# martinmodrak/math

Measured on AMD Instinct MI355X. Metric: gradient evals/sec (fp64), GP-marginal log-density N=4096, higher is better.
Workload: dtype f64; 1 GPU; gp_marginal_gradient; N=4096, kernel=exp_quad, parallelism=replicas1

## Files before the change

### include/smg_hip.h

```cpp
#ifndef SMG_HIP_H
#define SMG_HIP_H

#include <stddef.h>

#ifdef __cplusplus
extern "C" {
#endif

enum smg_status_code {
  SMG_OK = 0,
  SMG_ERR_HIP = 1,
  SMG_ERR_NOT_PD = 2,
  SMG_ERR_NOT_SYMMETRIC = 4,
  SMG_ERR_NONFINITE = 8,
  SMG_ERR_ARG = 16,
  SMG_ERR_OOM = 32,
  SMG_ERR_NOT_POSITIVE = 64,
  SMG_ERR_SYNC = 128
};

typedef struct smg_ctx smg_ctx;

int smg_device_count(int* n_host);
int smg_ctx_create(int device, size_t initial_arena_bytes, smg_ctx** out_host);
// ... 13 lines not shown
int smg_publish_to_host(smg_ctx* ctx, const double* src, long long n, double* dst);
int smg_gather_scalars(smg_ctx* ctx, const double* const* src, int n, double* dst, int* status_out);

int smg_memcpy_h2d(smg_ctx* ctx, void* dst, const void* src_host, size_t bytes);
int smg_memcpy_d2h(smg_ctx* ctx, void* dst_host, const void* src, size_t bytes);
int smg_memcpy_d2d(smg_ctx* ctx, void* dst, const void* src, size_t bytes);
int smg_memset(smg_ctx* ctx, void* dst, int value, size_t bytes);
int smg_memset_async(smg_ctx* ctx, void* dst, size_t bytes);
int smg_join_async(smg_ctx* ctx);
int smg_sync(smg_ctx* ctx);
int smg_sync_all(smg_ctx* ctx);
int smg_marker_record(smg_ctx* ctx, int slot);
int smg_marker_wait(smg_ctx* ctx, int slot);
int smg_status(smg_ctx* ctx, int* status_host);
int smg_status_armed(smg_ctx* ctx, int* armed);
int smg_status_enqueue(smg_ctx* ctx, int* host_dst);
int smg_status_inject(smg_ctx* ctx, int bits);
int smg_set_inv_block_mode(smg_ctx* ctx, int mode);
int smg_inv_block_fused(smg_ctx* ctx, int n);
int smg_set_gemm_stage_mode(smg_ctx* ctx, int mode);
int smg_set_gemm_cut_mode(smg_ctx* ctx, int mode);

enum smg_family {
  SMG_FAM_GEMM = 0, SMG_FAM_CHOL_FWD = 1, SMG_FAM_CHOL_REV = 2,
  SMG_FAM_GP = 3, SMG_FAM_MVN = 4, SMG_FAM_TRSV = 5, SMG_FAM_GLM = 6,
  SMG_FAM_ELEMWISE = 7,
  SMG_FAM_PANEL = 8,
  SMG_FAM_COMM = 9,
  SMG_FAM_COUNT = 10
};
int smg_profile_enable(smg_ctx* ctx, int on);
int smg_profile_read(smg_ctx* ctx, int family, double* total_ms_host, long long* count_host);
int smg_profile_flops(smg_ctx* ctx, int family, double* flops_host);

int smg_fill_unif(smg_ctx* ctx, double* out, long long n, unsigned long long seed,
                  double a, double b, double scale);
int smg_fill_bernoulli(smg_ctx* ctx, int* out, long long n, unsigned long long seed, double p);

int smg_gemm(smg_ctx* ctx, int transA, int transB, int uplo, int m, int n, int k,
             double alpha, const double* A, int lda, const double* B, int ldb,
             double beta, double* C, int ldc);
#define SMG_TRI_A_LOWER 1
#define SMG_TRI_A_UPPER 2
#define SMG_TRI_B_LOWER 4
#define SMG_TRI_B_UPPER 8
int smg_gemm_tri(smg_ctx* ctx, int transA, int transB, int uplo, int tri, int m, int n, int k, double alpha,
                 const double* A, int lda, const double* B, int ldb, double beta, double* C, int ldc);
int smg_gemm_bz(smg_ctx* ctx, int transA, int transB, int uplo, int tri, int m, int n, int k, double alpha,
                const double* A, int lda, const double* B, int ldb, double beta, double* C, int ldc, int bz);
int smg_gemm_cut(smg_ctx* ctx, int transA, int transB, int uplo, int tri, int m, int n, int k, double alpha,
                 const double* A, int lda, const double* B, int ldb, double beta, double* C, int ldc, int bz,
                 int cut_a, int cut_b);


int smg_gp_exp_quad_cov_fwd(smg_ctx* ctx, const double* x, int n, double sigma,
                            double l, double* K, int ldk);
int smg_gp_exp_quad_cov_rev(smg_ctx* ctx, const double* x, int n, double sigma,
                            double l, const double* Kadj, int ldka, double* out2);

int smg_gp_exp_quad_cov_nd_fwd(smg_ctx* ctx, const double* x, int D, int n, double sigma,
                               double l, double* K, int ldk);
int smg_gp_exp_quad_cov_nd_rev(smg_ctx* ctx, const double* x, int D, int n, double sigma,
                               double l, const double* Kadj, int ldka, double* out2);

enum smg_gp_family { SMG_GP_EXP_QUAD = 0, SMG_GP_EXPONENTIAL = 1, SMG_GP_MATERN32 = 2, SMG_GP_MATERN52 = 3 };
int smg_gp_cov_fwd(smg_ctx* ctx, int family, const double* x, int D, int n, double sigma, double l,
// ... 274 lines not shown
```

### math_amd/csrc/ctx.hip

```cpp
#include <cstdio>
#include <cstdlib>
#include <cstring>

#include "smg_internal.h"

namespace {

constexpr size_t kAlign = 256;

__global__ void k_reduce_partials(const double* __restrict__ p, int nparts,
                                  int width, double* out, int accumulate) {
  __shared__ double lds[16];
  const int c = blockIdx.x;
  double s = 0.0;
  for (int i = threadIdx.x; i < nparts; i += blockDim.x) s += p[(size_t)i * width + c];
  s = block_sum(s, lds);
  if (threadIdx.x == 0) out[c] = accumulate ? out[c] + s : s;
}

__global__ __launch_bounds__(256) void k_publish(const double* __restrict__ src, long long n, double* dst,
                                                 long long* done, long long seq) {
  for (long long i = threadIdx.x; i < n; i += blockDim.x)
    __hip_atomic_store(dst + i, src[i], __ATOMIC_RELAXED, __HIP_MEMORY_SCOPE_SYSTEM);
  asm volatile("s_waitcnt vmcnt(0)" ::: "memory");
// ... 490 lines not shown
  SMG_HIP_TRY(hipMemcpyAsync(dst, src, bytes, hipMemcpyDeviceToDevice, ctx->stream));
  return SMG_OK;
}

int smg_memset(smg_ctx* ctx, void* dst, int v, size_t bytes) {
  if (!bytes) return SMG_OK;
  if (v == 0) {
    const std::pair<void*, size_t> r(dst, bytes);
    return smg_zero_ranges_impl(ctx, ctx->stream, &r, 1);
  }
  SMG_HIP_TRY(hipMemsetAsync(dst, v, bytes, ctx->stream));
  return SMG_OK;
}

}

int smg_zero_ranges_impl(smg_ctx* ctx, hipStream_t stream, const std::pair<void*, size_t>* r, int count,
                         unsigned max_grid) {
  zero_ranges z{};
  size_t most = 0;
  auto launch = [&]() -> int {
    if (!z.count) return SMG_OK;
    const size_t g = (most / 2 + 255) / 256;
    hipLaunchKernelGGL(k_zero_ranges, dim3(g < max_grid ? (g < 1 ? 1 : (unsigned)g) : max_grid), dim3(256), 0, stream,
                       z);
    SMG_LAUNCH_CHECK();
    z.count = 0;
    most = 0;
    return SMG_OK;
  };
  for (int i = 0; i < count; ++i) {
    const size_t b = r[i].second;
    if (!b) continue;
    if ((reinterpret_cast<uintptr_t>(r[i].first) & 7) || (b & 7)) {
      SMG_HIP_TRY(hipMemsetAsync(r[i].first, 0, b, stream));
      continue;
    }
    z.p[z.count] = static_cast<double*>(r[i].first);
    z.n[z.count] = b / 8;
    most = b / 8 > most ? b / 8 : most;
    if (++z.count == ZR_MAX)
      if (int rc = launch()) return rc;
  }
  return launch();
}

extern "C" {

int smg_zero_stream_begin(smg_ctx* ctx) {
  if (ctx->zero_stream) return SMG_OK;
  if (hipStreamCreateWithFlags(&ctx->zero_stream, hipStreamNonBlocking) != hipSuccess ||
      hipEventCreateWithFlags(&ctx->zero_ev_main, hipEventDisableTiming) != hipSuccess ||
      hipEventCreateWithFlags(&ctx->zero_ev_done, hipEventDisableTiming) != hipSuccess) {
    hipGetLastError();
    ctx->zero_stream = nullptr;
    return SMG_ERR_HIP;
  }
  return SMG_OK;
}

int smg_marker_event(smg_ctx* ctx, int slot, hipEvent_t* ev) {
  if (slot < 0 || slot >= 64) return SMG_ERR_ARG;
  while ((int)ctx->marker_ev.size() <= slot) {
    hipEvent_t e;
    if (hipEventCreateWithFlags(&e, hipEventDisableTiming) != hipSuccess) {
      ctx->host_status |= SMG_ERR_HIP;
// ... 142 lines not shown
  if (in_host_scratch(ctx, host_dst, sizeof(int))) {
    hipLaunchKernelGGL(k_status_copy, dim3(1), dim3(64), 0, ctx->stream, ctx->status_d, host_dst);
    SMG_LAUNCH_CHECK();
  } else {
    SMG_HIP_TRY(hipMemcpyAsync(host_dst, ctx->status_d, sizeof(int), hipMemcpyDeviceToHost, ctx->stream));
  }
  ctx->status_armed = 0;
  return SMG_OK;
}

namespace {
__global__ void k_status_or(int* st, int bits) {
  if (threadIdx.x == 0) st[0] |= bits;
}
}

int smg_status_inject(smg_ctx* ctx, int bits) {
  if (!ctx) return SMG_ERR_ARG;
  hipLaunchKernelGGL(k_status_or, dim3(1), dim3(64), 0, ctx->stream, ctx->status_d, bits);
  SMG_LAUNCH_CHECK();
  ctx->status_armed = 1;
  return SMG_OK;
}

int smg_profile_enable(smg_ctx* ctx, int on) {
  hipStreamSynchronize(ctx->stream);
  prof_drain(ctx);
  ctx->prof_on = on;
  for (int i = 0; i < SMG_FAM_COUNT; ++i) {
    ctx->prof_ms[i] = 0;
    ctx->prof_count[i] = 0;
    ctx->prof_flops[i] = 0;
  }
  return SMG_OK;
}

int smg_profile_read(smg_ctx* ctx, int family, double* ms, long long* count) {
  if (family < 0 || family >= SMG_FAM_COUNT) return SMG_ERR_ARG;
  hipStreamSynchronize(ctx->stream);
  prof_drain(ctx);
  if (ms) *ms = ctx->prof_ms[family];
  if (count) *count = ctx->prof_count[family];
  return SMG_OK;
}

int smg_profile_flops(smg_ctx* ctx, int family, double* flops) {
  if (!ctx || family < 0 || family >= SMG_FAM_COUNT || !flops) return SMG_ERR_ARG;
  *flops = ctx->prof_flops[family];
  return SMG_OK;
}

}

namespace {
__device__ __forceinline__ unsigned long long splitmix(unsigned long long seed, long long i) {
  unsigned long long z = seed + (unsigned long long)(i + 1) * 0x9E3779B97F4A7C15ULL;
  z = (z ^ (z >> 30)) * 0xBF58476D1CE4E5B9ULL;
  z = (z ^ (z >> 27)) * 0x94D049BB133111EBULL;
  return z ^ (z >> 31);
}
__global__ void k_fill_unif(double* out, long long n, unsigned long long seed, double a, double b,
                            double scale) {
  for (long long i = (long long)blockIdx.x * blockDim.x + threadIdx.x; i < n;
       i += (long long)gridDim.x * blockDim.x) {
    const double u = (double)(splitmix(seed, i) >> 11) * (1.0 / 9007199254740992.0);
    const double v = __dadd_rn(a, __dmul_rn(b - a, u));
    out[i] = scale == 1.0 ? v : __dmul_rn(v, scale);
  }
// ... 27 lines not shown
```

### math_amd/csrc/smg_internal.h

```cpp
#pragma once
#include <hip/hip_runtime.h>

#include <cstddef>
#include <cstdint>
#include <utility>
#include <vector>

#include "../../include/smg_hip.h"

#ifndef SMG_GEMM_CUT_DEFAULT
#define SMG_GEMM_CUT_DEFAULT 1
#endif

typedef double d4 __attribute__((ext_vector_type(4)));
typedef double d2v __attribute__((ext_vector_type(2)));

struct smg_arena_block {
  char* base;
  size_t size;
};

struct smg_prof_slot {
  hipEvent_t start, stop;
  int family;
// ... 23 lines not shown
  hipStream_t copy_stream;
  hipEvent_t zero_ev_main, zero_ev_done;
  int zero_pending;
  std::vector<std::pair<void*, size_t>> zero_queue;
  hipEvent_t inv_ev, inv_ev_main, inv_ev_aux;
  int inv_pending;
  hipEvent_t inv_ev_w;
  int inv_w_recorded;
  int* flags_d;
  int flag_epoch;
  unsigned* inv_ctr_d;
  long long inv_launches;
  int inv_per_cu, inv_cus;
  int inv_mode;
  int gemm_stage;
  int gemm_cut;
  void* host_scratch;
  size_t host_scratch_size;
  void* pin_io;
  size_t pin_io_size;
  void* res_h;
  size_t res_h_size;
  long long* done_h;
  long long done_seq;
  unsigned int* red_counter_d;
  double* ws[12];
  size_t ws_doubles[12];
  int prof_on;
  std::vector<smg_prof_slot> prof_pending;
  std::vector<hipEvent_t> prof_pool;
  double prof_ms[SMG_FAM_COUNT];
  double prof_flops[SMG_FAM_COUNT];
  long long prof_count[SMG_FAM_COUNT];
  void* comm;
};

#define SMG_HIP_TRY(expr)                          \
  do {                                             \
    hipError_t _e = (expr);                        \
    if (_e != hipSuccess) {                        \
      if (ctx) ctx->host_status |= SMG_ERR_HIP;    \
      return SMG_ERR_HIP;                          \
    }                                              \
  } while (0)

#define SMG_LAUNCH_CHECK()                         \
  do {                                             \
    hipError_t _e = hipGetLastError();             \
    if (_e != hipSuccess) {                        \
      ctx->host_status |= SMG_ERR_HIP;             \
      return SMG_ERR_HIP;                          \
    }                                              \
  } while (0)

struct smg_prof_scope {
  smg_ctx* ctx;
  int fam;
  hipEvent_t a, b;
  bool on;
  smg_prof_scope(smg_ctx* c, int f);
  ~smg_prof_scope();
};

enum { SMG_WS_GEMM = 0, SMG_WS_RED = 1, SMG_WS_TMP = 2, SMG_WS_TMP2 = 3, SMG_WS_ALIAS = 4,
       SMG_WS_GEMM_SIDE = 5, SMG_WS_INV = 6, SMG_WS_CW = 7, SMG_WS_RHS = 8,
       SMG_WS_GLM = 9,
// ... 121 lines not shown
```

### math_amd/hip.py

```python
import ctypes
import os

import numpy as np

_HERE = os.path.dirname(os.path.abspath(__file__))
LIB_PATH = os.path.join(_HERE, "lib", "libsmg_hip.so")

SMG_OK = 0
STATUS = {1: "hip", 2: "not_pd", 4: "not_symmetric", 8: "nonfinite", 16: "arg", 32: "oom", 64: "not_positive"}
GP_FAMILIES = {"exp_quad": 0, "exponential": 1, "matern32": 2, "matern52": 3}
FAMILIES = {"gemm": 0, "chol_fwd": 1, "chol_rev": 2, "gp": 3, "mvn": 4, "trsv": 5, "glm": 6, "elementwise": 7, "panel": 8, "comm": 9}

_P = ctypes.c_void_p
_I = ctypes.c_int
_L = ctypes.c_longlong
_D = ctypes.c_double
_S = ctypes.c_size_t

_SIGS = {
    "smg_device_count": (_I, [ctypes.POINTER(_I)]),
    "smg_ctx_create": (_I, [_I, _S, ctypes.POINTER(_P)]),
    "smg_ctx_destroy": (_I, [_P]),
    "smg_ctx_device": (_I, [_P]),
    "smg_ctx_stream": (_P, [_P]),
    "smg_arena_alloc": (_P, [_P, _S]),
    "smg_arena_mark": (_S, [_P]),
    "smg_arena_rewind": (_I, [_P, _S]),
    "smg_arena_recover_all": (_I, [_P]),
    "smg_arena_used": (_S, [_P]),
    "smg_arena_reserved": (_S, [_P]),
    "smg_host_scratch": (_P, [_P, _S]),
    "smg_memcpy_h2d": (_I, [_P, _P, _P, _S]),
    "smg_memcpy_d2h": (_I, [_P, _P, _P, _S]),
    "smg_memcpy_d2d": (_I, [_P, _P, _P, _S]),
    "smg_memset": (_I, [_P, _P, _I, _S]),
    "smg_memset_async": (_I, [_P, _P, _S]),
    "smg_join_async": (_I, [_P]),
    "smg_sync": (_I, [_P]),
    "smg_sync_all": (_I, [_P]),
    "smg_status": (_I, [_P, ctypes.POINTER(_I)]),
    "smg_status_armed": (_I, [_P, ctypes.POINTER(_I)]),
    "smg_status_enqueue": (_I, [_P, _P]),
    "smg_status_inject": (_I, [_P, _I]),
    "smg_set_inv_block_mode": (_I, [_P, _I]),
    "smg_inv_block_fused": (_I, [_P, _I]),
    "smg_set_gemm_stage_mode": (_I, [_P, _I]),
    "smg_set_gemm_cut_mode": (_I, [_P, _I]),
    "smg_pinned_io": (_P, [_P, _S]),
    "smg_pinned_result": (_P, [_P, _S]),
    "smg_gather_scalars": (_I, [_P, _P, _I, _P, _P]),
    "smg_pack_tril": (_I, [_P, _I, _I, _P, _I, _P]),
    "smg_unpack_tril_add": (_I, [_P, _I, _I, _P, _P, _I]),
    "smg_publish_to_host": (_I, [_P, _P, _L, _P]),
    "smg_profile_enable": (_I, [_P, _I]),
    "smg_profile_read": (_I, [_P, _I, ctypes.POINTER(_D), ctypes.POINTER(_L)]),
    "smg_profile_flops": (_I, [_P, _I, ctypes.POINTER(_D)]),
    "smg_fill_unif": (_I, [_P, _P, _L, ctypes.c_ulonglong, _D, _D, _D]),
    "smg_fill_bernoulli": (_I, [_P, _P, _L, ctypes.c_ulonglong, _D]),
    "smg_gemm": (_I, [_P, _I, _I, _I, _I, _I, _I, _D, _P, _I, _P, _I, _D, _P, _I]),
    "smg_gemm_tri": (_I, [_P, _I, _I, _I, _I, _I, _I, _I, _D, _P, _I, _P, _I, _D, _P, _I]),
    "smg_gemm_bz": (_I, [_P, _I, _I, _I, _I, _I, _I, _I, _D, _P, _I, _P, _I, _D, _P, _I, _I]),
    "smg_gemm_cut": (_I, [_P, _I, _I, _I, _I, _I, _I, _I, _D, _P, _I, _P, _I, _D, _P, _I, _I, _I, _I]),
    "smg_gp_exp_quad_cov_fwd": (_I, [_P, _P, _I, _D, _D, _P, _I]),
    "smg_gp_exp_quad_cov_rev": (_I, [_P, _P, _I, _D, _D, _P, _I, _P]),
    "smg_bernoulli_logit_glm_checked": (_I, [_P, _P, _P, _L, _I, _L, _P, _P, _P]),
    "smg_bernoulli_logit_glm_io": (_I, [_P, _P, _P, _L, _I, _L, _D, _P, _P, _P, _P]),
    "smg_marker_record": (_I, [_P, _I]),
    "smg_marker_wait": (_I, [_P, _I]),
    "smg_gp_exp_quad_cov_nd_fwd": (_I, [_P, _P, _I, _I, _D, _D, _P, _I]),
    "smg_gp_exp_quad_cov_nd_rev": (_I, [_P, _P, _I, _I, _D, _D, _P, _I, _P]),
    "smg_add_diag_fwd": (_I, [_P, _P, _I, _I, _D, _P, _P, _I]),
    "smg_add_diag_rev": (_I, [_P, _P, _I, _I, _P, _I, _P, _I]),
    "smg_cholesky_block_size": (_I, [_I]),
    "smg_check_symmetric": (_I, [_P, _P, _I, _I]),
    "smg_cholesky_fwd": (_I, [_P, _P, _I, _I, _P, _I, _P]),
    "smg_cholesky_fwd_checked": (_I, [_P, _P, _I, _I, _P, _I, _P]),
    "smg_cholesky_fwd_checked_mark": (_I, [_P, _P, _I, _I, _P, _I, _P]),
    "smg_status_mark_wait": (_I, [_P, _P]),
    "smg_cholesky_rev": (_I, [_P, _P, _I, _P, _P, _I, _I, _P, _I]),
    "smg_mdivide_left_tri_fwd": (_I, [_P, _I, _P, _I, _P, _I, _I, _I, _P, _I]),
    "smg_mdivide_left_tri_rev": (_I, [_P, _I, _P, _I, _P, _I, _P, _I, _I, _I, _P, _I, _P, _I, _P]),
    "smg_mdivide_left_tri_aux_fwd": (_I, [_P, _I, _P, _I, _P, _P, _I, _I, _I, _P, _I]),
    "smg_mdivide_left_tri_aux_rev": (_I, [_P, _I, _P, _I, _P, _P, _I, _P, _I, _I, _I, _P, _I, _P, _I, _P]),
    "smg_chol_tangent_fwd": (_I, [_P, _P, _I, _P, _P, _I, _I, _P, _P, _P, _P, _P, _I]),
    "smg_chol_tangent_fwd_w": (_I, [_P, _P, _I, _P, _P, _I, _I, _P, _P, _P, _P, _I]),
    "smg_chol_tangent_rev": (_I, [_P, _P, _I, _P, _P, _P, _P, _I, _P, _I, _I, _P, _I, _P, _I, _P]),
    "smg_multiply_lower_fwd": (_I, [_P, _P, _I, _P, _I, _I, _P, _I]),
    "smg_multiply_lower_rev": (_I, [_P, _P, _I, _P, _I, _P, _I, _I, _P, _I, _P, _I, _P]),
    "smg_multiply_fwd": (_I, [_P, _P, _I, _P, _I, _I, _I, _I, _P, _I]),
# ... 214 lines not shown
```

### math_amd/include/stan/math/amd/matrix.hpp

```cpp
#ifndef STAN_MATH_AMD_MATRIX_HPP
#define STAN_MATH_AMD_MATRIX_HPP


#include <stan/math/amd/device.hpp>
#include <stan/math/amd/host_parallel.hpp>
#include <stan/math/rev/core/grad.hpp>
#include <stan/math/rev/core/var.hpp>
#include <stan/math/rev/core/vari.hpp>

#include <algorithm>
#include <cmath>
#include <functional>
#include <new>
#include <sstream>
#include <stdexcept>
#include <vector>

namespace stan {
namespace math {

enum class dev_structure : int {
  general = 0,
  lower = 1,
  symmetric = 2
// ... 6 lines not shown
  int n = 0, k = 1;
  long long ss = 0;
  double adj = 0.0;
  size_t sweep = 0;
  void expand_into(double* Aadj) const {
    amd::check(smg_cholesky_inverse_adjoint(amd::ctx(), C, n, n, s, k, ss, adj, Aadj, n), "cholesky_decompose");
  }
};

inline bool others_write_device_adjoint(size_t pos, const void* node, const vari* except) {
  const auto& w = ChainableStack::instance_->dev_writers_;
  auto it = std::upper_bound(w.begin(), w.end(), pos, [](size_t p, const dev_writer& d) { return p < d.pos; });
  for (; it != w.end(); ++it)
    if (it->v != except && it->v->may_write_device_adjoint(node)) return true;
  return false;
}

class structured_adjoint_sink {
 public:
  virtual bool take_inverse_adjoint(const inverse_adjoint& d, double* dadj) {
    (void)d;
    (void)dadj;
    return false;
  }
  virtual bool take_mvn_adjoint(const vari* owner, const double* ws, double adj, int k = 1) {
    (void)owner;
    (void)ws;
    (void)adj;
    (void)k;
    return false;
  }
  virtual void prepare_mvn_adjoint() {}
  virtual void expand_adjoint() {}
  virtual const double* inverse_factor() { return nullptr; }
  virtual bool gp_source(smg_gp_source* out) {
    (void)out;
    return false;
  }
  virtual bool chol_source(smg_gp_source* out) {
    (void)out;
    return false;
  }
};

class dev_matrix_vari;

class deferred_value_source {
 public:
  virtual void form_values(dev_matrix_vari* m) = 0;

 protected:
  ~deferred_value_source() = default;
};

namespace amd {
inline bool& deferred_values_flag() {
  static thread_local bool on = true;
  return on;
}
inline bool deferred_values_enabled() { return deferred_values_flag(); }
inline void set_deferred_values(bool on) { deferred_values_flag() = on; }
inline size_t& materialisation_count() {
  static thread_local size_t n = 0;
  return n;
}
}

class dev_matrix_vari {
  double* val_;
  deferred_value_source* pending_ = nullptr;

 public:
  const int rows_;
  const int cols_;
  double* adj_;
  dev_structure structure_;
  double* aux_;
  dev_matrix_vari* transpose_of_ = nullptr;
  structured_adjoint_sink* sink_ = nullptr;

  dev_matrix_vari(int rows, int cols, dev_structure s = dev_structure::general)
      : val_(amd::alloc_doubles(size_t(rows) * cols)),
        rows_(rows),
        cols_(cols),
        adj_(amd::alloc_doubles(size_t(rows) * cols)),
        structure_(s),
        aux_(nullptr) {
    register_device_adjoint(adj_, size_t(rows) * cols);
  }

  size_t size() const { return size_t(rows_) * cols_; }

  const double* val() {
    if (pending_) force_values();
    return val_;
  }
  double* raw_val() { return val_; }
  bool values_pending() const { return pending_ != nullptr; }
  void defer_values(deferred_value_source* producer) { pending_ = producer; }
  void force_values() {
    deferred_value_source* p = pending_;
    if (!p) return;
    pending_ = nullptr;
    ++amd::materialisation_count();
    p->form_values(this);
  }

  static inline void* operator new(size_t nbytes) {
    return ChainableStack::instance_->memalloc_.alloc(nbytes);
  }
  static inline void operator delete(void*) {}
};

class dev_var_matrix {
 public:
  dev_matrix_vari* vi_;

  dev_var_matrix() : vi_(nullptr) {}
  explicit dev_var_matrix(dev_matrix_vari* vi) : vi_(vi) {}

  int rows() const { return vi_->rows_; }
  int cols() const { return vi_->cols_; }
  size_t size() const { return vi_->size(); }
  const double* val_ptr() const { return vi_->val(); }
  double* adj_ptr() const { return vi_->adj_; }

  std::vector<double> val() const {
    std::vector<double> h(size());
    amd::to_host(h.data(), vi_->val(), size());
    return h;
  }
  std::vector<double> adj() const {
    if (vi_->sink_) vi_->sink_->expand_adjoint();
    join_device_adjoints();
    std::vector<double> h(size());
    amd::to_host(h.data(), vi_->adj_, size());
    return h;
  }

#ifdef STAN_MATH_AMD_HAS_EIGEN
  operator Eigen::Matrix<var, Eigen::Dynamic, Eigen::Dynamic>() const;
  operator Eigen::Matrix<var, Eigen::Dynamic, 1>() const;
#endif
};

template <typename T>
class dev_data {
 public:
  const T* ptr_ = nullptr;
  size_t n_ = 0;
  int rows_ = 0, cols_ = 0;
  dev_data() = default;
  dev_data(const T* p, size_t n, int rows, int cols) : ptr_(p), n_(n), rows_(rows), cols_(cols) {}
  size_t size() const { return n_; }
  int rows() const { return rows_; }
  int cols() const { return cols_; }
  const T* data() const { return ptr_; }
};

inline dev_data<double> to_dev_data(const double* h, size_t n, int rows = -1, int cols = 1) {
  double* d = amd::alloc_doubles(n);
  amd::to_device(d, h, n);
  return dev_data<double>(d, n, rows < 0 ? int(n) : rows, cols);
}
inline dev_data<double> to_dev_data(const std::vector<double>& v) {
  return to_dev_data(v.data(), v.size());
}
inline dev_data<int> to_dev_data(const std::vector<int>& v) {
  int* d = amd::alloc_ints(v.size());
  amd::to_device_int(d, v.data(), v.size());
  return dev_data<int>(d, v.size(), int(v.size()), 1);
}

namespace internal {
struct dev_operand {
  dev_matrix_vari* vi = nullptr;
  const double* data = nullptr;
  int rows = 0, cols = 0;
  const double* val() const { return vi ? vi->val() : data; }
  double* adj() const { return vi ? vi->adj_ : nullptr; }
  size_t size() const { return size_t(rows) * size_t(cols); }
};
inline dev_operand operand(const dev_var_matrix& m) { return dev_operand{m.vi_, nullptr, m.rows(), m.cols()}; }
inline dev_operand operand(const dev_data<double>& d) { return dev_operand{nullptr, d.data(), d.rows(), d.cols()}; }
}

inline dev_var_matrix to_dev_var_matrix(const double* host_colmajor, int rows, int cols) {
  auto* vi = new dev_matrix_vari(rows, cols);
  amd::to_device(vi->raw_val(), host_colmajor, size_t(rows) * cols);
  return dev_var_matrix(vi);
}

namespace internal {

enum block_layout : int { layout_dense = 0, layout_lower = 1, layout_sym = 2, layout_diag = 3 };

inline size_t tril_off(size_t n, size_t j) { return j * n - j * (j - 1) / 2; }
inline size_t tril_count(size_t n) { return n * (n + 1) / 2; }

inline void block_column_ptrs(const std::vector<host_block>& blocks, const host_block& b, size_t j, vari** out);

template <typename F>
inline void block_column_own(const host_block& b, size_t j, F&& f) {
  const size_t r = size_t(b.rows);
  switch (b.layout) {
    case layout_lower: {
      for (size_t i = 0; i < j && i < r; ++i) f(i, b.dummy);
      vari* c = b.first + tril_off(r, j) - j;
      for (size_t i = j; i < r; ++i) f(i, c + i);
      break;
    }
    case layout_sym: {
      vari* p = b.first + j;
      for (size_t i = 0; i < j && i < r; ++i) {
        f(i, p);
        p += r - i - 1;
// ... 101 lines not shown
  size_t pos_;
  size_t ran_ = 0;
  bool wrote_ = false;
  explicit dev_to_host_vari(size_t blk)
      : vari(0.0), blk_(blk), pos_(ChainableStack::instance_->var_stack_.size() - 1) {
    local_adjoint_vari::register_dev_writer(this);
  }
  bool reads_other_adjoints() const override { return true; }
  bool touches_adjoints_in(const vari*, const vari*) const override { return false; }
  bool may_write_device_adjoint(const void* node) const override {
    auto* st = ChainableStack::instance_;
    return node == st->host_blocks_[blk_].node && (ran_ != st->sweep_ || wrote_);
  }
  void chain() override {
    auto* st = ChainableStack::instance_;
    ran_ = st->sweep_;
    wrote_ = false;
    const host_block b = st->host_blocks_[blk_];
    if (!b.n) return;
    const bool touched = b.dirty || b.touched_sweep == st->sweep_;
    if (!touched) return;
    wrote_ = true;
    smg_ctx* c = amd::ctx();
    double* stage = static_cast<double*>(smg_host_scratch(c, b.n * sizeof(double)));
    if (!stage) throw std::bad_alloc();
    host_parallel_for(b.n, [&](size_t s, size_t e) {
      for (size_t i = s; i < e; ++i) stage[i] = b.first[i].adj_;
    });
    double* dst = amd::alloc_doubles(b.n);
    auto* node = static_cast<dev_matrix_vari*>(b.node);
    amd::check(smg_memcpy_h2d(c, dst, stage, b.n * sizeof(double)), "to_host");
    const int mode = block_pack_mode(b.layout);
    if (mode < 0)
      amd::check(smg_axpy(c, (long long)b.n, 1.0, dst, 1, node->adj_, 1), "to_host");
    else
      amd::check(smg_unpack_tril_add(c, mode, mode == 2 ? int(b.n) : b.rows, dst, node->adj_, b.rows), "to_host");
    amd::check(smg_sync(c), "to_host");
  }
};

inline void publish_block_adjoints(size_t from) {
  auto* st = ChainableStack::instance_;
  if (from >= st->host_blocks_.size() || !amd::has_ctx()) return;
  smg_ctx* c = amd::ctx();
  join_device_adjoints();
  const size_t nb = st->host_blocks_.size();
  std::vector<size_t> off(nb + 1, 0);
  for (size_t k = from; k < nb; ++k) {
    const host_block& b = st->host_blocks_[k];
    off[k + 1] = off[k] + (b.n ? b.n + (b.layout == layout_lower ? 1 : 0) : 0);
  }
  if (off[nb] == 0) return;
  double* stage = static_cast<double*>(smg_host_scratch(c, off[nb] * sizeof(double)));
  if (!stage) throw std::bad_alloc();
  for (size_t k = from; k < nb; ++k) {
    const host_block b = st->host_blocks_[k];
    if (!b.n) continue;
    auto* node = static_cast<dev_matrix_vari*>(b.node);
    if (node->sink_) node->sink_->expand_adjoint();
    const double* src = node->adj_;
    const int mode = block_pack_mode(b.layout);
    const size_t cnt = off[k + 1] - off[k];
    if (mode >= 0) {
      double* t = amd::alloc_doubles(cnt);
      amd::check(smg_pack_tril(c, mode, mode == 2 ? int(b.n) : b.rows, node->adj_, b.rows, t), "grad");
      if (b.layout == layout_lower) amd::check(smg_sum_strict_upper(c, b.rows, node->adj_, b.rows, t + b.n), "grad");
      src = t;
    }
    amd::check(smg_memcpy_d2h(c, stage + off[k], src, cnt * sizeof(double)), "grad");
  }
  amd::check(smg_sync(c), "grad");
  for (size_t k = from; k < nb; ++k) {
    host_block& b = st->host_blocks_[k];
    if (!b.n) continue;
    const double* h = stage + off[k];
    host_parallel_for(b.n, [&](size_t s, size_t e) {
      for (size_t i = s; i < e; ++i) b.first[i].adj_ = h[i];
    });
    if (b.layout == layout_lower && b.dummy) {
      b.dummy->adj_ += h[b.n] - b.dummy_dev;
      b.dummy_dev = h[b.n];
    }
  }
}

inline void stream_varis(vari* first, const double* src, size_t n, const std::function<void()>& overlap) {
  if (!n) {
    if (overlap) overlap();
    return;
  }
  smg_ctx* c = amd::ctx();
  int armed = 0;
  amd::check(smg_status_armed(c, &armed), "to_host");
  double* stage = static_cast<double*>(smg_host_scratch(c, (n + 1) * sizeof(double)));
  if (!stage) throw std::bad_alloc();
  const int nch = n >= (size_t(1) << 21) ? 8 : 1;
  const size_t chunk = (n + size_t(nch) - 1) / size_t(nch);
  if (armed) amd::check(smg_status_enqueue(c, reinterpret_cast<int*>(stage + n)), "to_host");
  for (int k = 0; k < nch; ++k) {
// ... 56 lines not shown
  b.base_elems = base_elems;
  b.n = size_t(std::min(B->rows_, B->cols_));
  b.first = static_cast<vari*>(st->memalloc_.alloc((b.n ? b.n : 1) * sizeof(vari)));
  b.dummy = nullptr;
  if (b.n) {
    double* t = amd::alloc_doubles(b.n);
    amd::check(smg_pack_tril(amd::ctx(), 2, int(b.n), B->val(), b.rows, t), "add_diag");
    stream_varis(b.first, t, b.n, nullptr);
  }
  return push_block(b);
}

class host_to_dev_vari : public host_local_vari {
 public:
  dev_matrix_vari* dst_;
  vari** elems_;
  host_to_dev_vari(dev_matrix_vari* dst, vari** elems) : host_local_vari(0.0), dst_(dst), elems_(elems) {}
  bool touches_adjoints_in(const vari* lo, const vari* hi) const override {
    const size_t n = dst_->size();
    return !host_parallel_all(n, [&](size_t s, size_t e) {
      for (size_t i = s; i < e; ++i)
        if (elems_[i] >= lo && elems_[i] < hi) return false;
      return true;
    });
  }
  void chain() override {
    const size_t n = dst_->size();
    if (!n) return;
    smg_ctx* c = amd::ctx();
    int armed = 0;
    amd::check(smg_status_armed(c, &armed), "to_dev");
    double* h = static_cast<double*>(smg_host_scratch(c, (n + 1) * sizeof(double)));
    if (!h) throw std::bad_alloc();
    amd::check(smg_memcpy_d2h(c, h, dst_->adj_, n * sizeof(double)), "to_dev");
    if (armed) amd::check(smg_status_enqueue(c, reinterpret_cast<int*>(h + n)), "to_dev");
    amd::check(smg_sync(c), "to_dev");
    if (armed) amd::throw_if_sync(*reinterpret_cast<int*>(h + n), "to_dev", "a persistent solve");
    for (size_t i = 0; i < n; ++i) elems_[i]->adj_ += h[i];
  }
};

inline dev_var_matrix to_dev_vars(const var* d, size_t n, int rows, int cols, const char* nan_fn = nullptr,
                                  const char* nan_name = nullptr);
}

inline dev_var_matrix to_dev(const std::vector<var>& v, int rows = -1, int cols = 1) {
  const size_t n = v.size();
  if (rows < 0) rows = int(n);
  if (size_t(rows) * size_t(cols) != n) throw std::invalid_argument("to_dev: rows * cols != size");
  return internal::to_dev_vars(v.data(), n, rows, cols);
}

inline std::vector<var> to_var_vector(const dev_var_matrix& m) {
  std::vector<var> out(m.size());
  internal::materialise(m.vi_, [&](const host_block& b) { internal::fill_block_pointers(b, out.data()); });
  return out;
}

namespace internal {
inline void throw_not_nan(const char* fn, const char* name, size_t i) {
  std::ostringstream m;
  m << fn << ": " << name << "[" << i + 1 << "] is nan, but must not be nan!";
  throw std::domain_error(m.str());
}

inline dev_var_matrix to_dev_vars(const var* d, size_t n, int rows, int cols, const char* nan_fn,
                                  const char* nan_name) {
// ... 41 lines not shown
```

### math_amd/include/stan/math/eigen/interop.hpp

```cpp
#ifndef STAN_MATH_EIGEN_INTEROP_HPP
#define STAN_MATH_EIGEN_INTEROP_HPP


#include <Eigen/Dense>

#if defined(STAN_MATH_AMD_MATRIX_HPP) && !defined(STAN_MATH_AMD_HAS_EIGEN)
#error "include <stan/math.hpp> (or define STAN_MATH_AMD_HAS_EIGEN) before stan/math/amd/matrix.hpp"
#endif
#ifndef STAN_MATH_AMD_HAS_EIGEN
#define STAN_MATH_AMD_HAS_EIGEN 1
#endif

#include <stan/math/amd/matrix.hpp>
#include <stan/math/rev/core.hpp>
#include <stan/math/rev/fun/cholesky_decompose.hpp>
#include <stan/math/rev/fun/gp_exp_quad_cov.hpp>
#include <stan/math/rev/fun/gp_matern_cov.hpp>
#include <stan/math/rev/fun/gp_ard_cov.hpp>
#include <stan/math/rev/fun/gp_cross_cov.hpp>
#include <stan/math/rev/fun/gp_periodic_cov.hpp>
#include <stan/math/rev/fun/multi_normal_cholesky_lpdf.hpp>
#include <stan/math/rev/fun/bernoulli_logit_glm_lpmf.hpp>
#include <stan/math/rev/fun/categorical_logit_glm_lpmf.hpp>
#include <stan/math/rev/fun/neg_binomial_2_log_glm_lpmf.hpp>
// ... 78 lines not shown
  e.n = size_t(m.size());
  e.rows = int(m.rows());
  e.cols = int(m.cols());
  e.block = recognise_block_index(e.vd, e.n, e.rows, e.cols);
  if (e.block >= 0) e.node = static_cast<dev_matrix_vari*>(ChainableStack::instance_->host_blocks_[size_t(e.block)].node);
  if (nan_fn) {
    if (e.node) {
      smg_ctx* c = amd::ctx();
      double* flag = amd::alloc_doubles(1);
      amd::check(smg_memset(c, flag, 0, sizeof(double)), nan_fn);
      amd::check(smg_check_domain(c, e.node->val(), (long long)e.n, 0, flag), nan_fn);
      double f = 0;
      amd::to_host(&f, flag, 1);
      if (f == 0.0) return e;
    }
    for (size_t i = 0; i < e.n; ++i)
      if (std::isnan(e.vd[i].vi_->val_)) throw_not_nan(nan_fn, nan_name, i);
  }
  return e;
}
template <int R, int C, int O, int MR, int MC>
inline eig_in prepare(const Eigen::Matrix<double, R, C, O, MR, MC>& m, const char* nan_fn = nullptr,
                      const char* nan_name = nullptr) {
  eig_in e;
  e.dd = m.data();
  e.n = size_t(m.size());
  e.rows = int(m.rows());
  e.cols = int(m.cols());
  if (nan_fn)
    for (size_t i = 0; i < e.n; ++i)
      if (std::isnan(e.dd[i])) throw_not_nan(nan_fn, nan_name, i);
  return e;
}
inline dev_operand commit(const eig_in& e) {
  if (e.node) return operand(dev_var_matrix(e.node));
  if (e.vd) return operand(to_dev_vars(e.vd, e.n, e.rows, e.cols));
  return operand(to_dev_data(e.dd, e.n, e.rows, e.cols));
}
}

template <int R = Eigen::Dynamic, int C = Eigen::Dynamic>
inline Eigen::Matrix<var, R, C> to_host_matrix(const dev_var_matrix& m) {
  Eigen::Matrix<var, R, C> out(m.rows(), m.cols());
  var* d = out.data();
  internal::materialise(m.vi_, [&](const host_block& b) { internal::fill_block_pointers(b, d); });
  return out;
}

template <int R, int C, int O, int MR, int MC>
inline dev_var_matrix to_dev(const Eigen::Matrix<var, R, C, O, MR, MC>& m) {
  return internal::to_dev_vars(m.data(), size_t(m.size()), int(m.rows()), int(m.cols()));
}

inline dev_var_matrix::operator Eigen::Matrix<var, Eigen::Dynamic, Eigen::Dynamic>() const {
  return to_host_matrix<Eigen::Dynamic, Eigen::Dynamic>(*this);
}
inline dev_var_matrix::operator Eigen::Matrix<var, Eigen::Dynamic, 1>() const {
  return to_host_matrix<Eigen::Dynamic, 1>(*this);
}

template <int R, int C, int O, int MR, int MC>
inline dev_data<double> to_dev_data(const Eigen::Matrix<double, R, C, O, MR, MC>& m) {
  return to_dev_data(m.data(), size_t(m.size()), int(m.rows()), int(m.cols()));
}

inline matrix_d value_of(const dev_var_matrix& m) {
  std::vector<double> v = m.val();
  return Eigen::Map<matrix_d>(v.data(), m.rows(), m.cols());
// ... 86 lines not shown
template <int R, int C>
inline var sum(const Eigen::Matrix<var, R, C>& m) {
  return sum(to_dev(m));
}

namespace internal {
template <typename T_m>
inline matrix_v add_diag_output(const Eigen::Matrix<T_m, Eigen::Dynamic, Eigen::Dynamic>& mat, const eig_in& em,
                                const dev_var_matrix& B) {
  if constexpr (!is_var<T_m>::value) {
    return to_host_matrix(B);
  } else {
    matrix_v out(mat.rows(), mat.cols());
    const long base = em.block;
    vari** elems = nullptr;
    if (base < 0 && em.n) {
      elems = ChainableStack::instance_->memalloc_.alloc_array<vari*>(em.n);
      host_parallel_for(em.n, [&](size_t s, size_t e) {
        for (size_t i = s; i < e; ++i) elems[i] = em.vd[i].vi_;
      });
    }
    const size_t k = materialise_diag(B.vi_, base, elems);
    fill_block_pointers(ChainableStack::instance_->host_blocks_[k], out.data());
    return out;
  }
}
}

template <typename T_m, typename T_a,
          typename = std::enable_if_t<internal::is_ad_scalar<T_m>::value && internal::is_ad_scalar<T_a>::value &&
                                      internal::any_var<T_m, T_a>::value>>
inline matrix_v add_diag(const Eigen::Matrix<T_m, Eigen::Dynamic, Eigen::Dynamic>& mat, const T_a& to_add) {
  const internal::eig_in em = internal::prepare(mat);
  const internal::dev_operand a = internal::commit(em);
  if constexpr (internal::is_var<T_a>::value)
    return internal::add_diag_output(mat, em, internal::add_diag_dev(a, to_add.val(), to_add.vi_, {}));
  else
    return internal::add_diag_output(mat, em, internal::add_diag_dev(a, double(to_add), nullptr, {}));
}
template <typename T_m, typename T_a, int R, int C,
          typename = std::enable_if_t<internal::is_ad_scalar<T_m>::value && internal::is_ad_scalar<T_a>::value &&
                                      internal::any_var<T_m, T_a>::value>>
inline matrix_v add_diag(const Eigen::Matrix<T_m, Eigen::Dynamic, Eigen::Dynamic>& mat,
                         const Eigen::Matrix<T_a, R, C>& to_add) {
  const size_t k = size_t(std::min(mat.rows(), mat.cols()));
  if (size_t(to_add.size()) != k) {
    std::ostringstream m;
    m << "add_diag: number of elements of to_add has dimension = " << to_add.size() << ", expecting dimension = " << k
      << "; a function was called with arguments of different scalar, array, vector, or matrix types, and they "
         "were not consistently sized;  all arguments must be scalars or multidimensional values of the same shape.";
    throw std::invalid_argument(m.str());
  }
  const internal::eig_in em = internal::prepare(mat);
  const internal::eig_in ed = internal::prepare(to_add);
  const internal::dev_operand a = internal::commit(em);
  internal::dev_operand d = internal::commit(ed);
  d.rows = int(d.size());
  d.cols = 1;
  return internal::add_diag_output(mat, em, internal::add_diag_dev(a, 0.0, nullptr, d));
}

template <int R, int C>
inline var log_sum_exp(const Eigen::Matrix<var, R, C>& x) {
  return log_sum_exp(to_dev(x));
}
template <int R, int C>
inline Eigen::Matrix<var, R, C> lgamma(const Eigen::Matrix<var, R, C>& x) {
  return to_host_matrix<R, C>(lgamma(to_dev(x)));
}
template <int R, int C>
inline Eigen::Matrix<var, R, C> digamma(const Eigen::Matrix<var, R, C>& x) {
  return to_host_matrix<R, C>(digamma(to_dev(x)));
}

template <int TriView, typename T1, int R1, int C1, typename T2, int R2, int C2,
          typename = std::enable_if_t<internal::is_ad_scalar<T1>::value && internal::is_ad_scalar<T2>::value &&
                                      internal::any_var<T1, T2>::value>>
inline Eigen::Matrix<var, R1, C2> mdivide_left_tri(const Eigen::Matrix<T1, R1, C1>& A,
                                                   const Eigen::Matrix<T2, R2, C2>& b) {
  internal::check_square("mdivide_left_tri", "A", int(A.rows()), int(A.cols()));
  internal::check_multiplicable("mdivide_left_tri", int(A.rows()), int(A.cols()), int(b.rows()), int(b.cols()), "A",
                                "b");
  const internal::dev_operand a = internal::commit(internal::prepare(A));
  const internal::dev_operand bb = internal::commit(internal::prepare(b));
  return to_host_matrix<R1, C2>(internal::mdivide_left_tri_dev<TriView>(a, bb));
}
template <int TriView, int R, int C>
inline Eigen::Matrix<var, R, C> mdivide_left_tri(const Eigen::Matrix<var, R, C>& A) {
// ... 217 lines not shown
  throw std::invalid_argument(m.str());
}

template <typename S>
struct mvt_dev {
  std::vector<const double*> val;
  std::vector<double*> adj;
};
inline mvt_dev<double> mvt_to_dev(const std::vector<const double*>& p, int n) {
  std::vector<double> h;
  h.reserve(p.size() * size_t(n));
  for (const double* e : p) h.insert(h.end(), e, e + n);
  dev_data<double> d = to_dev_data(h.data(), h.size(), n, int(p.size()));
  mvt_dev<double> out;
  for (size_t i = 0; i < p.size(); ++i) {
    out.val.push_back(d.data() + i * size_t(n));
    out.adj.push_back(nullptr);
  }
  return out;
}
inline mvt_dev<var> mvt_to_dev(const std::vector<const var*>& p, int n) {
  dev_matrix_vari* node = nullptr;
  if (p.size() == 1) {
    node = to_dev_vars(p[0], size_t(n), n, 1).vi_;
  } else {
    std::vector<var> h;
    h.reserve(p.size() * size_t(n));
    for (const var* e : p) h.insert(h.end(), e, e + n);
    node = to_dev_vars(h.data(), h.size(), n, int(p.size())).vi_;
  }
  mvt_dev<var> out;
  for (size_t i = 0; i < p.size(); ++i) {
    out.val.push_back(node->val() + i * size_t(n));
    out.adj.push_back(node->adj_ + i * size_t(n));
  }
  return out;
}

}

template <bool propto = false, typename T_y, typename T_loc, typename T_covar,
          typename = std::enable_if_t<internal::is_mvt_arg<T_y>::value && internal::is_mvt_arg<T_loc>::value &&
                                      (internal::is_ad_scalar<typename internal::scalar_of<T_covar>::type>::value)>>
inline std::conditional_t<internal::any_var<T_y, T_loc, T_covar>::value, var, double> multi_normal_cholesky_lpdf(
    const T_y& y, const T_loc& mu, const T_covar& L) {
  using S_y = typename internal::scalar_of<T_y>::type;
  using S_mu = typename internal::scalar_of<T_loc>::type;
  using S_L = typename internal::scalar_of<T_covar>::type;
  using ret_t = std::conditional_t<internal::any_var<T_y, T_loc, T_covar>::value, var, double>;
  constexpr bool L_var = internal::is_var<S_L>::value;
  constexpr bool any_v = internal::any_var<T_y, T_loc, T_covar>::value;
  const char* fn = "multi_normal_cholesky_lpdf";
  const size_t len_y = internal::is_array_mvt<T_y>::value ? size_t(y.size()) : 1;
  const size_t len_mu = internal::is_array_mvt<T_loc>::value ? size_t(mu.size()) : 1;
  const size_t max_len = std::max(len_y, len_mu);
  internal::check_consistent_size_mvt(fn, "y", y, max_len);
  internal::check_consistent_size_mvt(fn, "mu", mu, max_len);
  if (len_y == 0 || len_mu == 0) return ret_t(0.0);
  std::vector<const S_y*> py;
  std::vector<const S_mu*> pm;
  std::vector<int> ny, nm;
  internal::seq_of(y, py, ny);
  internal::seq_of(mu, pm, nm);
  const size_t size_vec = max_len;
  const int size_y = ny[0], size_mu = nm[0];
  if (size_vec > 1) {
    for (size_t i = 1; i < ny.size(); ++i)
// ... 2 lines not shown
    for (size_t i = 1; i < nm.size(); ++i)
      internal::size_match(fn, "Size of one of the vectors of the location variable", nm[i],
                           "Size of another vector of the location variable", nm[i - 1]);
  }
  internal::size_match(fn, "Size of random variable", size_y, "size of location parameter", size_mu);
  internal::size_match(fn, "Size of random variable", size_y, "rows of covariance parameter", (long long)L.rows());
  internal::size_match(fn, "Size of random variable", size_y, "columns of covariance parameter",
                       (long long)L.cols());
  for (size_t i = 0; i < size_vec; ++i) {
    const S_mu* m = pm[len_mu > 1 ? i : 0];
    for (int j = 0; j < size_mu; ++j) {
      const double v = internal::host_value(m[j]);
      if (!std::isfinite(v)) {
        std::ostringstream o;
        o << fn << ": Location parameter[" << j + 1 << "] is " << v << ", but must be finite!";
        throw std::domain_error(o.str());
      }
    }
    const S_y* yy = py[len_y > 1 ? i : 0];
    for (int j = 0; j < size_y; ++j)
      if (std::isnan(internal::host_value(yy[j]))) {
        std::ostringstream o;
        o << fn << ": Random variable[" << j + 1 << "] is nan, but must not be nan!";
        throw std::domain_error(o.str());
      }
  }
  if (size_y == 0) return ret_t(0.0);
  if (propto && !any_v) return ret_t(0.0);
  internal::dev_operand Ld;
  const double* aux = nullptr;
  bool lower_only = false;
  double host_logdet = 0.0;
  if constexpr (std::is_same<T_covar, dev_var_matrix>::value) {
    Ld = internal::operand(L);
    aux = L.vi_->aux_;
    lower_only = L.vi_->structure_ == dev_structure::lower;
  } else {
    const internal::eig_in eL = internal::prepare(L);
    Ld = internal::commit(eL);
    if (Ld.vi) {
      aux = Ld.vi->aux_;
      lower_only = Ld.vi->structure_ == dev_structure::lower;
    }
    if (!L_var && propto)
      for (int i = 0; i < size_y; ++i) host_logdet += std::log(1.0 / internal::host_value(L(i, i)));
  }
  const internal::mvt_dev<S_y> dy = internal::mvt_to_dev(py, size_y);
  const internal::mvt_dev<S_mu> dm = internal::mvt_to_dev(pm, size_y);
  auto* obs = ChainableStack::instance_->memalloc_.alloc_array<internal::mvn_obs>(size_vec);
  for (size_t i = 0; i < size_vec; ++i) {
    const size_t iy = len_y > 1 ? i : 0, im = len_mu > 1 ? i : 0;
    obs[i] = internal::mvn_obs{dy.val[iy], dy.adj[iy], dm.val[im], dm.adj[im]};
  }
  double lp = 0.0;
  vari* node = internal::mvn_cholesky_multi(Ld, aux, lower_only, obs, int(size_vec), !propto, !propto || L_var,
                                            host_logdet, &lp);
  if constexpr (any_v)
    return node ? var(node) : var(lp);
  else
    return lp;
}

namespace internal {
template <typename T_x>
inline dev_data<double> gp_points_to_device(const std::vector<T_x>& x, int& D) {
  const size_t n = x.size();
  D = n ? int(x[0].size()) : 1;
  for (size_t i = 0; i < n; ++i)
    for (int d = 0; d < int(x[i].size()); ++d)
      if (std::isnan(x[i](d))) {
        std::ostringstream m;
        m << "gp_exp_quad_cov: x[" << d + 1 << "] is nan, but must not be nan!";
// ... 314 lines not shown
```

### math_amd/include/stan/math/mix/fvar_functors.hpp

```cpp
#ifndef STAN_MATH_MIX_FVAR_FUNCTORS_HPP
#define STAN_MATH_MIX_FVAR_FUNCTORS_HPP


#include <stan/math/amd/matrix.hpp>
#include <stan/math/fwd/core/fvar.hpp>
#include <stan/math/rev/core.hpp>
#include <stan/math/rev/fun/cholesky_decompose.hpp>
#include <cstdlib>
#include <stan/math/rev/fun/gp_exp_quad_cov.hpp>
#include <stan/math/rev/fun/mdivide_left_tri.hpp>
#include <stan/math/rev/fun/multi_normal_cholesky_lpdf.hpp>
#include <stan/math/rev/fun/multiply.hpp>
#include <stan/math/rev/fun/tangent_ops.hpp>
#include <stan/math/rev/fun/log_sum_exp.hpp>
#include <stan/math/rev/fun/bernoulli_logit_glm_lpmf.hpp>

#include <vector>

namespace stan {
namespace math {

struct dev_fvar_matrix {
  dev_var_matrix val_;
  dev_var_matrix d_;
  int rows() const { return val_.rows(); }
  int cols() const { return val_.cols(); }
};

inline dev_fvar_matrix gp_exp_quad_cov(const dev_data<double>& x, const fvar<var>& sigma,
                                       const fvar<var>& length_scale) {
  dev_fvar_matrix K;
  K.val_ = gp_exp_quad_cov(x, sigma.val_, length_scale.val_);
  K.d_ = gp_exp_quad_cov_tangent(x, sigma.val_, length_scale.val_, sigma.d_, length_scale.d_);
  return K;
}
inline dev_fvar_matrix gp_exp_quad_cov(const std::vector<double>& x, const fvar<var>& sigma,
                                       const fvar<var>& length_scale) {
  return gp_exp_quad_cov(internal::gp_x_to_device(x), sigma, length_scale);
}

inline dev_fvar_matrix add_diag(const dev_fvar_matrix& A, const fvar<var>& d) {
  return dev_fvar_matrix{add_diag(A.val_, d.val_), add_diag(A.d_, d.d_)};
}
inline dev_fvar_matrix add_diag(const dev_fvar_matrix& A, double d) {
  return dev_fvar_matrix{add_diag(A.val_, d), A.d_};
}

namespace internal {
class multiply_lower_dev_vari : public device_vari {
 public:
  dev_matrix_vari* A_;
  dev_matrix_vari* B_;
  dev_matrix_vari* C_;
  multiply_lower_dev_vari(dev_matrix_vari* A, dev_matrix_vari* B)
      : device_vari(0.0), A_(A), B_(B), C_(new dev_matrix_vari(A->rows_, B->cols_, dev_structure::lower)) {
    const int n = A->rows_;
    amd::check(smg_multiply_lower_fwd(amd::ctx(), A_->val(), n, B_->val(), n, n, C_->raw_val(), n), "multiply");
  }
  void chain() override {
    const int n = A_->rows_;
    double* ws = amd::alloc_doubles(size_t(n) * n);
    amd::check(smg_multiply_lower_rev(amd::ctx(), A_->val(), n, B_->val(), n, C_->adj_, n, n, A_->adj_, n,
                                      B_->adj_, n, ws),
               "multiply");
  }
};
}

namespace internal {
class add_dev_vari : public device_vari {
 public:
  dev_matrix_vari* A_;
  dev_matrix_vari* B_;
  dev_matrix_vari* C_;
  add_dev_vari(dev_matrix_vari* A, dev_matrix_vari* B)
      : device_vari(0.0), A_(A), B_(B), C_(new dev_matrix_vari(A->rows_, A->cols_)) {
    smg_ctx* c = amd::ctx();
    amd::check(smg_copy_matrix(c, A->rows_, A->cols_, A->val(), A->rows_, C_->raw_val(), C_->rows_, 0, 0), "add");
    amd::check(smg_axpy(c, (long long)C_->size(), 1.0, B->val(), 1, C_->raw_val(), 1), "add");
  }
  void chain() override {
    smg_ctx* c = amd::ctx();
    amd::check(smg_axpy(c, (long long)C_->size(), 1.0, C_->adj_, 1, A_->adj_, 1), "add");
    amd::check(smg_axpy(c, (long long)C_->size(), 1.0, C_->adj_, 1, B_->adj_, 1), "add");
  }
};

class tril_dev_vari : public device_vari {
 public:
  dev_matrix_vari* A_;
  dev_matrix_vari* C_;
  explicit tril_dev_vari(dev_matrix_vari* A)
      : device_vari(0.0), A_(A), C_(new dev_matrix_vari(A->rows_, A->cols_, dev_structure::lower)) {
    smg_ctx* c = amd::ctx();
    amd::zero(C_->raw_val(), C_->size());
    amd::check(smg_add_tril(c, A->rows_, A->cols_, 1.0, A->val(), A->rows_, C_->raw_val(), C_->rows_), "tril");
  }
  void chain() override {
    amd::check(smg_add_tril(amd::ctx(), A_->rows_, A_->cols_, 1.0, C_->adj_, C_->rows_, A_->adj_, A_->rows_),
               "tril");
  }
};

class lse_tangent_dev_vari : public device_vari {
 public:
  dev_matrix_vari* x_;
  dev_matrix_vari* xd_;
  double lse_;
  lse_tangent_dev_vari(double t, double lse, dev_matrix_vari* x, dev_matrix_vari* xd)
      : device_vari(t), x_(x), xd_(xd), lse_(lse) {}
  void chain() override {
    amd::check(smg_lse_tangent_rev(amd::ctx(), x_->val(), xd_->val(), (long long)x_->size(), lse_, val_, adj_,
                                   x_->adj_, xd_->adj_),
               "log_sum_exp");
  }
};

class glm_tangent_dev_vari : public device_vari {
 public:
  dev_matrix_vari* eta_;
  dev_matrix_vari* etad_;
  vari* alpha_;
  vari* alphad_;
  double a_, ad_;
  const int* y_;
  double* out2_;
  glm_tangent_dev_vari(double t, dev_matrix_vari* eta, dev_matrix_vari* etad, vari* alpha, vari* alphad, double a,
                       double ad, const int* y)
      : device_vari(t), eta_(eta), etad_(etad), alpha_(alpha), alphad_(alphad), a_(a), ad_(ad), y_(y),
        out2_(amd::alloc_doubles(2)) {}
  void chain() override {
    amd::check(smg_glm_tangent_rev(amd::ctx(), eta_->val(), a_, etad_->val(), ad_, y_, (long long)eta_->size(), adj_,
                                   eta_->adj_, etad_->adj_, out2_),
               "bernoulli_logit_glm_lpmf");
    if (alpha_) add_pending_adjoint(alpha_, out2_);
    if (alphad_) add_pending_adjoint(alphad_, out2_ + 1);
  }
};
}

inline dev_var_matrix add(const dev_var_matrix& A, const dev_var_matrix& B) {
  if (A.rows() != B.rows() || A.cols() != B.cols()) throw std::invalid_argument("add: size mismatch");
  return dev_var_matrix((new internal::add_dev_vari(A.vi_, B.vi_))->C_);
}
inline dev_var_matrix tril(const dev_var_matrix& A) {
  return dev_var_matrix((new internal::tril_dev_vari(A.vi_))->C_);
}

#ifdef STAN_MATH_AMD_HAS_EIGEN
template <int R, int C>
inline dev_fvar_matrix to_dev(const Eigen::Matrix<fvar<var>, R, C>& m, int rows = -1, int cols = -1) {
  const size_t n = size_t(m.size());
  std::vector<var> v(n), d(n);
  for (size_t i = 0; i < n; ++i) {
    v[i] = m(Eigen::Index(i)).val_;
    d[i] = m(Eigen::Index(i)).d_;
  }
  if (rows < 0) {
    rows = int(m.rows());
    cols = int(m.cols());
  }
  return dev_fvar_matrix{to_dev(v, rows, cols), to_dev(d, rows, cols)};
}
#endif
inline dev_fvar_matrix to_dev(const std::vector<fvar<var>>& x, int rows = -1, int cols = 1) {
  std::vector<var> v(x.size()), d(x.size());
// ... 77 lines not shown
    lp.d_ = var(0.0);
    return lp;
  }
  dev_var_matrix eta = multiply(x, beta.val_);
  dev_var_matrix etad = multiply(x, beta.d_);
  smg_ctx* c = amd::ctx();
  double* out = amd::alloc_doubles(1);
  amd::check(smg_glm_tangent_fwd(c, eta.val_ptr(), alpha.val_.val(), etad.val_ptr(), alpha.d_.val(), y.data(), R, out),
             "bernoulli_logit_glm_lpmf");
  double t = 0.0;
  amd::to_host(&t, out, 1);
  lp.d_ = var(new internal::glm_tangent_dev_vari(t, eta.vi_, etad.vi_, alpha.val_.vi_, alpha.d_.vi_,
                                                 alpha.val_.val(), alpha.d_.val(), y.data()));
  return lp;
}
template <bool propto = false>
inline fvar<var> bernoulli_logit_glm_lpmf(const dev_data<int>& y, const dev_data<double>& x, const fvar<var>& alpha,
                                          const std::vector<fvar<var>>& beta) {
  return bernoulli_logit_glm_lpmf<propto>(y, x, alpha, to_dev(beta));
}

namespace internal {
class chol_tangent_dev_vari : public device_vari {
 public:
  dev_matrix_vari* L_;
  dev_matrix_vari* Ad_;
  dev_matrix_vari* Ld_;
  double* W_;
  double* Wt_;
  double* Y_;
  double* P_;
  chol_tangent_dev_vari(dev_matrix_vari* L, dev_matrix_vari* Ad)
      : device_vari(0.0), L_(L), Ad_(Ad), Ld_(new dev_matrix_vari(L->rows_, L->cols_, dev_structure::lower)) {
    const int n = L->rows_;
    const size_t nn = size_t(n) * n;
    Wt_ = amd::alloc_doubles(nn);
    Y_ = amd::alloc_doubles(nn);
    P_ = amd::alloc_doubles(nn);
    const double* Wf = L_->sink_ ? L_->sink_->inverse_factor() : nullptr;
    if (Wf) {
      W_ = const_cast<double*>(Wf);
      amd::check(smg_chol_tangent_fwd_w(amd::ctx(), L_->val(), n, W_, Ad_->val(), n, n, Wt_, Y_, P_, Ld_->raw_val(), n),
                 "cholesky_decompose");
      return;
    }
    W_ = amd::alloc_doubles(nn);
    amd::check(smg_chol_tangent_fwd(amd::ctx(), L_->val(), n, L_->aux_, Ad_->val(), n, n, W_, Wt_, Y_, P_, Ld_->raw_val(), n),
               "cholesky_decompose");
  }
  void chain() override {
    const int n = L_->rows_;
    double* ws = amd::alloc_doubles(2 * size_t(n) * n);
    amd::check(smg_chol_tangent_rev(amd::ctx(), L_->val(), n, W_, Wt_, Y_, P_, n, Ld_->adj_, n, n, L_->adj_, n,
                                    Ad_->adj_, n, ws),
               "cholesky_decompose");
  }
};
inline bool chol_tangent_composed() {
  static const bool c = [] {
    const char* e = std::getenv("SMG_CHOL_TANGENT_COMPOSED");
    return e && std::atoi(e) != 0;
  }();
  return c;
}
}

inline dev_fvar_matrix cholesky_decompose(const dev_fvar_matrix& A) {
  dev_fvar_matrix L;
  if (!internal::chol_tangent_composed()) {
    L.val_ = internal::cholesky_decompose_with_inverse(A.val_);
    L.d_ = dev_var_matrix((new internal::chol_tangent_dev_vari(L.val_.vi_, A.d_.vi_))->Ld_);
    return L;
  }
  L.val_ = cholesky_decompose(A.val_);
  dev_var_matrix X = mdivide_left_tri<1>(L.val_, A.d_);
  dev_var_matrix Y = mdivide_left_tri<1>(L.val_, transpose(X));
  dev_var_matrix P = phi_lower(Y);
  L.d_ = dev_var_matrix((new internal::multiply_lower_dev_vari(L.val_.vi_, P.vi_))->C_);
  return L;
}

namespace internal {
inline var mvn_cholesky_tangent(const dev_fvar_matrix& L, const dev_data<double>& r) {
  dev_var_matrix w = mdivide_left_tri<1>(L.val_, r);
  dev_var_matrix z = mdivide_left_tri<1>(L.val_, multiply(L.d_, w));
  return dot_product(w, z) - diag_ratio_sum(L.d_, L.val_);
}
template <bool propto>
inline fvar<var> mvn_cholesky_fvar(const std::vector<double>& y, const std::vector<double>& mu,
                                   const dev_fvar_matrix& L) {
  fvar<var> lp;
  lp.val_ = multi_normal_cholesky_lpdf<propto>(y, mu, L.val_);
  if (y.empty()) return lp;
  std::vector<double> r(y.size());
  for (size_t i = 0; i < y.size(); ++i) r[i] = y[i] - mu[i];
  lp.d_ = mvn_cholesky_tangent(L, to_dev_data(r));
  return lp;
}
}

template <bool propto = false>
inline fvar<var> multi_normal_cholesky_lpdf(const dev_data<double>& y, const dev_fvar_matrix& L) {
// ... 36 lines not shown
```

### math_amd/include/stan/math/rev/core/autodiffstackstorage.hpp

```cpp
#ifndef STAN_MATH_REV_CORE_AUTODIFFSTACKSTORAGE_HPP
#define STAN_MATH_REV_CORE_AUTODIFFSTACKSTORAGE_HPP


#include <stan/math/memory/stack_alloc.hpp>

#include <cstddef>
#include <vector>

namespace stan {
namespace math {

class vari;
class chainable_alloc;

struct dev_buffer {
  double* ptr;
  size_t n;
};
struct pending_adjoint {
  vari* target;
  const double* src;
};
struct host_block {
  vari* first;
  size_t n;
  void* node;
  vari* dummy;
  int rows, cols;
  bool dirty;
  int layout = 0;
  long base = -1;
  vari* const* base_elems = nullptr;
  double dummy_dev = 0.0;
  size_t touched_sweep = 0;
};
struct dev_writer {
  size_t pos;
  vari* v;
};

template <typename ChainableT, typename ChainableAllocT>
struct AutodiffStackSingleton {
  using AutodiffStackSingleton_t = AutodiffStackSingleton<ChainableT, ChainableAllocT>;

  struct AutodiffStackStorage {
    AutodiffStackStorage& operator=(const AutodiffStackStorage&) = delete;

    std::vector<ChainableT*> var_stack_;
    std::vector<ChainableT*> var_nochain_stack_;
    std::vector<ChainableAllocT*> var_alloc_stack_;
    stack_alloc memalloc_;

    std::vector<size_t> nested_var_stack_sizes_;
    std::vector<size_t> nested_var_nochain_stack_sizes_;
    std::vector<size_t> nested_var_alloc_stack_starts_;

    std::vector<dev_buffer> dev_adj_stack_;
    std::vector<size_t> nested_dev_adj_sizes_;
    std::vector<size_t> nested_dev_marks_;
    std::vector<pending_adjoint> pending_;
    std::vector<host_block> host_blocks_;
    std::vector<size_t> nested_host_block_sizes_;
    std::vector<dev_writer> dev_writers_;
    std::vector<size_t> block_order_;
    size_t block_order_sweep_ = 0;
    size_t sweep_ = 0;
    void (*publish_)(size_t from) = nullptr;
    int no_publish_ = 0;
  };

  AutodiffStackSingleton() : own_instance_(init()) {}
  ~AutodiffStackSingleton() {
    if (own_instance_) {
      delete instance_;
      instance_ = nullptr;
    }
  }
  AutodiffStackSingleton(const AutodiffStackSingleton_t&) = delete;
  AutodiffStackSingleton& operator=(const AutodiffStackSingleton_t&) = delete;

#ifdef STAN_MATH_AMD_TLS_INITIAL_EXEC
  static inline thread_local AutodiffStackStorage* instance_ __attribute__((tls_model("initial-exec"))) = nullptr;
#else
  static inline thread_local AutodiffStackStorage* instance_ = nullptr;
#endif

 private:
  static bool init() {
    if (!instance_) {
      instance_ = new AutodiffStackStorage();
      return true;
    }
    return false;
  }
  bool own_instance_;
};

using ChainableStack = AutodiffStackSingleton<vari, chainable_alloc>;

// ... 6 lines not shown
```

### math_amd/include/stan/math/rev/core/grad.hpp

```cpp
#ifndef STAN_MATH_REV_CORE_GRAD_HPP
#define STAN_MATH_REV_CORE_GRAD_HPP


#include <stan/math/amd/device.hpp>
#include <stan/math/rev/core/vari.hpp>

#include <algorithm>
#include <cstdint>
#include <typeinfo>
#include <stdexcept>
#include <vector>

namespace stan {
namespace math {

inline void register_device_adjoint(double* p, size_t n) {
  if (n >= (size_t(1) << 17))
    amd::check(smg_memset_async(amd::ctx(), p, n * sizeof(double)), "zero");
  else
    amd::zero(p, n);
  ChainableStack::instance_->dev_adj_stack_.push_back({p, n});
}

inline void join_device_adjoints() {
  if (amd::has_ctx()) amd::check(smg_join_async(amd::ctx()), "grad");
}

inline void add_pending_adjoint(vari* target, const double* src) {
  ChainableStack::instance_->pending_.push_back({target, src});
}

inline void flush_pending(bool status = false) {
  auto& pend = ChainableStack::instance_->pending_;
  int armed = 0;
  if (status && amd::has_ctx()) amd::check(smg_status_armed(amd::ctx(), &armed), "grad");
  if (pend.empty() && !armed) return;
  smg_ctx* c = amd::ctx();
  const size_t n = pend.size();
  double* stage = static_cast<double*>(smg_pinned_result(c, (n + 1) * sizeof(double)));
  if (!stage) throw std::bad_alloc();
  std::vector<const double*> src(n);
  for (size_t i = 0; i < n; ++i) src[i] = pend[i].src;
  int* st = reinterpret_cast<int*>(stage + n);
  amd::check(smg_gather_scalars(c, src.data(), int(n), stage, armed ? st : nullptr), "flush_pending");
  auto& blocks = ChainableStack::instance_->host_blocks_;
  for (size_t i = 0; i < n; ++i) {
    vari* t = pend[i].target;
    t->adj_ += stage[i];
    for (auto& b : blocks)
      if (t >= b.first && t < b.first + b.n) b.dirty = true;
  }
  pend.clear();
  if (armed) amd::throw_if_sync(*st, "grad", "the reverse sweep");
}

inline void log_host_touches(vari* v) {
  auto* st = ChainableStack::instance_;
  auto& blocks = st->host_blocks_;
// ... 105 lines not shown

static inline void recover_memory() {
  if (!empty_nested())
    throw std::logic_error("empty_nested() must be true before calling recover_memory()");
  auto* st = ChainableStack::instance_;
  st->var_stack_.clear();
  st->dev_writers_.clear();
  st->var_nochain_stack_.clear();
  for (auto* a : st->var_alloc_stack_) delete a;
  st->var_alloc_stack_.clear();
  st->dev_adj_stack_.clear();
  st->pending_.clear();
  st->host_blocks_.clear();
  if (amd::has_ctx()) smg_arena_recover_all(amd::ctx());
  st->memalloc_.recover_all();
}

static inline void zero_host_blocks(size_t from) {
  auto& blocks = ChainableStack::instance_->host_blocks_;
  for (size_t k = from; k < blocks.size(); ++k) {
    host_block& b = blocks[k];
    for (size_t i = 0; i < b.n; ++i) b.first[i].adj_ = 0.0;
    if (b.dummy) b.dummy->adj_ = 0.0;
    b.dummy_dev = 0.0;
    b.dirty = false;
  }
}

static inline void set_zero_all_adjoints() {
  auto* st = ChainableStack::instance_;
  ++st->sweep_;
  for (auto* v : st->var_stack_) v->set_zero_adjoint();
  for (auto* v : st->var_nochain_stack_) v->set_zero_adjoint();
  for (auto& b : st->dev_adj_stack_) amd::zero(b.ptr, b.n);
  zero_host_blocks(0);
  st->pending_.clear();
}

static inline void set_zero_all_adjoints_nested() {
  if (empty_nested())
    throw std::logic_error(
        "empty_nested() must be false before calling set_zero_all_adjoints_nested()");
  auto* st = ChainableStack::instance_;
  ++st->sweep_;
  const size_t s1 = st->nested_var_stack_sizes_.back();
  for (size_t i = (s1 == 0U) ? 0U : (s1 - 1); i < st->var_stack_.size(); ++i)
    st->var_stack_[i]->set_zero_adjoint();
  const size_t s2 = st->nested_var_nochain_stack_sizes_.back();
  for (size_t i = (s2 == 0U) ? 0U : (s2 - 1); i < st->var_nochain_stack_.size(); ++i)
    st->var_nochain_stack_[i]->set_zero_adjoint();
  for (size_t i = st->nested_dev_adj_sizes_.back(); i < st->dev_adj_stack_.size(); ++i)
    amd::zero(st->dev_adj_stack_[i].ptr, st->dev_adj_stack_[i].n);
  zero_host_blocks(st->nested_host_block_sizes_.back());
  st->pending_.clear();
}

static inline void free_memory() { ChainableStack::instance_->memalloc_.free_all(); }

}
}
#endif
```

### math_amd/include/stan/math/rev/fun/bernoulli_logit_glm_lpmf.hpp

```cpp
#ifndef STAN_MATH_REV_FUN_BERNOULLI_LOGIT_GLM_LPMF_HPP
#define STAN_MATH_REV_FUN_BERNOULLI_LOGIT_GLM_LPMF_HPP


#include <stan/math/amd/comm.hpp>
#include <stan/math/amd/matrix.hpp>
#include <stan/math/rev/core.hpp>
#include <stan/math/rev/fun/normal_lpdf.hpp>

#include <cmath>
#include <sstream>
#include <stdexcept>
#include <string>
#include <type_traits>
#include <vector>

namespace stan {
namespace math {

struct glm_shard {
  const int* y = nullptr;
  const double* yd = nullptr;
  const double* x = nullptr;
  long long rows = 0;
  int M = 0;
// ... 3 lines not shown
  bool distributed = false;
};

inline void row_partition(long long R, int world, int rank, long long* begin, long long* end) {
  *begin = R * rank / world;
  *end = R * (rank + 1) / world;
}

namespace internal {

class glm_dev_vari : public local_adjoint_vari {
 public:
  vari* alpha_vi_;
  vari** beta_vi_;
  dev_matrix_vari* beta_dev_;
  double* g_;
  const double* g_dev_;
  int M_;
  glm_dev_vari(double lp, vari* a, vari** b, dev_matrix_vari* bd, double* g, const double* gd, int M)
      : local_adjoint_vari(lp), alpha_vi_(a), beta_vi_(b), beta_dev_(bd), g_(g), g_dev_(gd), M_(M) {}
  bool touches_adjoints_in(const vari* lo, const vari* hi) const override {
    auto in = [&](const vari* v) { return v && v >= lo && v < hi; };
    if (in(alpha_vi_)) return true;
    if (beta_vi_)
      for (int j = 0; j < M_; ++j)
        if (in(beta_vi_[j])) return true;
    return false;
  }
  void chain() override {
    if (alpha_vi_) alpha_vi_->adj_ += adj_ * g_[0];
    if (beta_vi_)
      for (int j = 0; j < M_; ++j) beta_vi_[j]->adj_ += adj_ * g_[1 + j];
    if (beta_dev_)
      amd::check(smg_axpy(amd::ctx(), M_, adj_, g_dev_, 1, beta_dev_->adj_, 1),
                 "bernoulli_logit_glm_lpmf");
  }
};

inline void glm_throw_y_bounds(const char* fn, const int* y, long long n, int lo, int hi, long long row0) {
  smg_ctx* c = amd::ctx();
  const long long chunk = 1 << 20;
  for (long long i0 = 0; i0 < n; i0 += chunk) {
    const long long k = n - i0 < chunk ? n - i0 : chunk;
    int* stage = static_cast<int*>(smg_host_scratch(c, size_t(k) * sizeof(int)));
    if (!stage) throw std::bad_alloc();
    amd::check(smg_memcpy_d2h(c, stage, y + i0, size_t(k) * sizeof(int)), fn);
    amd::check(smg_sync(c), fn);
    for (long long i = 0; i < k; ++i)
      if (stage[i] < lo || stage[i] > hi) {
        std::ostringstream m;
        m << fn << ": Vector of dependent variables[" << row0 + i0 + i + 1 << "] is " << stage[i]
          << ", but must be in the interval [" << lo << ", " << hi << "]";
        throw std::domain_error(m.str());
      }
  }
  std::ostringstream m;
  m << fn << ": Vector of dependent variables is out of bounds (on another rank's rows), but must be in "
          "the interval [" << lo << ", " << hi << "]";
  throw std::domain_error(m.str());
}

struct glm_params {
  double alpha = 0;
  vari* alpha_vi = nullptr;
  std::vector<double> beta;
  vari** beta_vi = nullptr;
  dev_matrix_vari* beta_dev = nullptr;
// ... 175 lines not shown
```

### math_amd/include/stan/math/rev/fun/cholesky_decompose.hpp

```cpp
#ifndef STAN_MATH_REV_FUN_CHOLESKY_DECOMPOSE_HPP
#define STAN_MATH_REV_FUN_CHOLESKY_DECOMPOSE_HPP


#include <stan/math/amd/matrix.hpp>
#include <stan/math/rev/core.hpp>

#include <cmath>
#include <cstdlib>
#include <sstream>
#include <stdexcept>
#include <utility>
#include <vector>

namespace stan {
namespace math {

namespace internal {

class add_diag_dev_vari : public device_vari, public structured_adjoint_sink, public deferred_value_source {
 public:
  dev_operand A_;
  dev_matrix_vari* B_;
  vari* d_vi_;
  double* dadj_;
  dev_operand dv_;
  size_t pos_;
  inverse_adjoint dep_, exp_;
  const double d_;
  smg_gp_source src_;
  bool has_src_ = false;

  add_diag_dev_vari(const dev_operand& A, double d, vari* d_vi, const dev_operand& dv)
      : device_vari(0.0), A_(A), B_(new dev_matrix_vari(A.rows, A.cols)), d_vi_(d_vi),
        dadj_(d_vi ? amd::alloc_doubles(1) : nullptr), dv_(dv),
        pos_(ChainableStack::instance_->var_stack_.size() - 1), d_(d), src_{} {
    if (A.rows == A.cols && !dv.rows) B_->sink_ = this;
    if (amd::deferred_values_enabled() && B_->sink_ == this && A.rows > 0 && A_.vi && A_.vi->sink_ &&
        std::isfinite(d) && A_.vi->sink_->gp_source(&src_) && src_.n == A.rows) {
      src_.d = d;
      has_src_ = true;
      B_->defer_values(this);
      return;
    }
    form_values(B_);
  }
  void form_values(dev_matrix_vari*) override {
    smg_ctx* c = amd::ctx();
    const int m = A_.rows, n = A_.cols, k = m < n ? m : n;
    const double* dvec = dv_.rows ? dv_.val() : nullptr;
    if (m == n) {
      amd::check(smg_add_diag_fwd(c, A_.val(), m, m, d_, dvec, B_->raw_val(), m), "add_diag");
    } else if (m && n) {
      amd::check(smg_memcpy_d2d(c, B_->raw_val(), A_.val(), size_t(m) * n * sizeof(double)), "add_diag");
      amd::check(smg_add_diag_fwd(c, B_->raw_val(), m, k, d_, dvec, B_->raw_val(), m), "add_diag");
    }
  }
  bool chol_source(smg_gp_source* out) override {
    if (!has_src_ || !B_->values_pending()) return false;
    *out = src_;
    return true;
  }
  bool may_write_device_adjoint(const void* node) const override {
    return (A_.vi && node == A_.vi) || (dv_.vi && node == dv_.vi);
  }
  bool take_inverse_adjoint(const inverse_adjoint& d, double*) override {
    if (B_->sink_ != this) return false;
    if (dep_.C && dep_.sweep == ChainableStack::instance_->sweep_) return false;
    dep_ = d;
    return true;
  }
  void expand_adjoint() override {
    const size_t sw = ChainableStack::instance_->sweep_;
    if (exp_.C && exp_.sweep == sw) exp_.expand_into(B_->adj_);
    exp_ = inverse_adjoint{};
    if (dep_.C && dep_.sweep == sw) dep_.expand_into(B_->adj_);
    dep_ = inverse_adjoint{};
  }

  void chain() override {
    smg_ctx* c = amd::ctx();
    const int m = A_.rows, n = A_.cols, k = m < n ? m : n;
    if (!m || !n) return;
    auto* st = ChainableStack::instance_;
    if (dep_.C && dep_.sweep == st->sweep_) {
      const inverse_adjoint d = dep_;
      dep_ = inverse_adjoint{};
      if (!others_write_device_adjoint(pos_, B_, d.owner)) {
        inverse_adjoint pass = d;
        pass.owner = this;
        const bool passed = A_.vi && A_.vi->sink_ && A_.vi->sink_->take_inverse_adjoint(pass, dadj_);
        if (!passed) {
          if (A_.adj()) pass.expand_into(A_.adj());
          if (dadj_)
            amd::check(smg_gp_inverse_adjoint(c, d.C, n, n, d.s, d.k, d.ss, d.adj, nullptr, n, nullptr, 1, 1.0, 1.0,
                                              dadj_, nullptr),
                       "add_diag");
        }
        if (d_vi_) add_pending_adjoint(d_vi_, dadj_);
        exp_ = d;
        return;
      }
      d.expand_into(B_->adj_);
    }
    double* dadj = dv_.rows ? dv_.adj() : dadj_;
    if (dadj_) amd::check(smg_memset(c, dadj_, 0, sizeof(double)), "add_diag");
    const int vec = dv_.rows ? 1 : 0;
    if (m == n) {
      amd::check(smg_add_diag_rev(c, B_->adj_, m, m, A_.adj(), m, dadj, vec), "add_diag");
    } else {
      if (A_.adj())
        amd::check(smg_axpy(c, (long long)m * n, 1.0, B_->adj_, 1, A_.adj(), 1), "add_diag");
      amd::check(smg_add_diag_rev(c, B_->adj_, m, k, nullptr, 0, dadj, vec), "add_diag");
    }
    if (d_vi_) add_pending_adjoint(d_vi_, dadj_);
  }
};

class cholesky_dev_vari : public device_vari, public structured_adjoint_sink {
 public:
  dev_matrix_vari* A_;
  dev_matrix_vari* L_;
  int n_;
  size_t pos_;
  const vari* dep_owner_ = nullptr;
  const double* dep_ws_ = nullptr;
  double dep_adj_ = 0.0;
  int dep_k_ = 1;
  size_t dep_sweep_ = 0;
  double* ws_ = nullptr;
  bool early_ = false;
  const double* winv_ = nullptr;
  bool v_ready_ = false;
  bool c_ready_ = false;
  const double* exp_ws_ = nullptr;
  double exp_adj_ = 0.0;
  int exp_k_ = 1;
  size_t exp_sweep_ = 0;
  void expand(const double* ws, double adj, int k) const {
    for (int o = 0; o < k; ++o)
      amd::check(smg_mvn_cholesky_rev(amd::ctx(), L_->raw_val(), n_, L_->aux_, n_, ws + 2 * size_t(n_) * o, adj, 1, nullptr,
                                      nullptr, L_->adj_, n_),
                 "cholesky_decompose");
  }

  static std::vector<std::pair<std::pair<size_t, int>, bool>>& history() {
    static thread_local std::vector<std::pair<std::pair<size_t, int>, bool>> h;
    return h;
  }
  static int history_of(size_t pos, int n) {
    for (const auto& e : history())
      if (e.first.first == pos && e.first.second == n) return e.second ? 1 : 0;
    return -1;
  }
  static bool predicted(size_t pos, int n) { return history_of(pos, n) == 1; }
  void record(bool closed) const {
    auto& h = history();
    for (auto& e : h)
      if (e.first.first == pos_ && e.first.second == n_) {
        e.second = closed;
        return;
      }
    if (h.size() >= 64) h.erase(h.begin());
    h.push_back({{pos_, n_}, closed});
  }

  static bool closed_form_enabled() {
    static const bool on = [] {
      const char* e = std::getenv("SMG_CHOL_MVN_CLOSED_FORM");
      return !(e && e[0] == '0');
    }();
    return on;
  }

  cholesky_dev_vari(dev_matrix_vari* A, dev_matrix_vari* L)
// ... 49 lines not shown
    smg_ctx* c = amd::ctx();
    auto* st = ChainableStack::instance_;
    const size_t nn = size_t(n_) * n_;
    const bool deposit = dep_owner_ && dep_sweep_ == st->sweep_;
    if (deposit) {
      const vari* owner = dep_owner_;
      dep_owner_ = nullptr;
      const bool dense = others_write_device_adjoint(pos_, L_, owner);
      record(!dense);
      if (!dense) {
        exp_ws_ = dep_ws_;
        exp_adj_ = dep_adj_;
        exp_k_ = dep_k_;
        exp_sweep_ = st->sweep_;
        if (v_ready_) {
          amd::check(smg_cholesky_mvn_rev_v(c, n_, dep_ws_ + n_, dep_k_, 2LL * n_, dep_adj_, nullptr, n_, ws_,
                                            c_ready_ ? 1 : 0),
                     "cholesky_decompose");
        } else {
          if (!ws_) ws_ = amd::alloc_doubles(smg_cholesky_mvn_rev_ws_doubles(n_));
          amd::check(smg_cholesky_mvn_rev(c, L_->raw_val(), n_, L_->aux_, n_, dep_ws_ + n_, dep_k_, 2LL * n_, dep_adj_,
                                          nullptr, n_, ws_),
                     "cholesky_decompose");
        }
        inverse_adjoint d;
        d.owner = this;
        d.C = ws_ + size_t(n_) * n_;
        d.s = dep_ws_ + n_;
        d.n = n_;
        d.k = dep_k_;
        d.ss = 2LL * n_;
        d.adj = dep_adj_;
        d.sweep = st->sweep_;
        if (!(A_->sink_ && A_->sink_->take_inverse_adjoint(d, nullptr))) d.expand_into(A_->adj_);
        return;
      }
      expand(dep_ws_, dep_adj_, dep_k_);
    }
    if (!deposit) record(false);
    double* work = amd::alloc_doubles(nn);
    amd::check(smg_copy_tril(c, n_, n_, L_->adj_, n_, work, n_), "cholesky_decompose");
    amd::check(smg_cholesky_rev(c, L_->raw_val(), n_, L_->aux_, work, n_, n_, A_->adj_, n_),
               "cholesky_decompose");
  }
};

inline void check_square(const char* fn, const char* name, int rows, int cols) {
  if (rows != cols) {
    std::ostringstream m;
    m << fn << ": Expecting a square matrix; rows of " << name << " (" << rows << ") and columns of "
      << name << " (" << cols << ") must match in size";
    throw std::invalid_argument(m.str());
  }
}

inline void throw_not_symmetric_dev(const char* fn, const char* name, const double* A, int n) {
  std::vector<double> h(size_t(n) * n);
  amd::to_host(h.data(), A, h.size());
  amd::throw_not_symmetric_host(fn, name, h.data(), n);
}


inline dev_var_matrix add_diag_dev(const dev_operand& A, double d, vari* d_vi, const dev_operand& dv) {
  if (dv.rows || dv.cols) {
    const size_t k = size_t(A.rows < A.cols ? A.rows : A.cols);
    if (dv.size() != k) {
      std::ostringstream m;
      m << "add_diag: number of elements of to_add has dimension = " << dv.size() << ", expecting dimension = " << k
        << "; a function was called with arguments of different scalar, array, vector, or matrix types, and they "
           "were not consistently sized;  all arguments must be scalars or multidimensional values of the same shape.";
      throw std::invalid_argument(m.str());
    }
  }
  auto* node = new add_diag_dev_vari(A, d, d_vi, dv);
  return dev_var_matrix(node->B_);
}

}

inline dev_var_matrix add_diag(const dev_var_matrix& A, const var& d) {
  return internal::add_diag_dev(internal::operand(A), d.val(), d.vi_, {});
}
inline dev_var_matrix add_diag(const dev_var_matrix& A, double d) {
  return internal::add_diag_dev(internal::operand(A), d, nullptr, {});
}
inline dev_var_matrix add_diag(const dev_data<double>& A, const var& d) {
  return internal::add_diag_dev(internal::operand(A), d.val(), d.vi_, {});
}
inline dev_var_matrix add_diag(const dev_var_matrix& A, const dev_var_matrix& d) {
  return internal::add_diag_dev(internal::operand(A), 0.0, nullptr, internal::operand(d));
}
inline dev_var_matrix add_diag(const dev_var_matrix& A, const dev_data<double>& d) {
  return internal::add_diag_dev(internal::operand(A), 0.0, nullptr, internal::operand(d));
}
inline dev_var_matrix add_diag(const dev_data<double>& A, const dev_var_matrix& d) {
  return internal::add_diag_dev(internal::operand(A), 0.0, nullptr, internal::operand(d));
}

namespace internal {
inline dev_var_matrix cholesky_decompose_impl(const dev_var_matrix& A, var* host_out,
                                              const std::function<bool()>* verify = nullptr, bool want_w = false) {
  const char* fn = "cholesky_decompose";
  internal::check_square(fn, "A", A.rows(), A.cols());
  const int n = A.rows();
  smg_ctx* c = amd::ctx();
  if (verify && !(host_out && n > 0 && smg_cholesky_stream_panels(n) <= 64)) {
    if (!(*verify)()) return dev_var_matrix();
    verify = nullptr;
  }
  if (n == 0) return dev_var_matrix(new dev_matrix_vari(0, 0, dev_structure::lower));
  auto* L = new dev_matrix_vari(n, n, dev_structure::lower);
  L->aux_ = amd::alloc_doubles(size_t(smg_cholesky_aux_doubles(n)));
  const size_t pos = ChainableStack::instance_->var_stack_.size();
  double* inv_ws = nullptr;
  want_w = want_w && !host_out && n % 512 == 0 && n >= 1024;
  if (want_w || (internal::cholesky_dev_vari::closed_form_enabled() && internal::cholesky_dev_vari::predicted(pos, n)))
    inv_ws = amd::alloc_doubles(smg_cholesky_mvn_rev_ws_doubles(n));
  int inv_started = 0;
  const int panels = smg_cholesky_stream_panels(n);
  smg_gp_source src{};
  const bool gen = A.vi_->values_pending() && A.vi_->sink_ && A.vi_->sink_->chol_source(&src);
  const double* Aval = gen ? nullptr : A.val_ptr();
  host_block b{};
  if (host_out && panels <= 64) {
    b.node = L;
    b.rows = b.cols = n;
    b.dirty = false;
    b.layout = layout_lower;
    b.n = tril_count(size_t(n));
    b.first = static_cast<vari*>(ChainableStack::instance_->memalloc_.alloc(b.n * sizeof(vari)));
    b.dummy = new vari(0.0, vari::unstacked_tag{});
    double* packed = amd::alloc_doubles(b.n);
    double* stage = static_cast<double*>(smg_host_scratch(c, b.n * sizeof(double)));
    if (!stage) throw std::bad_alloc();
    amd::phase_mark(20);
    amd::check(gen ? smg_cholesky_fwd_gp_mark_stream(c, &src, L->raw_val(), n, L->aux_, inv_ws, &inv_started, packed,
                                                     stage, 0)
                   : smg_cholesky_fwd_checked_mark_stream(c, Aval, n, n, L->raw_val(), n, L->aux_, inv_ws, &inv_started,
                                                          packed, stage, 0),
               fn);
    amd::phase_mark(0);
    if (verify && !(*verify)()) {
      amd::check(smg_sync_all(c), fn);
      int st = 0;
      amd::check(smg_status_mark_wait(c, &st), fn);
      return dev_var_matrix();
// ... 64 lines not shown
```

### math_amd/include/stan/math/rev/fun/gp_ard_cov.hpp

```cpp
#ifndef STAN_MATH_REV_FUN_GP_ARD_COV_HPP
#define STAN_MATH_REV_FUN_GP_ARD_COV_HPP


#include <stan/math/rev/fun/gp_matern_cov.hpp>

#include <cmath>
#include <sstream>
#include <stdexcept>
#include <string>
#include <vector>

namespace stan {
namespace math {

namespace internal {

class gp_ard_cov_dev_vari : public device_vari, public structured_adjoint_sink, public deferred_value_source {
 public:
  const int family_;
  const char* fn_;
  const double* x_;
  double* z_;
  double* zt_;
  const int n_;
// ... 43 lines not shown
  bool gp_source(smg_gp_source* out) override {
    if (!std::isfinite(sigma_d_)) return false;
    out->family = family_;
    out->D = D_;
    out->n = n_;
    out->x = z_;
    out->sigma = sigma_d_;
    out->l = 1.0;
    out->d = 0.0;
    return true;
  }

  bool may_write_device_adjoint(const void*) const override { return false; }

  bool wants_out() const { return sigma_vi_ || l_vis_; }
  void deposit_out() {
    if (sigma_vi_) add_pending_adjoint(sigma_vi_, out_);
    if (l_vis_)
      for (int d = 0; d < D_; ++d) add_pending_adjoint(l_vis_[d], out_ + 1 + d);
  }

  bool take_inverse_adjoint(const inverse_adjoint& d, double* dadj) override {
    if (d.n != n_) return false;
    if (dep_.C && dep_.sweep == ChainableStack::instance_->sweep_) return false;
    amd::check(smg_gp_ard_cov_inverse_adjoint(amd::ctx(), family_, d.C, n_, n_, d.s, d.k, d.ss, d.adj, zt_, D_, sigma_d_,
                                              l_d_, dadj, wants_out() ? out_ : nullptr),
               fn_);
    dep_ = d;
    return true;
  }

  void expand_adjoint() override {
    const size_t sw = ChainableStack::instance_->sweep_;
    if (exp_.C && exp_.sweep == sw) exp_.expand_into(K_->adj_);
    exp_ = inverse_adjoint{};
    if (dep_.C && dep_.sweep == sw) dep_.expand_into(K_->adj_);
    dep_ = inverse_adjoint{};
  }

  void chain() override {
    auto* st = ChainableStack::instance_;
    if (dep_.C && dep_.sweep == st->sweep_) {
      const inverse_adjoint d = dep_;
      dep_ = inverse_adjoint{};
      if (!others_write_device_adjoint(pos_, K_, d.owner)) {
        deposit_out();
        exp_ = d;
        return;
      }
      d.expand_into(K_->adj_);
    }
    if (!wants_out()) return;
    smg_ctx* c = amd::ctx();
    amd::check(smg_memset(c, out_, 0, size_t(1 + D_) * sizeof(double)), fn_);
    amd::check(smg_gp_ard_cov_rev(c, family_, zt_, D_, n_, sigma_d_, l_d_, K_->adj_, n_, out_), fn_);
    deposit_out();
  }
};

inline void gp_ard_check_hyper(const char* fn, double sigma, const std::vector<double>& l, size_t D) {
  gp_check_positive_finite(fn, "magnitude", sigma);
  for (size_t d = 0; d < l.size(); ++d) {
    const std::string name = "length scale[" + std::to_string(d + 1) + "]";
    gp_check_positive_finite(fn, name.c_str(), l[d]);
  }
  if (l.size() != D) {
    std::ostringstream m;
    m << fn << ": x dimension (" << D << ") and number of length scales (" << l.size() << ") must match in size";
    throw std::invalid_argument(m.str());
  }
  if (l.size() > size_t(SMG_GP_ARD_MAX_D)) {
    std::ostringstream m;
    m << fn << ": number of length scales (" << l.size() << ") exceeds the supported " << SMG_GP_ARD_MAX_D;
    throw std::invalid_argument(m.str());
  }
}

inline dev_var_matrix gp_ard_cov_dev(int family, const char* fn, const dev_data<double>& x, int D, double sigma,
                                     vari* sigma_vi, const std::vector<double>& l, const std::vector<vari*>& l_vis) {
  const int n = D > 0 ? int(x.size() / size_t(D)) : 0;
  auto* node = new gp_ard_cov_dev_vari(family, fn, x.data(), n, D, sigma, sigma_vi, l.data(),
                                       l_vis.empty() ? nullptr : l_vis.data());
  return dev_var_matrix(node->K_);
}

}
}
}
// ... 2 lines not shown
```

### math_amd/include/stan/math/rev/fun/gp_cross_cov.hpp

```cpp
#ifndef STAN_MATH_REV_FUN_GP_CROSS_COV_HPP
#define STAN_MATH_REV_FUN_GP_CROSS_COV_HPP


#include <stan/math/rev/fun/gp_ard_cov.hpp>

#include <cmath>
#include <sstream>
#include <stdexcept>
#include <vector>

namespace stan {
namespace math {

namespace internal {

class gp_cross_cov_dev_vari : public device_vari {
 public:
  const int family_;
  const char* fn_;
  const double* x1_;
  const double* x2_;
  const int n1_, n2_, D_;
  const double sigma_d_, l_d_;
  vari* sigma_vi_;
  vari* l_vi_;
  dev_matrix_vari* K_;
  double* out2_;

  gp_cross_cov_dev_vari(int family, const char* fn, const double* x1, int n1, const double* x2, int n2, int D,
                        double sigma, vari* sigma_vi, double l, vari* l_vi)
      : device_vari(0.0),
        family_(family),
        fn_(fn),
        x1_(x1),
        x2_(x2),
        n1_(n1),
        n2_(n2),
        D_(D),
        sigma_d_(sigma),
        l_d_(l),
        sigma_vi_(sigma_vi),
        l_vi_(l_vi),
        K_(new dev_matrix_vari(n1, n2, dev_structure::general)),
        out2_(amd::alloc_doubles(2)) {
    amd::check(smg_gp_cross_cov_fwd(amd::ctx(), family_, x1_, n1_, x2_, n2_, D_, sigma_d_, l_d_, K_->raw_val(), n1_),
               fn_);
  }

  bool may_write_device_adjoint(const void*) const override { return false; }

  void chain() override {
    if (!sigma_vi_ && !l_vi_) return;
    smg_ctx* c = amd::ctx();
    amd::check(smg_memset(c, out2_, 0, 2 * sizeof(double)), fn_);
    amd::check(smg_gp_cross_cov_rev(c, family_, x1_, n1_, x2_, n2_, D_, sigma_d_, l_d_, K_->adj_, n1_, out2_), fn_);
    if (sigma_vi_) add_pending_adjoint(sigma_vi_, out2_);
    if (l_vi_) add_pending_adjoint(l_vi_, out2_ + 1);
  }
};

class gp_ard_cross_cov_dev_vari : public device_vari {
 public:
  const int family_;
  const char* fn_;
  const int n1_, n2_, D_;
  double* z1_;
  double* z1t_;
  double* z2_;
  double* z2t_;
  const double sigma_d_;
  double* l_d_;
  vari* sigma_vi_;
  vari** l_vis_;
  dev_matrix_vari* K_;
  double* out_;

  gp_ard_cross_cov_dev_vari(int family, const char* fn, const double* x1, int n1, const double* x2, int n2, int D,
                            double sigma, vari* sigma_vi, const double* l, vari* const* l_vis)
      : device_vari(0.0),
        family_(family),
        fn_(fn),
        n1_(n1),
        n2_(n2),
        D_(D),
        z1_(amd::alloc_doubles(size_t(n1) * D)),
        z1t_(amd::alloc_doubles(size_t(n1) * D)),
        z2_(amd::alloc_doubles(size_t(n2) * D)),
        z2t_(amd::alloc_doubles(size_t(n2) * D)),
        sigma_d_(sigma),
        l_d_(ChainableStack::instance_->memalloc_.alloc_array<double>(D)),
        sigma_vi_(sigma_vi),
        l_vis_(l_vis ? ChainableStack::instance_->memalloc_.alloc_array<vari*>(D) : nullptr),
        K_(new dev_matrix_vari(n1, n2, dev_structure::general)),
        out_(amd::alloc_doubles(size_t(1 + D))) {
    for (int d = 0; d < D; ++d) {
      l_d_[d] = l[d];
      if (l_vis_) l_vis_[d] = l_vis[d];
    }
    smg_ctx* c = amd::ctx();
    amd::check(smg_gp_ard_scale(c, x1, D_, n1_, l_d_, z1_, z1t_), fn_);
    amd::check(smg_gp_ard_scale(c, x2, D_, n2_, l_d_, z2_, z2t_), fn_);
    amd::check(smg_gp_cross_cov_fwd(c, family_, z1_, n1_, z2_, n2_, D_, sigma_d_, 1.0, K_->raw_val(), n1_), fn_);
  }

  bool may_write_device_adjoint(const void*) const override { return false; }

  void chain() override {
    if (!sigma_vi_ && !l_vis_) return;
    smg_ctx* c = amd::ctx();
    amd::check(smg_memset(c, out_, 0, size_t(1 + D_) * sizeof(double)), fn_);
    amd::check(smg_gp_ard_cross_cov_rev(c, family_, z1t_, n1_, z2t_, n2_, D_, sigma_d_, l_d_, K_->adj_, n1_, out_), fn_);
    if (sigma_vi_) add_pending_adjoint(sigma_vi_, out_);
    if (l_vis_)
      for (int d = 0; d < D_; ++d) add_pending_adjoint(l_vis_[d], out_ + 1 + d);
  }
};

inline void gp_cross_throw_nan(const char* fn, const char* name) {
  std::ostringstream m;
  m << fn << ": " << name << " is nan, but must not be nan!";
  throw std::domain_error(m.str());
}
inline void gp_cross_check_not_nan(const char* fn, const char* name, const std::vector<double>& x) {
  for (size_t i = 0; i < x.size(); ++i)
    if (std::isnan(x[i])) gp_cross_throw_nan(fn, name);
}

inline void gp_cross_check_hyper(int family, const char* fn, double sigma, const vari* sigma_vi, double l,
                                 const vari* l_vi) {
  if (family != SMG_GP_EXP_QUAD) {
    gp_check_hyper(fn, sigma, l);
    return;
  }
  const bool vv = sigma_vi && l_vi, dv = !sigma_vi;
  gp_check_positive(fn, vv ? "sigma" : dv ? "marginal variance" : "magnitude", sigma);
  gp_check_positive(fn, vv ? "length_scale" : dv ? "length-scale" : "length scale", l);
}

inline dev_var_matrix gp_cross_cov_dev(int family, const char* fn, const dev_data<double>& x1,
                                       const dev_data<double>& x2, int D, double sigma, vari* sigma_vi, double l,
                                       vari* l_vi) {
  const int n1 = int(x1.size() / size_t(D)), n2 = int(x2.size() / size_t(D));
  if (n1 == 0 || n2 == 0) return dev_var_matrix(new dev_matrix_vari(n1, n2, dev_structure::general));
  auto* node = new gp_cross_cov_dev_vari(family, fn, x1.data(), n1, x2.data(), n2, D, sigma, sigma_vi, l, l_vi);
// ... 55 lines not shown
```

### math_amd/include/stan/math/rev/fun/gp_exp_quad_cov.hpp

```cpp
#ifndef STAN_MATH_REV_FUN_GP_EXP_QUAD_COV_HPP
#define STAN_MATH_REV_FUN_GP_EXP_QUAD_COV_HPP


#include <stan/math/amd/matrix.hpp>
#include <stan/math/rev/core.hpp>

#include <cmath>
#include <sstream>
#include <stdexcept>
#include <vector>

namespace stan {
namespace math {

namespace internal {
inline void gp_check_positive(const char* fn, const char* name, double v) {
  if (!(v > 0)) {
    std::ostringstream m;
    m << fn << ": " << name << " is " << v << ", but must be > 0!";
    throw std::domain_error(m.str());
  }
}

class gp_exp_quad_cov_dev_vari : public device_vari, public structured_adjoint_sink, public deferred_value_source {
// ... 44 lines not shown
    if (!std::isfinite(sigma_d_) || !std::isfinite(l_d_)) return false;
    out->family = family_;
    out->D = D_;
    out->n = n_;
    out->x = x_;
    out->sigma = sigma_d_;
    out->l = l_d_;
    out->d = 0.0;
    return true;
  }

  bool may_write_device_adjoint(const void*) const override { return false; }

  bool take_inverse_adjoint(const inverse_adjoint& d, double* dadj) override {
    if (d.n != n_) return false;
    if (dep_.C && dep_.sweep == ChainableStack::instance_->sweep_) return false;
    double* const out2 = (sigma_vi_ || l_vi_) ? out2_ : nullptr;
    if (K_->values_pending())
      amd::check(smg_gp_cov_inverse_adjoint_x(amd::ctx(), family_, d.C, n_, n_, d.s, d.k, d.ss, d.adj, x_, D_, sigma_d_,
                                              l_d_, dadj, out2),
                 fn_);
    else
      amd::check(family_ == SMG_GP_EXP_QUAD
                     ? smg_gp_inverse_adjoint(amd::ctx(), d.C, n_, n_, d.s, d.k, d.ss, d.adj, K_->raw_val(), n_, x_, D_,
                                              sigma_d_, l_d_, dadj, out2)
                     : smg_gp_cov_inverse_adjoint(amd::ctx(), family_, d.C, n_, n_, d.s, d.k, d.ss, d.adj,
                                                  K_->raw_val(), n_, x_, D_, sigma_d_, l_d_, dadj, out2),
                 fn_);
    dep_ = d;
    return true;
  }
  void expand_adjoint() override {
    const size_t sw = ChainableStack::instance_->sweep_;
    if (exp_.C && exp_.sweep == sw) exp_.expand_into(K_->adj_);
    exp_ = inverse_adjoint{};
    if (dep_.C && dep_.sweep == sw) dep_.expand_into(K_->adj_);
    dep_ = inverse_adjoint{};
  }

  void chain() override {
    auto* st = ChainableStack::instance_;
    if (dep_.C && dep_.sweep == st->sweep_) {
      const inverse_adjoint d = dep_;
      dep_ = inverse_adjoint{};
      if (!others_write_device_adjoint(pos_, K_, d.owner)) {
        if (sigma_vi_) add_pending_adjoint(sigma_vi_, out2_);
        if (l_vi_) add_pending_adjoint(l_vi_, out2_ + 1);
        exp_ = d;
        return;
      }
      d.expand_into(K_->adj_);
    }
    if (!sigma_vi_ && !l_vi_) return;
    smg_ctx* c = amd::ctx();
    amd::check(smg_memset(c, out2_, 0, 2 * sizeof(double)), fn_);
    amd::check(family_ == SMG_GP_EXP_QUAD
                   ? smg_gp_exp_quad_cov_nd_rev(c, x_, D_, n_, sigma_d_, l_d_, K_->adj_, n_, out2_)
                   : smg_gp_cov_rev(c, family_, x_, D_, n_, sigma_d_, l_d_, K_->adj_, n_, out2_),
               fn_);
    if (sigma_vi_) add_pending_adjoint(sigma_vi_, out2_);
    if (l_vi_) add_pending_adjoint(l_vi_, out2_ + 1);
  }
};

inline dev_var_matrix gp_exp_quad_cov_dev(const dev_data<double>& x, int D, double sigma, vari* sigma_vi, double l,
                                          vari* l_vi, const char* sigma_name = nullptr,
                                          const char* l_name = nullptr) {
  const char* fn = "gp_exp_quad_cov";
  gp_check_positive(fn, sigma_name ? sigma_name : sigma_vi ? "sigma" : "marginal variance", sigma);
  gp_check_positive(fn, l_name ? l_name : l_vi ? "length_scale" : "length-scale", l);
  const int n = D > 0 ? int(x.size() / size_t(D)) : 0;
  auto* node = new gp_exp_quad_cov_dev_vari(x.data(), n, D, sigma, sigma_vi, l, l_vi);
  return dev_var_matrix(node->K_);
}
inline dev_var_matrix gp_exp_quad_cov_dev(const dev_data<double>& x, double sigma, vari* sigma_vi, double l,
                                          vari* l_vi) {
  return gp_exp_quad_cov_dev(x, 1, sigma, sigma_vi, l, l_vi);
}

inline dev_data<double> gp_x_to_device(const std::vector<double>& x) {
  for (size_t i = 0; i < x.size(); ++i)
    if (std::isnan(x[i])) {
      std::ostringstream m;
      m << "gp_exp_quad_cov: x is nan, but must not be nan!";
      throw std::domain_error(m.str());
    }
  return to_dev_data(x);
}
}

inline dev_var_matrix gp_exp_quad_cov(const std::vector<double>& x, const var& sigma,
// ... 27 lines not shown
```

### math_amd/include/stan/math/rev/fun/gp_periodic_cov.hpp

```cpp
#ifndef STAN_MATH_REV_FUN_GP_PERIODIC_COV_HPP
#define STAN_MATH_REV_FUN_GP_PERIODIC_COV_HPP


#include <stan/math/rev/fun/gp_cross_cov.hpp>

#include <cmath>
#include <sstream>
#include <stdexcept>
#include <type_traits>
#include <vector>

namespace stan {
namespace math {

namespace internal {

class gp_periodic_cov_dev_vari : public device_vari {
 public:
  const char* fn_;
  const double* x1_;
  const double* x2_;
  const int n1_, n2_, D_;
  const double sigma_d_, l_d_, p_d_;
  vari* sigma_vi_;
  vari* l_vi_;
  vari* p_vi_;
  dev_matrix_vari* K_;
  double* out3_;

  gp_periodic_cov_dev_vari(const char* fn, const double* x1, int n1, const double* x2, int n2, int D, double sigma,
                           vari* sigma_vi, double l, vari* l_vi, double p, vari* p_vi, dev_structure s)
      : device_vari(0.0),
        fn_(fn),
        x1_(x1),
        x2_(x2),
        n1_(n1),
        n2_(n2),
        D_(D),
        sigma_d_(sigma),
        l_d_(l),
        p_d_(p),
        sigma_vi_(sigma_vi),
        l_vi_(l_vi),
        p_vi_(p_vi),
        K_(new dev_matrix_vari(n1, n2, s)),
        out3_(amd::alloc_doubles(3)) {
    amd::check(smg_gp_periodic_cov_fwd(amd::ctx(), x1_, n1_, x2_, n2_, D_, sigma_d_, l_d_, p_d_, K_->raw_val(), n1_),
               fn_);
  }

  bool may_write_device_adjoint(const void*) const override { return false; }

  void chain() override {
    if (!sigma_vi_ && !l_vi_ && !p_vi_) return;
    smg_ctx* c = amd::ctx();
    amd::check(smg_memset(c, out3_, 0, 3 * sizeof(double)), fn_);
    amd::check(smg_gp_periodic_cov_rev(c, x1_, n1_, x2_, n2_, D_, sigma_d_, l_d_, p_d_, K_->adj_, n1_, out3_), fn_);
    if (sigma_vi_) add_pending_adjoint(sigma_vi_, out3_);
    if (l_vi_) add_pending_adjoint(l_vi_, out3_ + 1);
    if (p_vi_) add_pending_adjoint(p_vi_, out3_ + 2);
  }
};

class gp_dot_prod_cov_dev_vari : public device_vari {
 public:
  const char* fn_;
  const int n1_, n2_;
  const double sigma_d_;
  vari* sigma_vi_;
  dev_matrix_vari* K_;
  double* out1_;

  gp_dot_prod_cov_dev_vari(const char* fn, const double* x1, int n1, const double* x2, int n2, int D, double sigma,
                           vari* sigma_vi, dev_structure s)
      : device_vari(0.0),
        fn_(fn),
        n1_(n1),
        n2_(n2),
        sigma_d_(sigma),
        sigma_vi_(sigma_vi),
        K_(new dev_matrix_vari(n1, n2, s)),
        out1_(amd::alloc_doubles(1)) {
    amd::check(smg_gp_dot_prod_cov_fwd(amd::ctx(), x1, n1_, x2, n2_, D, sigma_d_, K_->raw_val(), n1_), fn_);
  }

  bool may_write_device_adjoint(const void*) const override { return false; }

  void chain() override {
    if (!sigma_vi_) return;
    smg_ctx* c = amd::ctx();
    amd::check(smg_memset(c, out1_, 0, sizeof(double)), fn_);
    amd::check(smg_gp_dot_prod_cov_rev(c, n1_, n2_, sigma_d_, K_->adj_, n1_, out1_), fn_);
    add_pending_adjoint(sigma_vi_, out1_);
  }
};

template <typename T>
struct gp_hyper_is_var : std::is_same<std::decay_t<T>, var> {};
template <typename T>
struct gp_hyper_ok : std::integral_constant<bool, gp_hyper_is_var<T>::value || std::is_arithmetic<std::decay_t<T>>::value> {
};
inline double gp_hyper_val(const var& v) { return v.val(); }
inline double gp_hyper_val(double v) { return v; }
inline vari* gp_hyper_vi(const var& v) { return v.vi_; }
inline vari* gp_hyper_vi(double) { return nullptr; }
template <typename T_s, typename T_l, typename T_p>
using gp_periodic_kinds = std::enable_if_t<gp_hyper_ok<T_s>::value && gp_hyper_ok<T_l>::value && gp_hyper_ok<T_p>::value &&
                                           (gp_hyper_is_var<T_s>::value || gp_hyper_is_var<T_l>::value ||
                                            gp_hyper_is_var<T_p>::value)>;

struct gp_periodic_hyper {
  double sigma;
  vari* sigma_vi;
  double l;
  vari* l_vi;
  double p;
  vari* p_vi;
  void check(const char* fn) const {
    gp_check_positive(fn, "signal standard deviation", sigma);
    gp_check_positive(fn, "length-scale", l);
    gp_check_positive(fn, "period", p);
  }
};
template <typename T_s, typename T_l, typename T_p>
inline gp_periodic_hyper gp_periodic_hyper_of(const T_s& sigma, const T_l& l, const T_p& p) {
// ... 104 lines not shown
```

### math_amd/include/stan/math/rev/fun/lgamma.hpp

```cpp
#ifndef STAN_MATH_REV_FUN_LGAMMA_HPP
#define STAN_MATH_REV_FUN_LGAMMA_HPP


#include <stan/math/amd/matrix.hpp>
#include <stan/math/prim/special.hpp>
#include <stan/math/rev/core.hpp>

#include <vector>

namespace stan {
namespace math {

namespace internal {
class lgamma_vari : public op_v_vari {
 public:
  lgamma_vari(double val, vari* avi) : op_v_vari(val, avi) {}
  void chain() override { avi_->adj_ += adj_ * digamma(avi_->val_); }
};
class digamma_vari : public op_v_vari {
 public:
  digamma_vari(double val, vari* avi) : op_v_vari(val, avi) {}
  void chain() override { avi_->adj_ += adj_ * trigamma(avi_->val_); }
};

template <int OP>
class unary_special_dev_vari : public device_vari {
 public:
  dev_matrix_vari* x_;
  dev_matrix_vari* y_;
  explicit unary_special_dev_vari(dev_matrix_vari* x)
      : device_vari(0.0), x_(x), y_(new dev_matrix_vari(x->rows_, x->cols_)) {
    const long long n = (long long)x_->size();
    amd::check(OP == 0 ? smg_lgamma_fwd(amd::ctx(), x_->val(), n, y_->raw_val())
                       : smg_digamma_fwd(amd::ctx(), x_->val(), n, y_->raw_val()),
               OP == 0 ? "lgamma" : "digamma");
  }
  void chain() override {
    const long long n = (long long)x_->size();
    amd::check(OP == 0 ? smg_lgamma_rev(amd::ctx(), x_->val(), n, y_->adj_, x_->adj_)
                       : smg_digamma_rev(amd::ctx(), x_->val(), n, y_->adj_, x_->adj_),
               OP == 0 ? "lgamma" : "digamma");
  }
};
}

inline var lgamma(const var& a) {
  return var(new internal::lgamma_vari(lgamma(a.val()), a.vi_));
}
inline var digamma(const var& a) {
  return var(new internal::digamma_vari(digamma(a.val()), a.vi_));
}

inline dev_var_matrix lgamma(const dev_var_matrix& x) {
  auto* node = new internal::unary_special_dev_vari<0>(x.vi_);
  return dev_var_matrix(node->y_);
}
inline dev_var_matrix digamma(const dev_var_matrix& x) {
  auto* node = new internal::unary_special_dev_vari<1>(x.vi_);
  return dev_var_matrix(node->y_);
}
inline std::vector<var> lgamma(const std::vector<var>& x) { return to_var_vector(lgamma(to_dev(x))); }
inline std::vector<var> digamma(const std::vector<var>& x) {
  return to_var_vector(digamma(to_dev(x)));
}

}
}
#endif
```

### math_amd/include/stan/math/rev/fun/log_determinant.hpp

```cpp
#ifndef STAN_MATH_REV_FUN_LOG_DETERMINANT_HPP
#define STAN_MATH_REV_FUN_LOG_DETERMINANT_HPP


#include <stan/math/amd/matrix.hpp>
#include <stan/math/rev/core.hpp>
#include <stan/math/rev/fun/cholesky_decompose.hpp>

namespace stan {
namespace math {
namespace internal {

class log_determinant_dev_vari : public device_vari {
 public:
  dev_matrix_vari* A_;
  double* LU_;
  int* piv_;
  log_determinant_dev_vari(double v, dev_matrix_vari* A, double* LU, int* piv)
      : device_vari(v), A_(A), LU_(LU), piv_(piv) {}
  void chain() override {
    const int n = A_->rows_;
    double* ws = amd::alloc_doubles(3 * size_t(n) * n);
    int* iws = amd::alloc_ints(size_t(n));
    amd::check(smg_log_determinant_rev(amd::ctx(), LU_, piv_, n, adj_, A_->adj_, n, ws, iws), "log_determinant");
  }
};

inline double log_determinant_value(const double* A, int n, double* LU, int* piv) {
  smg_ctx* c = amd::ctx();
  double* ws = amd::alloc_doubles(size_t(64) * 64);
  double* out = amd::alloc_doubles(1);
  amd::check(smg_log_determinant_fwd(c, A, n, n, LU, piv, ws, out), "log_determinant");
  double v = 0.0;
  amd::to_host(&v, out, 1);
  return v;
}

}

inline var log_determinant(const dev_var_matrix& m) {
  internal::check_square("log_determinant", "m", m.rows(), m.cols());
  const int n = m.rows();
  if (n == 0) return var(0.0);
  double* LU = amd::alloc_doubles(size_t(n) * n);
  int* piv = amd::alloc_ints(size_t(n));
  const double v = internal::log_determinant_value(m.val_ptr(), n, LU, piv);
  return var(new internal::log_determinant_dev_vari(v, m.vi_, LU, piv));
}

inline double log_determinant(const dev_data<double>& m) {
  internal::check_square("log_determinant", "m", m.rows(), m.cols());
  const int n = m.rows();
  if (n == 0) return 0.0;
  double* LU = amd::alloc_doubles(size_t(n) * n);
  int* piv = amd::alloc_ints(size_t(n));
  return internal::log_determinant_value(m.data(), n, LU, piv);
}
// ... 5 lines not shown
```

### math_amd/include/stan/math/rev/fun/log_sum_exp.hpp

```cpp
#ifndef STAN_MATH_REV_FUN_LOG_SUM_EXP_HPP
#define STAN_MATH_REV_FUN_LOG_SUM_EXP_HPP


#include <stan/math/amd/matrix.hpp>
#include <stan/math/rev/core.hpp>

#include <vector>

namespace stan {
namespace math {

namespace internal {
class log_sum_exp_dev_vari : public device_vari {
 public:
  dev_matrix_vari* x_;
  log_sum_exp_dev_vari(double v, dev_matrix_vari* x) : device_vari(v), x_(x) {}
  void chain() override {
    amd::check(smg_log_sum_exp_rev(amd::ctx(), x_->val(), (long long)x_->size(), val_, adj_,
                                   x_->adj_),
               "log_sum_exp");
  }
};
}

inline var log_sum_exp(const dev_var_matrix& x) {
  smg_ctx* c = amd::ctx();
  double* out = amd::alloc_doubles(1);
  amd::check(smg_log_sum_exp_fwd(c, x.val_ptr(), (long long)x.size(), out), "log_sum_exp");
  double v = 0;
  amd::to_host(&v, out, 1);
  return var(new internal::log_sum_exp_dev_vari(v, x.vi_));
}

inline var log_sum_exp(const std::vector<var>& x) { return log_sum_exp(to_dev(x)); }

}
}
#endif
```

### math_amd/include/stan/math/rev/fun/mdivide_left_tri.hpp

```cpp
#ifndef STAN_MATH_REV_FUN_MDIVIDE_LEFT_TRI_HPP
#define STAN_MATH_REV_FUN_MDIVIDE_LEFT_TRI_HPP


#include <stan/math/amd/matrix.hpp>
#include <stan/math/rev/core.hpp>
#include <stan/math/rev/fun/cholesky_decompose.hpp>
#include <stan/math/rev/fun/multiply.hpp>

namespace stan {
namespace math {

namespace internal {

class mdivide_left_tri_dev_vari : public device_vari {
 public:
  const int lower_;
  dev_operand A_, B_;
  dev_matrix_vari* C_;
  const double* W_ = nullptr;
  mdivide_left_tri_dev_vari(int lower, const dev_operand& A, const dev_operand& B)
      : device_vari(0.0), lower_(lower), A_(A), B_(B), C_(new dev_matrix_vari(B.rows, B.cols)) {
    if (lower_ && B_.cols == 1 && B_.rows % 64 == 0 && A_.vi && A_.vi->sink_) W_ = A_.vi->sink_->inverse_factor();
    if (W_) {
      amd::check(smg_trmv_inv(amd::ctx(), 0, W_, A_.rows, B_.rows, B_.val(), C_->raw_val()), "mdivide_left_tri");
      return;
    }
    amd::check(smg_mdivide_left_tri_aux_fwd(amd::ctx(), lower_, A_.val(), A_.rows, aux(), B_.val(), B_.rows,
                                            B_.rows, B_.cols, C_->raw_val(), C_->rows_),
               "mdivide_left_tri");
  }
  const double* aux() const { return lower_ && A_.vi ? A_.vi->aux_ : nullptr; }
  void chain() override {
    const int m = B_.rows, n = B_.cols;
    double* ws = amd::alloc_doubles(size_t(m) * n);
    if (W_) {
      smg_ctx* c = amd::ctx();
      amd::check(smg_trmv_inv(c, 1, W_, A_.rows, m, C_->adj_, ws), "mdivide_left_tri");
      if (A_.adj()) amd::check(smg_rank1_lower(c, m, -1.0, ws, C_->raw_val(), A_.adj(), A_.rows), "mdivide_left_tri");
      if (B_.adj()) amd::check(smg_axpy(c, (long long)m, 1.0, ws, 1, B_.adj(), 1), "mdivide_left_tri");
      return;
    }
    amd::check(smg_mdivide_left_tri_aux_rev(amd::ctx(), lower_, A_.val(), A_.rows, aux(), C_->raw_val(), m,
                                            C_->adj_, m, m, n, A_.adj(), A_.rows, B_.adj(), m, ws),
               "mdivide_left_tri");
  }
};

template <int TriView>
inline dev_var_matrix mdivide_left_tri_dev(const dev_operand& A, const dev_operand& B) {
  static_assert(TriView == 1 || TriView == 2, "TriView must be Eigen::Lower or Eigen::Upper");
  check_square("mdivide_left_tri", "A", A.rows, A.cols);
  check_multiplicable("mdivide_left_tri", A.rows, A.cols, B.rows, B.cols, "A", "b");
  auto* node = new mdivide_left_tri_dev_vari(TriView == 1 ? 1 : 0, A, B);
  return dev_var_matrix(node->C_);
}

inline dev_data<double> dev_identity(int n) {
  double* I = amd::alloc_doubles(size_t(n) * n);
  smg_ctx* c = amd::ctx();
  amd::check(smg_memset(c, I, 0, size_t(n) * n * sizeof(double)), "mdivide_left_tri");
  amd::check(smg_add_diag_fwd(c, I, n, n, 1.0, nullptr, I, n), "mdivide_left_tri");
  return dev_data<double>(I, size_t(n) * n, n, n);
}

}

template <int TriView>
inline dev_var_matrix mdivide_left_tri(const dev_var_matrix& A, const dev_var_matrix& B) {
  return internal::mdivide_left_tri_dev<TriView>(internal::operand(A), internal::operand(B));
}
template <int TriView>
inline dev_var_matrix mdivide_left_tri(const dev_data<double>& A, const dev_var_matrix& B) {
  return internal::mdivide_left_tri_dev<TriView>(internal::operand(A), internal::operand(B));
}
template <int TriView>
inline dev_var_matrix mdivide_left_tri(const dev_var_matrix& A, const dev_data<double>& B) {
// ... 13 lines not shown
```

### math_amd/include/stan/math/rev/fun/multi_normal_cholesky_lpdf.hpp

```cpp
#ifndef STAN_MATH_REV_FUN_MULTI_NORMAL_CHOLESKY_LPDF_HPP
#define STAN_MATH_REV_FUN_MULTI_NORMAL_CHOLESKY_LPDF_HPP


#include <stan/math/amd/matrix.hpp>
#include <stan/math/rev/core.hpp>
#include <stan/math/rev/fun/multiply.hpp>

#include <cmath>
#include <sstream>
#include <stdexcept>
#include <vector>

namespace stan {
namespace math {

namespace internal {

class mvn_cholesky_dev_vari : public device_vari {
 public:
  dev_matrix_vari* L_;
  const double* ws_;
  int n_;
  dev_matrix_vari* y_;
  dev_matrix_vari* mu_;

  bool deposited_ = false;

  mvn_cholesky_dev_vari(double lp, dev_matrix_vari* L, const double* ws,
                        dev_matrix_vari* y = nullptr, dev_matrix_vari* mu = nullptr)
      : device_vari(lp), L_(L), ws_(ws), n_(L->rows_), y_(y), mu_(mu) {}

  bool may_write_device_adjoint(const void* node) const override {
    return (node == L_ && !deposited_) || (y_ && node == y_) || (mu_ && node == mu_);
  }

  void chain() override {
    const int lower_only = L_->structure_ == dev_structure::lower ? 1 : 0;
    deposited_ = lower_only && L_->sink_ && L_->sink_->take_mvn_adjoint(this, ws_, adj_);
    amd::check(smg_mvn_cholesky_rev(amd::ctx(), L_->val(), n_, L_->aux_, n_, ws_, adj_, lower_only,
                                    y_ ? y_->adj_ : nullptr, mu_ ? mu_->adj_ : nullptr,
                                    deposited_ ? nullptr : L_->adj_, n_),
               "multi_normal_cholesky_lpdf");
  }
};

inline void mvn_check_sizes(int ny, int nmu, const dev_var_matrix& L) {
  const char* fn = "multi_normal_cholesky_lpdf";
  auto mismatch = [&](const char* a, int x, const char* b, int y) {
    std::ostringstream m;
    m << fn << ": " << a << " (" << x << ") and " << b << " (" << y << ") must match in size";
    throw std::invalid_argument(m.str());
  };
  if (ny != nmu) mismatch("Size of random variable", ny, "size of location parameter", nmu);
  if (ny != L.rows()) mismatch("Size of random variable", ny, "rows of covariance parameter", L.rows());
  if (ny != L.cols()) mismatch("Size of random variable", ny, "columns of covariance parameter", L.cols());
}

inline void mvn_check_data(const std::vector<double>& y, const std::vector<double>* mu) {
  const char* fn = "multi_normal_cholesky_lpdf";
  if (mu)
    for (size_t i = 0; i < mu->size(); ++i)
      if (!std::isfinite((*mu)[i])) {
        std::ostringstream m;
        m << fn << ": Location parameter[" << i + 1 << "] is " << (*mu)[i] << ", but must be finite!";
        throw std::domain_error(m.str());
      }
  for (size_t i = 0; i < y.size(); ++i)
    if (std::isnan(y[i])) {
      std::ostringstream m;
      m << fn << ": Random variable[" << i + 1 << "] is nan, but must not be nan!";
      throw std::domain_error(m.str());
    }
}

// ... 56 lines not shown
    return false;
  }
  void chain() override {
    smg_ctx* c = amd::ctx();
    deposited_ = lower_only_ && L_.vi && L_.vi->sink_ && L_.vi->sink_->take_mvn_adjoint(this, ws_, adj_, k_);
    for (int i = 0; i < k_; ++i)
      amd::check(smg_mvn_cholesky_rev(c, L_.val(), n_, aux_, n_, ws_ + 2 * size_t(n_) * i, adj_, lower_only_,
                                      obs_[i].yadj, obs_[i].muadj, deposited_ ? nullptr : L_.adj(), n_),
                 "multi_normal_cholesky_lpdf");
  }
};

inline vari* mvn_cholesky_multi(const dev_operand& L, const double* aux, bool lower_only, mvn_obs* obs, int k,
                                bool include_const, bool include_logdet, double host_logdet, double* lp_out) {
  const char* fn = "multi_normal_cholesky_lpdf";
  const int n = L.rows;
  smg_ctx* c = amd::ctx();
  double* ws = amd::alloc_doubles(2 * size_t(n) * size_t(k) + size_t(k));
  double* lp_d = ws + 2 * size_t(n) * size_t(k);
  const double* W = lower_only && L.vi && L.vi->sink_ ? L.vi->sink_->inverse_factor() : nullptr;
  for (int i = 0; i < k; ++i)
    amd::check(W ? smg_mvn_cholesky_fwd_inv(c, obs[i].y, obs[i].mu, L.val(), n, W, n, n, ws + 2 * size_t(n) * i,
                                            lp_d + i)
                 : smg_mvn_cholesky_fwd(c, obs[i].y, obs[i].mu, L.val(), n, aux, n, ws + 2 * size_t(n) * i, lp_d + i),
               fn);
  if (lower_only && L.vi && L.vi->sink_) L.vi->sink_->prepare_mvn_adjoint();
  std::vector<double> lps(static_cast<size_t>(k));
  amd::to_host(lps.data(), lp_d, lps.size());
  double lp = 0.0;
  for (double v : lps) lp += v;
  if (!include_const) lp -= -std::log(std::sqrt(2.0 * 3.14159265358979323846)) * n * k;
  if (!include_logdet) lp -= host_logdet * k;
  *lp_out = lp;
  bool any_adj = L.adj() != nullptr;
  for (int i = 0; i < k; ++i) any_adj = any_adj || obs[i].yadj || obs[i].muadj;
  if (!any_adj) return nullptr;
  return new mvn_multi_dev_vari(lp, L, aux, lower_only ? 1 : 0, ws, obs, k);
}

}

template <bool propto = false>
inline var multi_normal_cholesky_lpdf(const std::vector<double>& y, const std::vector<double>& mu,
                                      const dev_var_matrix& L) {
  internal::mvn_check_sizes(int(y.size()), int(mu.size()), L);
  internal::mvn_check_data(y, &mu);
  if (y.empty()) return var(0.0);
  dev_data<double> yd = to_dev_data(y), md = to_dev_data(mu);
  return internal::mvn_cholesky_dev<propto>(yd.data(), md.data(), int(y.size()), L);
}

template <bool propto = false>
inline var multi_normal_cholesky_lpdf(const dev_data<double>& y, const dev_var_matrix& L) {
  internal::mvn_check_sizes(int(y.size()), int(y.size()), L);
  return internal::mvn_cholesky_dev<propto>(y.data(), nullptr, int(y.size()), L);
}
template <bool propto = false>
inline var multi_normal_cholesky_lpdf(const dev_data<double>& y, const dev_data<double>& mu,
                                      const dev_var_matrix& L) {
  internal::mvn_check_sizes(int(y.size()), int(mu.size()), L);
  return internal::mvn_cholesky_dev<propto>(y.data(), mu.data(), int(y.size()), L);
}

template <bool propto = false>
inline var multi_normal_cholesky_lpdf(const dev_var_matrix& y, const dev_var_matrix& mu,
                                      const dev_var_matrix& L) {
  internal::mvn_check_sizes(int(y.size()), int(mu.size()), L);
// ... 15 lines not shown
```

### math_amd/include/stan/math/rev/fun/multiply.hpp

```cpp
#ifndef STAN_MATH_REV_FUN_MULTIPLY_HPP
#define STAN_MATH_REV_FUN_MULTIPLY_HPP


#include <stan/math/amd/matrix.hpp>
#include <stan/math/rev/core.hpp>

#include <sstream>
#include <stdexcept>

namespace stan {
namespace math {

namespace internal {

inline void check_positive_size(const char* fn, const char* name, const char* expr, int size) {
  if (size <= 0) {
    std::ostringstream m;
    m << fn << ": " << name << " must have a positive size, but is " << size << "; dimension size expression = "
      << expr;
    throw std::invalid_argument(m.str());
  }
}

inline void check_multiplicable(const char* fn, int a_rows, int a_cols, int b_rows, int b_cols,
// ... 10 lines not shown
}

class multiply_dev_vari : public device_vari {
 public:
  dev_operand A_, B_;
  dev_matrix_vari* C_;
  bool gram_;
  bool lowvec_;
  multiply_dev_vari(const dev_operand& A, const dev_operand& B)
      : device_vari(0.0), A_(A), B_(B), C_(new dev_matrix_vari(A.rows, B.cols)),
        gram_(A.vi && B.vi && B.vi->transpose_of_ == A.vi),
        lowvec_(A.vi && A.vi->structure_ == dev_structure::lower && A.rows == A.cols && B.cols == 1 &&
                A.rows % 64 == 0) {
    smg_ctx* c = amd::ctx();
    if (lowvec_) {
      amd::check(smg_trmv_inv(c, 0, A_.val(), A_.rows, A_.rows, B_.val(), C_->raw_val()), "multiply");
      return;
    }
    if (gram_) {
      amd::check(smg_gemm(c, 0, 1, 1, A_.rows, A_.rows, A_.cols, 1.0, A_.val(), A_.rows, A_.val(), A_.rows, 0.0,
                          C_->raw_val(), C_->rows_),
                 "multiply");
      amd::check(smg_sym_from_lower(c, C_->rows_, C_->raw_val(), C_->rows_), "multiply");
      return;
    }
    amd::check(smg_multiply_fwd(c, A_.val(), A_.rows, B_.val(), B_.rows, A_.rows, A_.cols, B_.cols, C_->raw_val(),
                                C_->rows_),
               "multiply");
  }
  void chain() override {
    smg_ctx* c = amd::ctx();
    if (lowvec_) {
      const int m = A_.rows;
      if (A_.adj()) amd::check(smg_rank1_lower(c, m, 1.0, C_->adj_, B_.val(), A_.adj(), m), "multiply");
      if (B_.adj()) {
        double* t = amd::alloc_doubles(size_t(m));
        amd::check(smg_trmv_inv(c, 1, A_.val(), A_.rows, m, C_->adj_, t), "multiply");
        amd::check(smg_axpy(c, (long long)m, 1.0, t, 1, B_.adj(), 1), "multiply");
      }
      return;
    }
    if (gram_) {
      const int m = C_->rows_;
      double* S = amd::alloc_doubles(size_t(m) * m);
      amd::check(smg_memcpy_d2d(c, S, C_->adj_, size_t(m) * m * sizeof(double)), "multiply");
      amd::check(smg_transpose(c, m, m, C_->adj_, m, S, m, 1.0), "multiply");
      amd::check(smg_gemm(c, 0, 0, 0, m, A_.cols, m, 1.0, S, m, A_.val(), A_.rows, 1.0, A_.adj(), A_.rows),
                 "multiply");
      return;
    }
    amd::check(smg_multiply_rev(c, A_.val(), A_.rows, B_.val(), B_.rows, C_->adj_, C_->rows_, A_.rows, A_.cols,
                                B_.cols, A_.adj(), A_.rows, B_.adj(), B_.rows),
               "multiply");
  }
};

class scale_dev_vari : public device_vari {
 public:
  dev_operand A_;
  double c_;
  vari* c_vi_;
  double* cadj_;
  dev_matrix_vari* B_;
  scale_dev_vari(const dev_operand& A, double c, vari* c_vi)
      : device_vari(0.0), A_(A), c_(c), c_vi_(c_vi), cadj_(c_vi ? amd::alloc_doubles(1) : nullptr),
        B_(new dev_matrix_vari(A.rows, A.cols)) {
    smg_ctx* x = amd::ctx();
    const long long n = (long long)A.rows * A.cols;
    amd::check(smg_memset(x, B_->raw_val(), 0, size_t(n) * sizeof(double)), "multiply");
    amd::check(smg_axpy(x, n, c_, A_.val(), 1, B_->raw_val(), 1), "multiply");
  }
  void chain() override {
    smg_ctx* x = amd::ctx();
    const long long n = (long long)A_.rows * A_.cols;
    if (A_.adj()) amd::check(smg_axpy(x, n, c_, B_->adj_, 1, A_.adj(), 1), "multiply");
    if (c_vi_) {
      amd::check(smg_memset(x, cadj_, 0, sizeof(double)), "multiply");
      amd::check(smg_dot(x, B_->adj_, A_.val(), n, cadj_), "multiply");
      add_pending_adjoint(c_vi_, cadj_);
    }
  }
};

class transpose_dev_vari : public device_vari {
 public:
  dev_matrix_vari* A_;
  dev_matrix_vari* B_;
  explicit transpose_dev_vari(dev_matrix_vari* A)
      : device_vari(0.0), A_(A), B_(new dev_matrix_vari(A->cols_, A->rows_)) {
    B_->transpose_of_ = A;
    amd::check(smg_transpose(amd::ctx(), A_->rows_, A_->cols_, A_->val(), A_->rows_, B_->raw_val(),
                             B_->rows_, 0.0),
               "transpose");
  }
  void chain() override {
    amd::check(smg_transpose(amd::ctx(), B_->rows_, B_->cols_, B_->adj_, B_->rows_, A_->adj_,
                             A_->rows_, 1.0),
               "transpose");
  }
};

class sum_dev_vari : public device_vari {
 public:
  dev_matrix_vari* A_;
  sum_dev_vari(double v, dev_matrix_vari* A) : device_vari(v), A_(A) {}
  void chain() override {
    const int uplo = A_->structure_ == dev_structure::lower ? 1 : 0;
    amd::check(smg_shift(amd::ctx(), A_->rows_, A_->cols_, adj_, A_->adj_, A_->rows_, uplo), "sum");
  }
};

class sum_v_vari : public host_local_vari {
 public:
  vari** v_;
  size_t n_;
  sum_v_vari(double s, vari** v, size_t n) : host_local_vari(s), v_(v), n_(n) {}
  void chain() override {
    for (size_t i = 0; i < n_; ++i) v_[i]->adj_ += adj_;
  }
  bool touches_adjoints_in(const vari* lo, const vari* hi) const override {
    for (size_t i = 0; i < n_; ++i)
      if (v_[i] >= lo && v_[i] < hi) return true;
    return false;
  }
};

inline dev_var_matrix multiply_dev(const dev_operand& A, const dev_operand& B) {
  check_multiplicable("multiply", A.rows, A.cols, B.rows, B.cols);
  auto* node = new multiply_dev_vari(A, B);
  return dev_var_matrix(node->C_);
}

}

inline dev_var_matrix multiply(const dev_var_matrix& A, const dev_var_matrix& B) {
  return internal::multiply_dev(internal::operand(A), internal::operand(B));
}
inline dev_var_matrix multiply(const dev_var_matrix& A, const dev_data<double>& B) {
  return internal::multiply_dev(internal::operand(A), internal::operand(B));
}
inline dev_var_matrix multiply(const dev_data<double>& A, const dev_var_matrix& B) {
// ... 53 lines not shown
```

### math_amd/include/stan/math/rev/fun/normal_id_glm_lpdf.hpp

```cpp
#ifndef STAN_MATH_REV_FUN_NORMAL_ID_GLM_LPDF_HPP
#define STAN_MATH_REV_FUN_NORMAL_ID_GLM_LPDF_HPP


#include <stan/math/rev/fun/bernoulli_logit_glm_lpmf.hpp>

#include <algorithm>
#include <cmath>
#include <sstream>
#include <stdexcept>
#include <string>
#include <vector>

namespace stan {
namespace math {
namespace internal {

class glm_sigma_dev_vari : public local_adjoint_vari {
 public:
  vari* alpha_vi_;
  vari** beta_vi_;
  dev_matrix_vari* beta_dev_;
  vari* sigma_vi_;
  double* g_;
  const double* g_dev_;
  int M_;
  glm_sigma_dev_vari(double lp, vari* a, vari** b, dev_matrix_vari* bd, vari* s, double* g,
                     const double* gd, int M)
      : local_adjoint_vari(lp), alpha_vi_(a), beta_vi_(b), beta_dev_(bd), sigma_vi_(s), g_(g), g_dev_(gd), M_(M) {}
  bool touches_adjoints_in(const vari* lo, const vari* hi) const override {
    auto in = [&](const vari* v) { return v && v >= lo && v < hi; };
    if (in(alpha_vi_) || in(sigma_vi_)) return true;
    if (beta_vi_)
      for (int j = 0; j < M_; ++j)
        if (in(beta_vi_[j])) return true;
    return false;
  }
  void chain() override {
    if (alpha_vi_) alpha_vi_->adj_ += adj_ * g_[0];
    if (beta_vi_)
      for (int j = 0; j < M_; ++j) beta_vi_[j]->adj_ += adj_ * g_[1 + j];
    if (beta_dev_)
      amd::check(smg_axpy(amd::ctx(), M_, adj_, g_dev_, 1, beta_dev_->adj_, 1), "normal_id_glm_lpdf");
    if (sigma_vi_) sigma_vi_->adj_ += adj_ * g_[M_ + 1];
  }
};

inline void glm_throw_nonfinite_y(const char* fn, const double* y, long long n, long long row0 = 0) {
  std::vector<double> h(size_t(n > 0 ? n : 0));
  for (long long i0 = 0; i0 < n; i0 += 1 << 20) {
    const long long c = std::min<long long>(1 << 20, n - i0);
    amd::to_host(h.data() + i0, y + i0, size_t(c));
  }
  for (long long i = 0; i < n; ++i)
    if (!std::isfinite(h[size_t(i)])) {
      std::ostringstream m;
      m << fn << ": Vector of dependent variables[" << row0 + i + 1 << "] is " << h[size_t(i)]
        << ", but must be finite!";
      throw std::domain_error(m.str());
    }
}

inline void normal_glm_check_scale(double sigma) {
  static const char* fn = "normal_id_glm_lpdf";
  if (!(sigma > 0)) {
    std::ostringstream m;
    m << fn << ": Scale vector is " << sigma << ", but must be > 0!";
    throw std::domain_error(m.str());
  }
  if (!std::isfinite(sigma)) {
    std::ostringstream m;
    m << fn << ": Scale vector is " << sigma << ", but must be finite!";
    throw std::domain_error(m.str());
  }
}

// ... 142 lines not shown
```

### math_amd/include/stan/math/rev/fun/spd_functors.hpp

```cpp
#ifndef STAN_MATH_REV_FUN_SPD_FUNCTORS_HPP
#define STAN_MATH_REV_FUN_SPD_FUNCTORS_HPP


#include <stan/math/amd/matrix.hpp>
#include <stan/math/rev/core.hpp>
#include <stan/math/rev/fun/cholesky_decompose.hpp>
#include <stan/math/rev/fun/multiply.hpp>

#include <cmath>
#include <sstream>
#include <stdexcept>
#include <string>

namespace stan {
namespace math {
namespace internal {

inline void check_multiplicable_named(const char* fn, const char* n1, int c1, const char* n2, int r2) {
  if (c1 != r2) {
    std::ostringstream m;
    m << fn << ": Columns of " << n1 << " (" << c1 << ") and Rows of " << n2 << " (" << r2
      << ") must match in size";
    throw std::invalid_argument(m.str());
  }
// ... 6 lines not shown
  amd::check(smg_status(c, &st), fn);
  if (st & SMG_ERR_NOT_SYMMETRIC) throw_not_symmetric_dev(fn, name, A, n);
  if (st) amd::throw_status(st, fn, name);
}

class mdivide_left_spd_dev_vari : public device_vari {
 public:
  dev_operand A_, B_;
  double* L_;
  double* aux_;
  dev_matrix_vari* C_;
  mdivide_left_spd_dev_vari(const dev_operand& A, const dev_operand& B)
      : device_vari(0.0), A_(A), B_(B), C_(new dev_matrix_vari(B.rows, B.cols)) {
    static const char* fn = "mdivide_left_spd";
    const int m = A.rows;
    smg_ctx* c = amd::ctx();
    L_ = amd::alloc_doubles(size_t(m) * m);
    aux_ = amd::alloc_doubles(size_t(smg_cholesky_aux_doubles(m)));
    amd::check(smg_mdivide_left_spd_fwd(c, A_.val(), m, B_.val(), m, m, B_.cols, L_, aux_, C_->raw_val(), m),
               fn);
    int st = 0;
    amd::check(smg_status(c, &st), fn);
    if (st & SMG_ERR_NOT_PD) {
      std::ostringstream msg;
      msg << fn << ": A is not positive definite.";
      throw std::domain_error(msg.str());
    }
    if (st) amd::throw_status(st, fn, "A");
  }
  void chain() override {
    const int m = B_.rows, n = B_.cols;
    if (!A_.adj() && !B_.adj()) return;
    double* ws = amd::alloc_doubles(size_t(m) * n);
    amd::check(smg_mdivide_left_spd_rev(amd::ctx(), L_, aux_, m, n, C_->raw_val(), m, C_->adj_, m, A_.adj(), m,
                                        B_.adj(), m, ws),
               "mdivide_left_spd");
  }
};

inline dev_var_matrix mdivide_left_spd_dev(const dev_operand& A, const dev_operand& B) {
  check_square("mdivide_left_spd", "A", A.rows, A.cols);
  check_multiplicable_named("mdivide_left_spd", "A", A.cols, "b", B.rows);
  auto* node = new mdivide_left_spd_dev_vari(A, B);
  return dev_var_matrix(node->C_);
}

class log_determinant_spd_dev_vari : public device_vari {
 public:
  dev_matrix_vari* A_;
  double* L_;
  double* aux_;
  log_determinant_spd_dev_vari(double v, dev_matrix_vari* A, double* L, double* aux)
      : device_vari(v), A_(A), L_(L), aux_(aux) {}
  void chain() override {
    const int n = A_->rows_;
    double* ws = amd::alloc_doubles(size_t(n) * n);
    amd::check(smg_log_determinant_spd_rev(amd::ctx(), L_, aux_, n, adj_, A_->adj_, n, ws),
               "log_determinant_spd");
  }
};

class mlt_self_transpose_dev_vari : public device_vari {
 public:
  dev_matrix_vari* L_;
  dev_matrix_vari* C_;
  explicit mlt_self_transpose_dev_vari(dev_matrix_vari* L)
      : device_vari(0.0), L_(L), C_(new dev_matrix_vari(L->rows_, L->rows_)) {
    const int K = L->rows_, J = L->cols_;
    double* ws = amd::alloc_doubles(size_t(K) * (J > 0 ? J : 1));
    amd::check(smg_multiply_lower_tri_self_transpose_fwd(amd::ctx(), L_->val(), K, K, J, C_->raw_val(), K, ws),
               "multiply_lower_tri_self_transpose");
  }
  void chain() override {
    const int K = L_->rows_, J = L_->cols_;
    double* ws = amd::alloc_doubles(size_t(2) * K * J + size_t(K) * K);
    amd::check(smg_multiply_lower_tri_self_transpose_rev(amd::ctx(), L_->val(), K, K, J, C_->adj_, K,
                                                         L_->adj_, K, ws),
               "multiply_lower_tri_self_transpose");
  }
};

class quad_form_sym_dev_vari : public device_vari {
 public:
  dev_operand A_, B_;
  dev_matrix_vari* C_;
  const int sym_adj_;
  quad_form_sym_dev_vari(const dev_operand& A, const dev_operand& B)
      : device_vari(0.0), A_(A), B_(B), C_(new dev_matrix_vari(B.cols, B.cols)),
        sym_adj_(A.vi && B.vi ? 1 : 0) {
    const int M = B.rows, N = B.cols;
    double* ws = amd::alloc_doubles(size_t(M) * N + size_t(N) * N);
    amd::check(smg_quad_form_sym_fwd(amd::ctx(), A_.val(), M, B_.val(), M, M, N, C_->raw_val(), N, ws),
               "quad_form_sym");
  }
  void chain() override {
    const int M = B_.rows, N = B_.cols;
    if (!A_.adj() && !B_.adj()) return;
    double* ws = amd::alloc_doubles(size_t(M) * N + size_t(N) * N);
    amd::check(smg_quad_form_sym_rev(amd::ctx(), A_.val(), M, B_.val(), M, M, N, C_->adj_, N, sym_adj_,
                                     A_.adj(), M, B_.adj(), M, ws),
               "quad_form_sym");
  }
};

inline dev_var_matrix quad_form_sym_dev(const dev_operand& A, const dev_operand& B) {
  static const char* fn = "quad_form_sym";
  check_square(fn, "A", A.rows, A.cols);
  if (A.vi && B.vi) {
    check_multiplicable_named(fn, "A", A.cols, "B", B.rows);
    check_symmetric_dev(fn, "A", A.val(), A.rows);
  } else {
    check_symmetric_dev(fn, "A", A.val(), A.rows);
    check_multiplicable_named(fn, "A", A.cols, "B", B.rows);
  }
  auto* node = new quad_form_sym_dev_vari(A, B);
  return dev_var_matrix(node->C_);
}

}

inline dev_var_matrix mdivide_left_spd(const dev_var_matrix& A, const dev_var_matrix& b) {
  return internal::mdivide_left_spd_dev(internal::operand(A), internal::operand(b));
}
inline dev_var_matrix mdivide_left_spd(const dev_data<double>& A, const dev_var_matrix& b) {
  return internal::mdivide_left_spd_dev(internal::operand(A), internal::operand(b));
}
inline dev_var_matrix mdivide_left_spd(const dev_var_matrix& A, const dev_data<double>& b) {
  return internal::mdivide_left_spd_dev(internal::operand(A), internal::operand(b));
}

inline var log_determinant_spd(const dev_var_matrix& m) {
  static const char* fn = "log_determinant_spd";
// ... 44 lines not shown
```

### math_amd/include/stan/math/rev/fun/tangent_ops.hpp

```cpp
#ifndef STAN_MATH_REV_FUN_TANGENT_OPS_HPP
#define STAN_MATH_REV_FUN_TANGENT_OPS_HPP


#include <stan/math/amd/matrix.hpp>
#include <stan/math/rev/core.hpp>

namespace stan {
namespace math {

namespace internal {

class gp_tangent_dev_vari : public device_vari {
 public:
  const double* x_;
  int n_;
  double s_, l_, ds_, dl_;
  vari* vis_[4];
  dev_matrix_vari* K_;
  double* out4_;
  gp_tangent_dev_vari(const double* x, int n, const var& s, const var& l, const var& ds,
                      const var& dl)
      : device_vari(0.0), x_(x), n_(n), s_(s.val()), l_(l.val()), ds_(ds.val()), dl_(dl.val()),
        vis_{s.vi_, l.vi_, ds.vi_, dl.vi_}, K_(new dev_matrix_vari(n, n)),
        out4_(amd::alloc_doubles(4)) {
    amd::check(smg_gp_exp_quad_cov_tangent_fwd(amd::ctx(), x_, n_, s_, l_, ds_, dl_, K_->raw_val(), n_),
               "gp_exp_quad_cov");
  }
  void chain() override {
    smg_ctx* c = amd::ctx();
    amd::check(smg_memset(c, out4_, 0, 4 * sizeof(double)), "gp_exp_quad_cov");
    amd::check(smg_gp_exp_quad_cov_tangent_rev(c, x_, n_, s_, l_, ds_, dl_, K_->adj_, n_, out4_),
               "gp_exp_quad_cov");
    for (int i = 0; i < 4; ++i)
      if (vis_[i]) add_pending_adjoint(vis_[i], out4_ + i);
  }
};

class phi_dev_vari : public device_vari {
 public:
  dev_matrix_vari* X_;
  dev_matrix_vari* Y_;
  explicit phi_dev_vari(dev_matrix_vari* X)
      : device_vari(0.0), X_(X), Y_(new dev_matrix_vari(X->rows_, X->cols_, dev_structure::lower)) {
    amd::check(smg_phi(amd::ctx(), X_->rows_, X_->val(), X_->rows_, Y_->raw_val(), Y_->rows_, 0), "phi");
  }
  void chain() override {
    amd::check(smg_phi(amd::ctx(), X_->rows_, Y_->adj_, Y_->rows_, X_->adj_, X_->rows_, 1), "phi");
  }
};

class dot_dev_vari : public device_vari {
 public:
  dev_matrix_vari* x_;
  dev_matrix_vari* y_;
  dot_dev_vari(double v, dev_matrix_vari* x, dev_matrix_vari* y) : device_vari(v), x_(x), y_(y) {}
  void chain() override {
    smg_ctx* c = amd::ctx();
    const long long n = (long long)x_->size();
    amd::check(smg_axpy(c, n, adj_, y_->val(), 1, x_->adj_, 1), "dot_product");
    amd::check(smg_axpy(c, n, adj_, x_->val(), 1, y_->adj_, 1), "dot_product");
  }
};

class diag_ratio_dev_vari : public device_vari {
 public:
  dev_matrix_vari* A_;
  dev_matrix_vari* B_;
  diag_ratio_dev_vari(double v, dev_matrix_vari* A, dev_matrix_vari* B) : device_vari(v), A_(A), B_(B) {}
  void chain() override {
    amd::check(smg_diag_ratio_rev(amd::ctx(), A_->rows_, A_->val(), A_->rows_, B_->val(), B_->rows_,
                                  adj_, A_->adj_, A_->rows_, B_->adj_, B_->rows_),
               "diag_ratio_sum");
  }
};

}

inline dev_var_matrix gp_exp_quad_cov_tangent(const dev_data<double>& x, const var& sigma,
                                              const var& l, const var& dsigma, const var& dl) {
  auto* node = new internal::gp_tangent_dev_vari(x.data(), int(x.size()), sigma, l, dsigma, dl);
  return dev_var_matrix(node->K_);
}

inline dev_var_matrix phi_lower(const dev_var_matrix& X) {
  auto* node = new internal::phi_dev_vari(X.vi_);
  return dev_var_matrix(node->Y_);
}

inline var dot_product(const dev_var_matrix& x, const dev_var_matrix& y) {
  if (x.size() != y.size()) throw std::invalid_argument("dot_product: size mismatch");
  smg_ctx* c = amd::ctx();
  double* out = amd::alloc_doubles(1);
  amd::check(smg_memset(c, out, 0, sizeof(double)), "dot_product");
  amd::check(smg_dot(c, x.val_ptr(), y.val_ptr(), (long long)x.size(), out), "dot_product");
  double v = 0;
  amd::to_host(&v, out, 1);
  return var(new internal::dot_dev_vari(v, x.vi_, y.vi_));
}

inline var diag_ratio_sum(const dev_var_matrix& A, const dev_var_matrix& B) {
  smg_ctx* c = amd::ctx();
  double* out = amd::alloc_doubles(1);
  amd::check(smg_memset(c, out, 0, sizeof(double)), "diag_ratio_sum");
  amd::check(smg_diag_ratio_fwd(c, A.rows(), A.val_ptr(), A.rows(), B.val_ptr(), B.rows(), out),
// ... 10 lines not shown
```

### math_amd/include/stan/math/rev/functor/gradient.hpp

```cpp
#ifndef STAN_MATH_REV_FUNCTOR_GRADIENT_HPP
#define STAN_MATH_REV_FUNCTOR_GRADIENT_HPP


#include <stan/math/amd/matrix.hpp>
#include <stan/math/rev/core.hpp>

#include <type_traits>
#include <vector>

namespace stan {
namespace math {

namespace internal {
template <typename Vec>
struct var_vector_of;
template <>
struct var_vector_of<std::vector<double>> {
  using type = std::vector<var>;
};
}

template <typename F, typename Vec>
void gradient(const F& f, const Vec& x, double& fx, Vec& grad_fx) {
  using VarVec = typename internal::var_vector_of<Vec>::type;
  start_nested();
  no_publish_scope quiet;
  try {
    VarVec x_var(x.size());
    for (size_t i = 0; i < size_t(x.size()); ++i) x_var[i] = var(new vari(x[i], false));
    var fx_var = f(x_var);
    fx = fx_var.val();
    grad(fx_var.vi_);
    grad_fx.resize(x.size());
    for (size_t i = 0; i < size_t(x.size()); ++i) grad_fx[i] = x_var[i].adj();
  } catch (const std::exception& e) {
    recover_memory_nested();
    throw;
  }
  recover_memory_nested();
}

template <typename F>
void gradient(const F& f, const dev_data<double>& x, double& fx, double* grad_dev) {
  start_nested();
  no_publish_scope quiet;
  try {
    smg_ctx* c = amd::ctx();
    auto* leaf = new dev_matrix_vari(x.rows(), x.cols());
    const size_t n = leaf->size();
    amd::check(smg_memcpy_d2d(c, leaf->raw_val(), x.data(), n * sizeof(double)), "gradient");
    var fx_var = f(dev_var_matrix(leaf));
    fx = fx_var.val();
    grad(fx_var.vi_);
    amd::check(smg_memcpy_d2d(c, grad_dev, leaf->adj_, n * sizeof(double)), "gradient");
  } catch (const std::exception& e) {
    recover_memory_nested();
    throw;
  }
  recover_memory_nested();
}

}
}
#endif
```

### math_amd/include/stan/math/rev/meta/operands_and_partials.hpp

```cpp
#ifndef STAN_MATH_REV_META_OPERANDS_AND_PARTIALS_HPP
#define STAN_MATH_REV_META_OPERANDS_AND_PARTIALS_HPP


#include <stan/math/amd/matrix.hpp>
#include <stan/math/rev/core.hpp>

#include <type_traits>
#include <vector>

namespace stan {
namespace math {

namespace internal {

template <typename T>
class broadcast_array {
  T& prim_;

 public:
  explicit broadcast_array(T& prim) : prim_(prim) {}
  T& operator[](int) { return prim_; }
  template <typename Y>
  void operator=(const Y& m) {
    prim_ = m[0];
// ... 192 lines not shown
      : partials_(amd::alloc_doubles(op.size())), operand_(op) {
    amd::zero(partials_, op.size());
  }
  void set_partials(const double* host) { amd::to_device(partials_, host, operand_.size()); }
  int size() const { return 0; }
  void dump_operands(vari**) const {}
  void dump_partials(double*) const {}
  dev_edge device() const { return dev_edge{operand_.vi_, partials_}; }

 private:
  const dev_var_matrix& operand_;
};

class ops_partials_vari : public local_adjoint_vari {
 public:
  size_t size_;
  vari** varis_;
  double* partials_;
  dev_edge dev_[5];
  int ndev_;
  ops_partials_vari(double v, size_t size, vari** varis, double* partials, const dev_edge* dev, int ndev)
      : local_adjoint_vari(v), size_(size), varis_(varis), partials_(partials), ndev_(ndev) {
    for (int i = 0; i < ndev; ++i) dev_[i] = dev[i];
  }
  bool touches_adjoints_in(const vari* lo, const vari* hi) const override {
    for (size_t i = 0; i < size_; ++i)
      if (varis_[i] >= lo && varis_[i] < hi) return true;
    return false;
  }
  void chain() override {
    for (size_t i = 0; i < size_; ++i) varis_[i]->adj_ += adj_ * partials_[i];
    for (int i = 0; i < ndev_; ++i)
      amd::check(smg_axpy(amd::ctx(), (long long)dev_[i].op->size(), adj_, dev_[i].partials, 1,
                          dev_[i].op->adj_, 1),
                 "operands_and_partials");
  }
};

template <typename... Ops>
struct ops_return {
  using type = typename std::conditional<(op_is_var<Ops>::value || ...), var, double>::type;
};

}

template <typename Op1 = double, typename Op2 = double, typename Op3 = double, typename Op4 = double,
          typename Op5 = double,
          typename T_return_type = typename internal::ops_return<Op1, Op2, Op3, Op4, Op5>::type>
class operands_and_partials;

template <typename Op1, typename Op2, typename Op3, typename Op4, typename Op5>
class operands_and_partials<Op1, Op2, Op3, Op4, Op5, double> {
 public:
  internal::ops_partials_edge<double, Op1> edge1_;
  internal::ops_partials_edge<double, Op2> edge2_;
  internal::ops_partials_edge<double, Op3> edge3_;
  internal::ops_partials_edge<double, Op4> edge4_;
  internal::ops_partials_edge<double, Op5> edge5_;
  explicit operands_and_partials(const Op1&) {}
  operands_and_partials(const Op1&, const Op2&) {}
  operands_and_partials(const Op1&, const Op2&, const Op3&) {}
  operands_and_partials(const Op1&, const Op2&, const Op3&, const Op4&) {}
  operands_and_partials(const Op1&, const Op2&, const Op3&, const Op4&, const Op5&) {}
  double build(double value) const { return value; }
};

template <typename Op1, typename Op2, typename Op3, typename Op4, typename Op5>
// ... 50 lines not shown
```

Measured before the change: 473.2 gradient evals/s.

## Defer zeroing of large device adjoints until first access

Large device adjoint buffers are no longer memset when a matrix vari is created. Each buffer is registered with a cleared flag and zeroed lazily the first time its adjoint is accessed or declared wanted by a consumer. Structured operands such as add_diag inputs and the lower Cholesky factor with a sink skip the eager request, so the large N×N adjoints they never accumulate into may never be zeroed. A zeroed-bytes counter is added for inspection. The risk is correctness if some code path writes an adjoint without going through the accessor.

```diff
diff --git a/include/smg_hip.h b/include/smg_hip.h
--- a/include/smg_hip.h
+++ b/include/smg_hip.h
@@ -69,6 +69,7 @@
 int smg_profile_enable(smg_ctx* ctx, int on);
 int smg_profile_read(smg_ctx* ctx, int family, double* total_ms_host, long long* count_host);
 int smg_profile_flops(smg_ctx* ctx, int family, double* flops_host);
+unsigned long long smg_zeroed_bytes(const smg_ctx* ctx);
 
 int smg_fill_unif(smg_ctx* ctx, double* out, long long n, unsigned long long seed,
                   double a, double b, double scale);
diff --git a/math_amd/csrc/ctx.hip b/math_amd/csrc/ctx.hip
--- a/math_amd/csrc/ctx.hip
+++ b/math_amd/csrc/ctx.hip
@@ -546,6 +546,7 @@
   for (int i = 0; i < count; ++i) {
     const size_t b = r[i].second;
     if (!b) continue;
+    ctx->zeroed_bytes += b;
     if ((reinterpret_cast<uintptr_t>(r[i].first) & 7) || (b & 7)) {
       SMG_HIP_TRY(hipMemsetAsync(r[i].first, 0, b, stream));
       continue;
@@ -754,8 +755,11 @@
     ctx->prof_count[i] = 0;
     ctx->prof_flops[i] = 0;
   }
-  return SMG_OK;
-}
+  ctx->zeroed_bytes = 0;
+  return SMG_OK;
+}
+
+unsigned long long smg_zeroed_bytes(const smg_ctx* ctx) { return ctx ? ctx->zeroed_bytes : 0; }
 
 int smg_profile_read(smg_ctx* ctx, int family, double* ms, long long* count) {
   if (family < 0 || family >= SMG_FAM_COUNT) return SMG_ERR_ARG;
diff --git a/math_amd/csrc/smg_internal.h b/math_amd/csrc/smg_internal.h
--- a/math_amd/csrc/smg_internal.h
+++ b/math_amd/csrc/smg_internal.h
@@ -79,6 +79,7 @@
   double prof_ms[SMG_FAM_COUNT];
   double prof_flops[SMG_FAM_COUNT];
   long long prof_count[SMG_FAM_COUNT];
+  unsigned long long zeroed_bytes;
   void* comm;
 };
 
diff --git a/math_amd/hip.py b/math_amd/hip.py
--- a/math_amd/hip.py
+++ b/math_amd/hip.py
@@ -55,6 +55,7 @@
     "smg_profile_enable": (_I, [_P, _I]),
     "smg_profile_read": (_I, [_P, _I, ctypes.POINTER(_D), ctypes.POINTER(_L)]),
     "smg_profile_flops": (_I, [_P, _I, ctypes.POINTER(_D)]),
+    "smg_zeroed_bytes": (ctypes.c_ulonglong, [_P]),
     "smg_fill_unif": (_I, [_P, _P, _L, ctypes.c_ulonglong, _D, _D, _D]),
     "smg_fill_bernoulli": (_I, [_P, _P, _L, ctypes.c_ulonglong, _D]),
     "smg_gemm": (_I, [_P, _I, _I, _I, _I, _I, _I, _D, _P, _I, _P, _I, _D, _P, _I]),
diff --git a/math_amd/include/stan/math/amd/matrix.hpp b/math_amd/include/stan/math/amd/matrix.hpp
--- a/math_amd/include/stan/math/amd/matrix.hpp
+++ b/math_amd/include/stan/math/amd/matrix.hpp
@@ -62,6 +62,7 @@
   }
   virtual void prepare_mvn_adjoint() {}
   virtual void expand_adjoint() {}
+  virtual void expect_dense_adjoint() {}
   virtual const double* inverse_factor() { return nullptr; }
   virtual bool gp_source(smg_gp_source* out) {
     (void)out;
@@ -99,11 +100,12 @@
 class dev_matrix_vari {
   double* val_;
   deferred_value_source* pending_ = nullptr;
+  double* adj_;
+  size_t adj_slot_;
 
  public:
   const int rows_;
   const int cols_;
-  double* adj_;
   dev_structure structure_;
   double* aux_;
   dev_matrix_vari* transpose_of_ = nullptr;
@@ -111,15 +113,20 @@
 
   dev_matrix_vari(int rows, int cols, dev_structure s = dev_structure::general)
       : val_(amd::alloc_doubles(size_t(rows) * cols)),
+        adj_(amd::alloc_doubles(size_t(rows) * cols)),
+        adj_slot_(register_device_adjoint(adj_, size_t(rows) * cols)),
         rows_(rows),
         cols_(cols),
-        adj_(amd::alloc_doubles(size_t(rows) * cols)),
         structure_(s),
-        aux_(nullptr) {
-    register_device_adjoint(adj_, size_t(rows) * cols);
-  }
+        aux_(nullptr) {}
 
   size_t size() const { return size_t(rows_) * cols_; }
+
+  double* adj() {
+    clear_device_adjoint(adj_slot_, true);
+    return adj_;
+  }
+  void want_adjoint() { clear_device_adjoint(adj_slot_, false); }
 
   const double* val() {
     if (pending_) force_values();
@@ -153,7 +160,7 @@
   int cols() const { return vi_->cols_; }
   size_t size() const { return vi_->size(); }
   const double* val_ptr() const { return vi_->val(); }
-  double* adj_ptr() const { return vi_->adj_; }
+  double* adj_ptr() const { return vi_->adj(); }
 
   std::vector<double> val() const {
     std::vector<double> h(size());
@@ -162,9 +169,10 @@
   }
   std::vector<double> adj() const {
     if (vi_->sink_) vi_->sink_->expand_adjoint();
+    const double* a = vi_->adj();
     join_device_adjoints();
     std::vector<double> h(size());
-    amd::to_host(h.data(), vi_->adj_, size());
+    amd::to_host(h.data(), a, size());
     return h;
   }
 
@@ -208,10 +216,16 @@
   const double* data = nullptr;
   int rows = 0, cols = 0;
   const double* val() const { return vi ? vi->val() : data; }
-  double* adj() const { return vi ? vi->adj_ : nullptr; }
+  double* adj() const { return vi ? vi->adj() : nullptr; }
   size_t size() const { return size_t(rows) * size_t(cols); }
 };
-inline dev_operand operand(const dev_var_matrix& m) { return dev_operand{m.vi_, nullptr, m.rows(), m.cols()}; }
+inline dev_operand operand(const dev_var_matrix& m) {
+  m.vi_->want_adjoint();
+  return dev_operand{m.vi_, nullptr, m.rows(), m.cols()};
+}
+inline dev_operand structured_operand(const dev_var_matrix& m) {
+  return dev_operand{m.vi_, nullptr, m.rows(), m.cols()};
+}
 inline dev_operand operand(const dev_data<double>& d) { return dev_operand{nullptr, d.data(), d.rows(), d.cols()}; }
 }
 
@@ -379,9 +393,9 @@
     amd::check(smg_memcpy_h2d(c, dst, stage, b.n * sizeof(double)), "to_host");
     const int mode = block_pack_mode(b.layout);
     if (mode < 0)
-      amd::check(smg_axpy(c, (long long)b.n, 1.0, dst, 1, node->adj_, 1), "to_host");
+      amd::check(smg_axpy(c, (long long)b.n, 1.0, dst, 1, node->adj(), 1), "to_host");
     else
-      amd::check(smg_unpack_tril_add(c, mode, mode == 2 ? int(b.n) : b.rows, dst, node->adj_, b.rows), "to_host");
+      amd::check(smg_unpack_tril_add(c, mode, mode == 2 ? int(b.n) : b.rows, dst, node->adj(), b.rows), "to_host");
     amd::check(smg_sync(c), "to_host");
   }
 };
@@ -390,7 +404,6 @@
   auto* st = ChainableStack::instance_;
   if (from >= st->host_blocks_.size() || !amd::has_ctx()) return;
   smg_ctx* c = amd::ctx();
-  join_device_adjoints();
   const size_t nb = st->host_blocks_.size();
   std::vector<size_t> off(nb + 1, 0);
   for (size_t k = from; k < nb; ++k) {
@@ -405,13 +418,14 @@
     if (!b.n) continue;
     auto* node = static_cast<dev_matrix_vari*>(b.node);
     if (node->sink_) node->sink_->expand_adjoint();
-    const double* src = node->adj_;
+    const double* src = node->adj();
+    join_device_adjoints();
     const int mode = block_pack_mode(b.layout);
     const size_t cnt = off[k + 1] - off[k];
     if (mode >= 0) {
       double* t = amd::alloc_doubles(cnt);
-      amd::check(smg_pack_tril(c, mode, mode == 2 ? int(b.n) : b.rows, node->adj_, b.rows, t), "grad");
-      if (b.layout == layout_lower) amd::check(smg_sum_strict_upper(c, b.rows, node->adj_, b.rows, t + b.n), "grad");
+      amd::check(smg_pack_tril(c, mode, mode == 2 ? int(b.n) : b.rows, src, b.rows, t), "grad");
+      if (b.layout == layout_lower) amd::check(smg_sum_strict_upper(c, b.rows, src, b.rows, t + b.n), "grad");
       src = t;
     }
     amd::check(smg_memcpy_d2h(c, stage + off[k], src, cnt * sizeof(double)), "grad");
@@ -534,7 +548,7 @@
     amd::check(smg_status_armed(c, &armed), "to_dev");
     double* h = static_cast<double*>(smg_host_scratch(c, (n + 1) * sizeof(double)));
     if (!h) throw std::bad_alloc();
-    amd::check(smg_memcpy_d2h(c, h, dst_->adj_, n * sizeof(double)), "to_dev");
+    amd::check(smg_memcpy_d2h(c, h, dst_->adj(), n * sizeof(double)), "to_dev");
     if (armed) amd::check(smg_status_enqueue(c, reinterpret_cast<int*>(h + n)), "to_dev");
     amd::check(smg_sync(c), "to_dev");
     if (armed) amd::throw_if_sync(*reinterpret_cast<int*>(h + n), "to_dev", "a persistent solve");
diff --git a/math_amd/include/stan/math/eigen/interop.hpp b/math_amd/include/stan/math/eigen/interop.hpp
--- a/math_amd/include/stan/math/eigen/interop.hpp
+++ b/math_amd/include/stan/math/eigen/interop.hpp
@@ -134,8 +134,8 @@
       if (std::isnan(e.dd[i])) throw_not_nan(nan_fn, nan_name, i);
   return e;
 }
-inline dev_operand commit(const eig_in& e) {
-  if (e.node) return operand(dev_var_matrix(e.node));
+inline dev_operand commit(const eig_in& e, bool structured = false) {
+  if (e.node) return structured ? structured_operand(dev_var_matrix(e.node)) : operand(dev_var_matrix(e.node));
   if (e.vd) return operand(to_dev_vars(e.vd, e.n, e.rows, e.cols));
   return operand(to_dev_data(e.dd, e.n, e.rows, e.cols));
 }
@@ -288,7 +288,7 @@
                                       internal::any_var<T_m, T_a>::value>>
 inline matrix_v add_diag(const Eigen::Matrix<T_m, Eigen::Dynamic, Eigen::Dynamic>& mat, const T_a& to_add) {
   const internal::eig_in em = internal::prepare(mat);
-  const internal::dev_operand a = internal::commit(em);
+  const internal::dev_operand a = internal::commit(em, true);
   if constexpr (internal::is_var<T_a>::value)
     return internal::add_diag_output(mat, em, internal::add_diag_dev(a, to_add.val(), to_add.vi_, {}));
   else
@@ -309,7 +309,7 @@
   }
   const internal::eig_in em = internal::prepare(mat);
   const internal::eig_in ed = internal::prepare(to_add);
-  const internal::dev_operand a = internal::commit(em);
+  const internal::dev_operand a = internal::commit(em, true);
   internal::dev_operand d = internal::commit(ed);
   d.rows = int(d.size());
   d.cols = 1;
@@ -593,7 +593,7 @@
   mvt_dev<var> out;
   for (size_t i = 0; i < p.size(); ++i) {
     out.val.push_back(node->val() + i * size_t(n));
-    out.adj.push_back(node->adj_ + i * size_t(n));
+    out.adj.push_back(node->adj() + i * size_t(n));
   }
   return out;
 }
@@ -662,12 +662,12 @@
   bool lower_only = false;
   double host_logdet = 0.0;
   if constexpr (std::is_same<T_covar, dev_var_matrix>::value) {
-    Ld = internal::operand(L);
     aux = L.vi_->aux_;
     lower_only = L.vi_->structure_ == dev_structure::lower;
+    Ld = lower_only && L.vi_->sink_ ? internal::structured_operand(L) : internal::operand(L);
   } else {
     const internal::eig_in eL = internal::prepare(L);
-    Ld = internal::commit(eL);
+    Ld = internal::commit(eL, eL.node && eL.node->structure_ == dev_structure::lower && eL.node->sink_);
     if (Ld.vi) {
       aux = Ld.vi->aux_;
       lower_only = Ld.vi->structure_ == dev_structure::lower;
diff --git a/math_amd/include/stan/math/mix/fvar_functors.hpp b/math_amd/include/stan/math/mix/fvar_functors.hpp
--- a/math_amd/include/stan/math/mix/fvar_functors.hpp
+++ b/math_amd/include/stan/math/mix/fvar_functors.hpp
@@ -54,14 +54,16 @@
   dev_matrix_vari* C_;
   multiply_lower_dev_vari(dev_matrix_vari* A, dev_matrix_vari* B)
       : device_vari(0.0), A_(A), B_(B), C_(new dev_matrix_vari(A->rows_, B->cols_, dev_structure::lower)) {
+    A->want_adjoint();
+    B->want_adjoint();
     const int n = A->rows_;
     amd::check(smg_multiply_lower_fwd(amd::ctx(), A_->val(), n, B_->val(), n, n, C_->raw_val(), n), "multiply");
   }
   void chain() override {
     const int n = A_->rows_;
     double* ws = amd::alloc_doubles(size_t(n) * n);
-    amd::check(smg_multiply_lower_rev(amd::ctx(), A_->val(), n, B_->val(), n, C_->adj_, n, n, A_->adj_, n,
-                                      B_->adj_, n, ws),
+    amd::check(smg_multiply_lower_rev(amd::ctx(), A_->val(), n, B_->val(), n, C_->adj(), n, n, A_->adj(), n,
+                                      B_->adj(), n, ws),
                "multiply");
   }
 };
@@ -75,14 +77,16 @@
   dev_matrix_vari* C_;
   add_dev_vari(dev_matrix_vari* A, dev_matrix_vari* B)
       : device_vari(0.0), A_(A), B_(B), C_(new dev_matrix_vari(A->rows_, A->cols_)) {
+    A->want_adjoint();
+    B->want_adjoint();
     smg_ctx* c = amd::ctx();
     amd::check(smg_copy_matrix(c, A->rows_, A->cols_, A->val(), A->rows_, C_->raw_val(), C_->rows_, 0, 0), "add");
     amd::check(smg_axpy(c, (long long)C_->size(), 1.0, B->val(), 1, C_->raw_val(), 1), "add");
   }
   void chain() override {
     smg_ctx* c = amd::ctx();
-    amd::check(smg_axpy(c, (long long)C_->size(), 1.0, C_->adj_, 1, A_->adj_, 1), "add");
-    amd::check(smg_axpy(c, (long long)C_->size(), 1.0, C_->adj_, 1, B_->adj_, 1), "add");
+    amd::check(smg_axpy(c, (long long)C_->size(), 1.0, C_->adj(), 1, A_->adj(), 1), "add");
+    amd::check(smg_axpy(c, (long long)C_->size(), 1.0, C_->adj(), 1, B_->adj(), 1), "add");
   }
 };
 
@@ -92,12 +96,13 @@
   dev_matrix_vari* C_;
   explicit tril_dev_vari(dev_matrix_vari* A)
       : device_vari(0.0), A_(A), C_(new dev_matrix_vari(A->rows_, A->cols_, dev_structure::lower)) {
+    A->want_adjoint();
     smg_ctx* c = amd::ctx();
     amd::zero(C_->raw_val(), C_->size());
     amd::check(smg_add_tril(c, A->rows_, A->cols_, 1.0, A->val(), A->rows_, C_->raw_val(), C_->rows_), "tril");
   }
   void chain() override {
-    amd::check(smg_add_tril(amd::ctx(), A_->rows_, A_->cols_, 1.0, C_->adj_, C_->rows_, A_->adj_, A_->rows_),
+    amd::check(smg_add_tril(amd::ctx(), A_->rows_, A_->cols_, 1.0, C_->adj(), C_->rows_, A_->adj(), A_->rows_),
                "tril");
   }
 };
@@ -108,10 +113,13 @@
   dev_matrix_vari* xd_;
   double lse_;
   lse_tangent_dev_vari(double t, double lse, dev_matrix_vari* x, dev_matrix_vari* xd)
-      : device_vari(t), x_(x), xd_(xd), lse_(lse) {}
+      : device_vari(t), x_(x), xd_(xd), lse_(lse) {
+    x->want_adjoint();
+    xd->want_adjoint();
+  }
   void chain() override {
     amd::check(smg_lse_tangent_rev(amd::ctx(), x_->val(), xd_->val(), (long long)x_->size(), lse_, val_, adj_,
-                                   x_->adj_, xd_->adj_),
+                                   x_->adj(), xd_->adj()),
                "log_sum_exp");
   }
 };
@@ -128,10 +136,13 @@
   glm_tangent_dev_vari(double t, dev_matrix_vari* eta, dev_matrix_vari* etad, vari* alpha, vari* alphad, double a,
                        double ad, const int* y)
       : device_vari(t), eta_(eta), etad_(etad), alpha_(alpha), alphad_(alphad), a_(a), ad_(ad), y_(y),
-        out2_(amd::alloc_doubles(2)) {}
+        out2_(amd::alloc_doubles(2)) {
+    eta->want_adjoint();
+    etad->want_adjoint();
+  }
   void chain() override {
     amd::check(smg_glm_tangent_rev(amd::ctx(), eta_->val(), a_, etad_->val(), ad_, y_, (long long)eta_->size(), adj_,
-                                   eta_->adj_, etad_->adj_, out2_),
+                                   eta_->adj(), etad_->adj(), out2_),
                "bernoulli_logit_glm_lpmf");
     if (alpha_) add_pending_adjoint(alpha_, out2_);
     if (alphad_) add_pending_adjoint(alphad_, out2_ + 1);
@@ -275,6 +286,8 @@
   double* P_;
   chol_tangent_dev_vari(dev_matrix_vari* L, dev_matrix_vari* Ad)
       : device_vari(0.0), L_(L), Ad_(Ad), Ld_(new dev_matrix_vari(L->rows_, L->cols_, dev_structure::lower)) {
+    L->want_adjoint();
+    Ad->want_adjoint();
     const int n = L->rows_;
     const size_t nn = size_t(n) * n;
     Wt_ = amd::alloc_doubles(nn);
@@ -294,8 +307,8 @@
   void chain() override {
     const int n = L_->rows_;
     double* ws = amd::alloc_doubles(2 * size_t(n) * n);
-    amd::check(smg_chol_tangent_rev(amd::ctx(), L_->val(), n, W_, Wt_, Y_, P_, n, Ld_->adj_, n, n, L_->adj_, n,
-                                    Ad_->adj_, n, ws),
+    amd::check(smg_chol_tangent_rev(amd::ctx(), L_->val(), n, W_, Wt_, Y_, P_, n, Ld_->adj(), n, n, L_->adj(), n,
+                                    Ad_->adj(), n, ws),
                "cholesky_decompose");
   }
 };
@@ -311,6 +324,7 @@
 inline dev_fvar_matrix cholesky_decompose(const dev_fvar_matrix& A) {
   dev_fvar_matrix L;
   if (!internal::chol_tangent_composed()) {
+    A.d_.vi_->want_adjoint();
     L.val_ = internal::cholesky_decompose_with_inverse(A.val_);
     L.d_ = dev_var_matrix((new internal::chol_tangent_dev_vari(L.val_.vi_, A.d_.vi_))->Ld_);
     return L;
diff --git a/math_amd/include/stan/math/rev/core/autodiffstackstorage.hpp b/math_amd/include/stan/math/rev/core/autodiffstackstorage.hpp
--- a/math_amd/include/stan/math/rev/core/autodiffstackstorage.hpp
+++ b/math_amd/include/stan/math/rev/core/autodiffstackstorage.hpp
@@ -16,6 +16,7 @@
 struct dev_buffer {
   double* ptr;
   size_t n;
+  bool cleared;
 };
 struct pending_adjoint {
   vari* target;
@@ -65,6 +66,7 @@
     std::vector<size_t> block_order_;
     size_t block_order_sweep_ = 0;
     size_t sweep_ = 0;
+    bool dev_clear_queued_ = false;
     void (*publish_)(size_t from) = nullptr;
     int no_publish_ = 0;
   };
diff --git a/math_amd/include/stan/math/rev/core/grad.hpp b/math_amd/include/stan/math/rev/core/grad.hpp
--- a/math_amd/include/stan/math/rev/core/grad.hpp
+++ b/math_amd/include/stan/math/rev/core/grad.hpp
@@ -14,16 +14,33 @@
 namespace stan {
 namespace math {
 
-inline void register_device_adjoint(double* p, size_t n) {
-  if (n >= (size_t(1) << 17))
-    amd::check(smg_memset_async(amd::ctx(), p, n * sizeof(double)), "zero");
-  else
-    amd::zero(p, n);
-  ChainableStack::instance_->dev_adj_stack_.push_back({p, n});
+inline size_t register_device_adjoint(double* p, size_t n) {
+  const bool large = n >= (size_t(1) << 17);
+  if (!large) amd::zero(p, n);
+  auto& s = ChainableStack::instance_->dev_adj_stack_;
+  s.push_back({p, n, !large});
+  return s.size() - 1;
 }
 
 inline void join_device_adjoints() {
   if (amd::has_ctx()) amd::check(smg_join_async(amd::ctx()), "grad");
+  ChainableStack::instance_->dev_clear_queued_ = false;
+}
+
+inline void clear_device_adjoint(size_t slot, bool now) {
+  auto* st = ChainableStack::instance_;
+  dev_buffer& b = st->dev_adj_stack_[slot];
+  if (b.cleared) {
+    if (now && st->dev_clear_queued_) join_device_adjoints();
+    return;
+  }
+  b.cleared = true;
+  if (now) {
+    amd::zero(b.ptr, b.n);
+  } else {
+    amd::check(smg_memset_async(amd::ctx(), b.ptr, b.n * sizeof(double)), "zero");
+    st->dev_clear_queued_ = true;
+  }
 }
 
 inline void add_pending_adjoint(vari* target, const double* src) {
@@ -195,7 +212,10 @@
   ++st->sweep_;
   for (auto* v : st->var_stack_) v->set_zero_adjoint();
   for (auto* v : st->var_nochain_stack_) v->set_zero_adjoint();
-  for (auto& b : st->dev_adj_stack_) amd::zero(b.ptr, b.n);
+  for (auto& b : st->dev_adj_stack_) {
+    amd::zero(b.ptr, b.n);
+    b.cleared = true;
+  }
   zero_host_blocks(0);
   st->pending_.clear();
 }
@@ -212,8 +232,10 @@
   const size_t s2 = st->nested_var_nochain_stack_sizes_.back();
   for (size_t i = (s2 == 0U) ? 0U : (s2 - 1); i < st->var_nochain_stack_.size(); ++i)
     st->var_nochain_stack_[i]->set_zero_adjoint();
-  for (size_t i = st->nested_dev_adj_sizes_.back(); i < st->dev_adj_stack_.size(); ++i)
+  for (size_t i = st->nested_dev_adj_sizes_.back(); i < st->dev_adj_stack_.size(); ++i) {
     amd::zero(st->dev_adj_stack_[i].ptr, st->dev_adj_stack_[i].n);
+    st->dev_adj_stack_[i].cleared = true;
+  }
   zero_host_blocks(st->nested_host_block_sizes_.back());
   st->pending_.clear();
 }
diff --git a/math_amd/include/stan/math/rev/fun/bernoulli_logit_glm_lpmf.hpp b/math_amd/include/stan/math/rev/fun/bernoulli_logit_glm_lpmf.hpp
--- a/math_amd/include/stan/math/rev/fun/bernoulli_logit_glm_lpmf.hpp
+++ b/math_amd/include/stan/math/rev/fun/bernoulli_logit_glm_lpmf.hpp
@@ -59,7 +59,7 @@
     if (beta_vi_)
       for (int j = 0; j < M_; ++j) beta_vi_[j]->adj_ += adj_ * g_[1 + j];
     if (beta_dev_)
-      amd::check(smg_axpy(amd::ctx(), M_, adj_, g_dev_, 1, beta_dev_->adj_, 1),
+      amd::check(smg_axpy(amd::ctx(), M_, adj_, g_dev_, 1, beta_dev_->adj(), 1),
                  "bernoulli_logit_glm_lpmf");
   }
 };
diff --git a/math_amd/include/stan/math/rev/fun/cholesky_decompose.hpp b/math_amd/include/stan/math/rev/fun/cholesky_decompose.hpp
--- a/math_amd/include/stan/math/rev/fun/cholesky_decompose.hpp
+++ b/math_amd/include/stan/math/rev/fun/cholesky_decompose.hpp
@@ -35,6 +35,7 @@
         dadj_(d_vi ? amd::alloc_doubles(1) : nullptr), dv_(dv),
         pos_(ChainableStack::instance_->var_stack_.size() - 1), d_(d), src_{} {
     if (A.rows == A.cols && !dv.rows) B_->sink_ = this;
+    if (A_.vi && !(B_->sink_ == this && A_.vi->sink_)) A_.vi->want_adjoint();
     if (amd::deferred_values_enabled() && B_->sink_ == this && A.rows > 0 && A_.vi && A_.vi->sink_ &&
         std::isfinite(d) && A_.vi->sink_->gp_source(&src_) && src_.n == A.rows) {
       src_.d = d;
@@ -63,6 +64,11 @@
   bool may_write_device_adjoint(const void* node) const override {
     return (A_.vi && node == A_.vi) || (dv_.vi && node == dv_.vi);
   }
+  void expect_dense_adjoint() override {
+    if (!A_.vi) return;
+    A_.vi->want_adjoint();
+    if (A_.vi->sink_) A_.vi->sink_->expect_dense_adjoint();
+  }
   bool take_inverse_adjoint(const inverse_adjoint& d, double*) override {
     if (B_->sink_ != this) return false;
     if (dep_.C && dep_.sweep == ChainableStack::instance_->sweep_) return false;
@@ -71,9 +77,9 @@
   }
   void expand_adjoint() override {
     const size_t sw = ChainableStack::instance_->sweep_;
-    if (exp_.C && exp_.sweep == sw) exp_.expand_into(B_->adj_);
+    if (exp_.C && exp_.sweep == sw) exp_.expand_into(B_->adj());
     exp_ = inverse_adjoint{};
-    if (dep_.C && dep_.sweep == sw) dep_.expand_into(B_->adj_);
+    if (dep_.C && dep_.sweep == sw) dep_.expand_into(B_->adj());
     dep_ = inverse_adjoint{};
   }
 
@@ -100,17 +106,17 @@
         exp_ = d;
         return;
       }
-      d.expand_into(B_->adj_);
+      d.expand_into(B_->adj());
     }
     double* dadj = dv_.rows ? dv_.adj() : dadj_;
     if (dadj_) amd::check(smg_memset(c, dadj_, 0, sizeof(double)), "add_diag");
     const int vec = dv_.rows ? 1 : 0;
     if (m == n) {
-      amd::check(smg_add_diag_rev(c, B_->adj_, m, m, A_.adj(), m, dadj, vec), "add_diag");
+      amd::check(smg_add_diag_rev(c, B_->adj(), m, m, A_.adj(), m, dadj, vec), "add_diag");
     } else {
       if (A_.adj())
-        amd::check(smg_axpy(c, (long long)m * n, 1.0, B_->adj_, 1, A_.adj(), 1), "add_diag");
-      amd::check(smg_add_diag_rev(c, B_->adj_, m, k, nullptr, 0, dadj, vec), "add_diag");
+        amd::check(smg_axpy(c, (long long)m * n, 1.0, B_->adj(), 1, A_.adj(), 1), "add_diag");
+      amd::check(smg_add_diag_rev(c, B_->adj(), m, k, nullptr, 0, dadj, vec), "add_diag");
     }
     if (d_vi_) add_pending_adjoint(d_vi_, dadj_);
   }
@@ -139,7 +145,7 @@
   void expand(const double* ws, double adj, int k) const {
     for (int o = 0; o < k; ++o)
       amd::check(smg_mvn_cholesky_rev(amd::ctx(), L_->raw_val(), n_, L_->aux_, n_, ws + 2 * size_t(n_) * o, adj, 1, nullptr,
-                                      nullptr, L_->adj_, n_),
+                                      nullptr, L_->adj(), n_),
                  "cholesky_decompose");
   }
 
@@ -255,15 +261,15 @@
         d.ss = 2LL * n_;
         d.adj = dep_adj_;
         d.sweep = st->sweep_;
-        if (!(A_->sink_ && A_->sink_->take_inverse_adjoint(d, nullptr))) d.expand_into(A_->adj_);
+        if (!(A_->sink_ && A_->sink_->take_inverse_adjoint(d, nullptr))) d.expand_into(A_->adj());
         return;
       }
       expand(dep_ws_, dep_adj_, dep_k_);
     }
     if (!deposit) record(false);
     double* work = amd::alloc_doubles(nn);
-    amd::check(smg_copy_tril(c, n_, n_, L_->adj_, n_, work, n_), "cholesky_decompose");
-    amd::check(smg_cholesky_rev(c, L_->raw_val(), n_, L_->aux_, work, n_, n_, A_->adj_, n_),
+    amd::check(smg_copy_tril(c, n_, n_, L_->adj(), n_, work, n_), "cholesky_decompose");
+    amd::check(smg_cholesky_rev(c, L_->raw_val(), n_, L_->aux_, work, n_, n_, A_->adj(), n_),
                "cholesky_decompose");
   }
 };
@@ -302,10 +308,10 @@
 }
 
 inline dev_var_matrix add_diag(const dev_var_matrix& A, const var& d) {
-  return internal::add_diag_dev(internal::operand(A), d.val(), d.vi_, {});
+  return internal::add_diag_dev(internal::structured_operand(A), d.val(), d.vi_, {});
 }
 inline dev_var_matrix add_diag(const dev_var_matrix& A, double d) {
-  return internal::add_diag_dev(internal::operand(A), d, nullptr, {});
+  return internal::add_diag_dev(internal::structured_operand(A), d, nullptr, {});
 }
 inline dev_var_matrix add_diag(const dev_data<double>& A, const var& d) {
   return internal::add_diag_dev(internal::operand(A), d.val(), d.vi_, {});
@@ -335,6 +341,13 @@
   auto* L = new dev_matrix_vari(n, n, dev_structure::lower);
   L->aux_ = amd::alloc_doubles(size_t(smg_cholesky_aux_doubles(n)));
   const size_t pos = ChainableStack::instance_->var_stack_.size();
+  {
+    const bool dense = !internal::cholesky_dev_vari::closed_form_enabled() ||
+                       internal::cholesky_dev_vari::history_of(pos, n) == 0;
+    if (dense || !A.vi_->sink_) A.vi_->want_adjoint();
+    if (dense && A.vi_->sink_) A.vi_->sink_->expect_dense_adjoint();
+    if (dense) L->want_adjoint();
+  }
   double* inv_ws = nullptr;
   want_w = want_w && !host_out && n % 512 == 0 && n >= 1024;
   if (want_w || (internal::cholesky_dev_vari::closed_form_enabled() && internal::cholesky_dev_vari::predicted(pos, n)))
diff --git a/math_amd/include/stan/math/rev/fun/gp_ard_cov.hpp b/math_amd/include/stan/math/rev/fun/gp_ard_cov.hpp
--- a/math_amd/include/stan/math/rev/fun/gp_ard_cov.hpp
+++ b/math_amd/include/stan/math/rev/fun/gp_ard_cov.hpp
@@ -99,9 +99,9 @@
 
   void expand_adjoint() override {
     const size_t sw = ChainableStack::instance_->sweep_;
-    if (exp_.C && exp_.sweep == sw) exp_.expand_into(K_->adj_);
+    if (exp_.C && exp_.sweep == sw) exp_.expand_into(K_->adj());
     exp_ = inverse_adjoint{};
-    if (dep_.C && dep_.sweep == sw) dep_.expand_into(K_->adj_);
+    if (dep_.C && dep_.sweep == sw) dep_.expand_into(K_->adj());
     dep_ = inverse_adjoint{};
   }
 
@@ -115,12 +115,12 @@
         exp_ = d;
         return;
       }
-      d.expand_into(K_->adj_);
+      d.expand_into(K_->adj());
     }
     if (!wants_out()) return;
     smg_ctx* c = amd::ctx();
     amd::check(smg_memset(c, out_, 0, size_t(1 + D_) * sizeof(double)), fn_);
-    amd::check(smg_gp_ard_cov_rev(c, family_, zt_, D_, n_, sigma_d_, l_d_, K_->adj_, n_, out_), fn_);
+    amd::check(smg_gp_ard_cov_rev(c, family_, zt_, D_, n_, sigma_d_, l_d_, K_->adj(), n_, out_), fn_);
     deposit_out();
   }
 };
diff --git a/math_amd/include/stan/math/rev/fun/gp_cross_cov.hpp b/math_amd/include/stan/math/rev/fun/gp_cross_cov.hpp
--- a/math_amd/include/stan/math/rev/fun/gp_cross_cov.hpp
+++ b/math_amd/include/stan/math/rev/fun/gp_cross_cov.hpp
@@ -53,7 +53,7 @@
     if (!sigma_vi_ && !l_vi_) return;
     smg_ctx* c = amd::ctx();
     amd::check(smg_memset(c, out2_, 0, 2 * sizeof(double)), fn_);
-    amd::check(smg_gp_cross_cov_rev(c, family_, x1_, n1_, x2_, n2_, D_, sigma_d_, l_d_, K_->adj_, n1_, out2_), fn_);
+    amd::check(smg_gp_cross_cov_rev(c, family_, x1_, n1_, x2_, n2_, D_, sigma_d_, l_d_, K_->adj(), n1_, out2_), fn_);
     if (sigma_vi_) add_pending_adjoint(sigma_vi_, out2_);
     if (l_vi_) add_pending_adjoint(l_vi_, out2_ + 1);
   }
@@ -109,7 +109,7 @@
     if (!sigma_vi_ && !l_vis_) return;
     smg_ctx* c = amd::ctx();
     amd::check(smg_memset(c, out_, 0, size_t(1 + D_) * sizeof(double)), fn_);
-    amd::check(smg_gp_ard_cross_cov_rev(c, family_, z1t_, n1_, z2t_, n2_, D_, sigma_d_, l_d_, K_->adj_, n1_, out_), fn_);
+    amd::check(smg_gp_ard_cross_cov_rev(c, family_, z1t_, n1_, z2t_, n2_, D_, sigma_d_, l_d_, K_->adj(), n1_, out_), fn_);
     if (sigma_vi_) add_pending_adjoint(sigma_vi_, out_);
     if (l_vis_)
       for (int d = 0; d < D_; ++d) add_pending_adjoint(l_vis_[d], out_ + 1 + d);
diff --git a/math_amd/include/stan/math/rev/fun/gp_exp_quad_cov.hpp b/math_amd/include/stan/math/rev/fun/gp_exp_quad_cov.hpp
--- a/math_amd/include/stan/math/rev/fun/gp_exp_quad_cov.hpp
+++ b/math_amd/include/stan/math/rev/fun/gp_exp_quad_cov.hpp
@@ -100,9 +100,9 @@
   }
   void expand_adjoint() override {
     const size_t sw = ChainableStack::instance_->sweep_;
-    if (exp_.C && exp_.sweep == sw) exp_.expand_into(K_->adj_);
+    if (exp_.C && exp_.sweep == sw) exp_.expand_into(K_->adj());
     exp_ = inverse_adjoint{};
-    if (dep_.C && dep_.sweep == sw) dep_.expand_into(K_->adj_);
+    if (dep_.C && dep_.sweep == sw) dep_.expand_into(K_->adj());
     dep_ = inverse_adjoint{};
   }
 
@@ -117,14 +117,14 @@
         exp_ = d;
         return;
       }
-      d.expand_into(K_->adj_);
+      d.expand_into(K_->adj());
     }
     if (!sigma_vi_ && !l_vi_) return;
     smg_ctx* c = amd::ctx();
     amd::check(smg_memset(c, out2_, 0, 2 * sizeof(double)), fn_);
     amd::check(family_ == SMG_GP_EXP_QUAD
-                   ? smg_gp_exp_quad_cov_nd_rev(c, x_, D_, n_, sigma_d_, l_d_, K_->adj_, n_, out2_)
-                   : smg_gp_cov_rev(c, family_, x_, D_, n_, sigma_d_, l_d_, K_->adj_, n_, out2_),
+                   ? smg_gp_exp_quad_cov_nd_rev(c, x_, D_, n_, sigma_d_, l_d_, K_->adj(), n_, out2_)
+                   : smg_gp_cov_rev(c, family_, x_, D_, n_, sigma_d_, l_d_, K_->adj(), n_, out2_),
                fn_);
     if (sigma_vi_) add_pending_adjoint(sigma_vi_, out2_);
     if (l_vi_) add_pending_adjoint(l_vi_, out2_ + 1);
diff --git a/math_amd/include/stan/math/rev/fun/gp_periodic_cov.hpp b/math_amd/include/stan/math/rev/fun/gp_periodic_cov.hpp
--- a/math_amd/include/stan/math/rev/fun/gp_periodic_cov.hpp
+++ b/math_amd/include/stan/math/rev/fun/gp_periodic_cov.hpp
@@ -55,7 +55,7 @@
     if (!sigma_vi_ && !l_vi_ && !p_vi_) return;
     smg_ctx* c = amd::ctx();
     amd::check(smg_memset(c, out3_, 0, 3 * sizeof(double)), fn_);
-    amd::check(smg_gp_periodic_cov_rev(c, x1_, n1_, x2_, n2_, D_, sigma_d_, l_d_, p_d_, K_->adj_, n1_, out3_), fn_);
+    amd::check(smg_gp_periodic_cov_rev(c, x1_, n1_, x2_, n2_, D_, sigma_d_, l_d_, p_d_, K_->adj(), n1_, out3_), fn_);
     if (sigma_vi_) add_pending_adjoint(sigma_vi_, out3_);
     if (l_vi_) add_pending_adjoint(l_vi_, out3_ + 1);
     if (p_vi_) add_pending_adjoint(p_vi_, out3_ + 2);
@@ -90,7 +90,7 @@
     if (!sigma_vi_) return;
     smg_ctx* c = amd::ctx();
     amd::check(smg_memset(c, out1_, 0, sizeof(double)), fn_);
-    amd::check(smg_gp_dot_prod_cov_rev(c, n1_, n2_, sigma_d_, K_->adj_, n1_, out1_), fn_);
+    amd::check(smg_gp_dot_prod_cov_rev(c, n1_, n2_, sigma_d_, K_->adj(), n1_, out1_), fn_);
     add_pending_adjoint(sigma_vi_, out1_);
   }
 };
diff --git a/math_amd/include/stan/math/rev/fun/lgamma.hpp b/math_amd/include/stan/math/rev/fun/lgamma.hpp
--- a/math_amd/include/stan/math/rev/fun/lgamma.hpp
+++ b/math_amd/include/stan/math/rev/fun/lgamma.hpp
@@ -30,6 +30,7 @@
   dev_matrix_vari* y_;
   explicit unary_special_dev_vari(dev_matrix_vari* x)
       : device_vari(0.0), x_(x), y_(new dev_matrix_vari(x->rows_, x->cols_)) {
+    x->want_adjoint();
     const long long n = (long long)x_->size();
     amd::check(OP == 0 ? smg_lgamma_fwd(amd::ctx(), x_->val(), n, y_->raw_val())
                        : smg_digamma_fwd(amd::ctx(), x_->val(), n, y_->raw_val()),
@@ -37,8 +38,8 @@
   }
   void chain() override {
     const long long n = (long long)x_->size();
-    amd::check(OP == 0 ? smg_lgamma_rev(amd::ctx(), x_->val(), n, y_->adj_, x_->adj_)
-                       : smg_digamma_rev(amd::ctx(), x_->val(), n, y_->adj_, x_->adj_),
+    amd::check(OP == 0 ? smg_lgamma_rev(amd::ctx(), x_->val(), n, y_->adj(), x_->adj())
+                       : smg_digamma_rev(amd::ctx(), x_->val(), n, y_->adj(), x_->adj()),
                OP == 0 ? "lgamma" : "digamma");
   }
 };
diff --git a/math_amd/include/stan/math/rev/fun/log_determinant.hpp b/math_amd/include/stan/math/rev/fun/log_determinant.hpp
--- a/math_amd/include/stan/math/rev/fun/log_determinant.hpp
+++ b/math_amd/include/stan/math/rev/fun/log_determinant.hpp
@@ -16,12 +16,14 @@
   double* LU_;
   int* piv_;
   log_determinant_dev_vari(double v, dev_matrix_vari* A, double* LU, int* piv)
-      : device_vari(v), A_(A), LU_(LU), piv_(piv) {}
+      : device_vari(v), A_(A), LU_(LU), piv_(piv) {
+    A->want_adjoint();
+  }
   void chain() override {
     const int n = A_->rows_;
     double* ws = amd::alloc_doubles(3 * size_t(n) * n);
     int* iws = amd::alloc_ints(size_t(n));
-    amd::check(smg_log_determinant_rev(amd::ctx(), LU_, piv_, n, adj_, A_->adj_, n, ws, iws), "log_determinant");
+    amd::check(smg_log_determinant_rev(amd::ctx(), LU_, piv_, n, adj_, A_->adj(), n, ws, iws), "log_determinant");
   }
 };
 
diff --git a/math_amd/include/stan/math/rev/fun/log_sum_exp.hpp b/math_amd/include/stan/math/rev/fun/log_sum_exp.hpp
--- a/math_amd/include/stan/math/rev/fun/log_sum_exp.hpp
+++ b/math_amd/include/stan/math/rev/fun/log_sum_exp.hpp
@@ -14,10 +14,12 @@
 class log_sum_exp_dev_vari : public device_vari {
  public:
   dev_matrix_vari* x_;
-  log_sum_exp_dev_vari(double v, dev_matrix_vari* x) : device_vari(v), x_(x) {}
+  log_sum_exp_dev_vari(double v, dev_matrix_vari* x) : device_vari(v), x_(x) {
+    x->want_adjoint();
+  }
   void chain() override {
     amd::check(smg_log_sum_exp_rev(amd::ctx(), x_->val(), (long long)x_->size(), val_, adj_,
-                                   x_->adj_),
+                                   x_->adj()),
                "log_sum_exp");
   }
 };
diff --git a/math_amd/include/stan/math/rev/fun/mdivide_left_tri.hpp b/math_amd/include/stan/math/rev/fun/mdivide_left_tri.hpp
--- a/math_amd/include/stan/math/rev/fun/mdivide_left_tri.hpp
+++ b/math_amd/include/stan/math/rev/fun/mdivide_left_tri.hpp
@@ -35,13 +35,13 @@
     double* ws = amd::alloc_doubles(size_t(m) * n);
     if (W_) {
       smg_ctx* c = amd::ctx();
-      amd::check(smg_trmv_inv(c, 1, W_, A_.rows, m, C_->adj_, ws), "mdivide_left_tri");
+      amd::check(smg_trmv_inv(c, 1, W_, A_.rows, m, C_->adj(), ws), "mdivide_left_tri");
       if (A_.adj()) amd::check(smg_rank1_lower(c, m, -1.0, ws, C_->raw_val(), A_.adj(), A_.rows), "mdivide_left_tri");
       if (B_.adj()) amd::check(smg_axpy(c, (long long)m, 1.0, ws, 1, B_.adj(), 1), "mdivide_left_tri");
       return;
     }
     amd::check(smg_mdivide_left_tri_aux_rev(amd::ctx(), lower_, A_.val(), A_.rows, aux(), C_->raw_val(), m,
-                                            C_->adj_, m, m, n, A_.adj(), A_.rows, B_.adj(), m, ws),
+                                            C_->adj(), m, m, n, A_.adj(), A_.rows, B_.adj(), m, ws),
                "mdivide_left_tri");
   }
 };
diff --git a/math_amd/include/stan/math/rev/fun/multi_normal_cholesky_lpdf.hpp b/math_amd/include/stan/math/rev/fun/multi_normal_cholesky_lpdf.hpp
--- a/math_amd/include/stan/math/rev/fun/multi_normal_cholesky_lpdf.hpp
+++ b/math_amd/include/stan/math/rev/fun/multi_normal_cholesky_lpdf.hpp
@@ -28,7 +28,11 @@
 
   mvn_cholesky_dev_vari(double lp, dev_matrix_vari* L, const double* ws,
                         dev_matrix_vari* y = nullptr, dev_matrix_vari* mu = nullptr)
-      : device_vari(lp), L_(L), ws_(ws), n_(L->rows_), y_(y), mu_(mu) {}
+      : device_vari(lp), L_(L), ws_(ws), n_(L->rows_), y_(y), mu_(mu) {
+    if (!(L->structure_ == dev_structure::lower && L->sink_)) L->want_adjoint();
+    if (y) y->want_adjoint();
+    if (mu) mu->want_adjoint();
+  }
 
   bool may_write_device_adjoint(const void* node) const override {
     return (node == L_ && !deposited_) || (y_ && node == y_) || (mu_ && node == mu_);
@@ -38,8 +42,8 @@
     const int lower_only = L_->structure_ == dev_structure::lower ? 1 : 0;
     deposited_ = lower_only && L_->sink_ && L_->sink_->take_mvn_adjoint(this, ws_, adj_);
     amd::check(smg_mvn_cholesky_rev(amd::ctx(), L_->val(), n_, L_->aux_, n_, ws_, adj_, lower_only,
-                                    y_ ? y_->adj_ : nullptr, mu_ ? mu_->adj_ : nullptr,
-                                    deposited_ ? nullptr : L_->adj_, n_),
+                                    y_ ? y_->adj() : nullptr, mu_ ? mu_->adj() : nullptr,
+                                    deposited_ ? nullptr : L_->adj(), n_),
                "multi_normal_cholesky_lpdf");
   }
 };
@@ -162,7 +166,7 @@
   if (!include_const) lp -= -std::log(std::sqrt(2.0 * 3.14159265358979323846)) * n * k;
   if (!include_logdet) lp -= host_logdet * k;
   *lp_out = lp;
-  bool any_adj = L.adj() != nullptr;
+  bool any_adj = L.vi != nullptr;
   for (int i = 0; i < k; ++i) any_adj = any_adj || obs[i].yadj || obs[i].muadj;
   if (!any_adj) return nullptr;
   return new mvn_multi_dev_vari(lp, L, aux, lower_only ? 1 : 0, ws, obs, k);
diff --git a/math_amd/include/stan/math/rev/fun/multiply.hpp b/math_amd/include/stan/math/rev/fun/multiply.hpp
--- a/math_amd/include/stan/math/rev/fun/multiply.hpp
+++ b/math_amd/include/stan/math/rev/fun/multiply.hpp
@@ -66,10 +66,10 @@
     smg_ctx* c = amd::ctx();
     if (lowvec_) {
       const int m = A_.rows;
-      if (A_.adj()) amd::check(smg_rank1_lower(c, m, 1.0, C_->adj_, B_.val(), A_.adj(), m), "multiply");
+      if (A_.adj()) amd::check(smg_rank1_lower(c, m, 1.0, C_->adj(), B_.val(), A_.adj(), m), "multiply");
       if (B_.adj()) {
         double* t = amd::alloc_doubles(size_t(m));
-        amd::check(smg_trmv_inv(c, 1, A_.val(), A_.rows, m, C_->adj_, t), "multiply");
+        amd::check(smg_trmv_inv(c, 1, A_.val(), A_.rows, m, C_->adj(), t), "multiply");
         amd::check(smg_axpy(c, (long long)m, 1.0, t, 1, B_.adj(), 1), "multiply");
       }
       return;
@@ -77,13 +77,13 @@
     if (gram_) {
       const int m = C_->rows_;
       double* S = amd::alloc_doubles(size_t(m) * m);
-      amd::check(smg_memcpy_d2d(c, S, C_->adj_, size_t(m) * m * sizeof(double)), "multiply");
-      amd::check(smg_transpose(c, m, m, C_->adj_, m, S, m, 1.0), "multiply");
+      amd::check(smg_memcpy_d2d(c, S, C_->adj(), size_t(m) * m * sizeof(double)), "multiply");
+      amd::check(smg_transpose(c, m, m, C_->adj(), m, S, m, 1.0), "multiply");
       amd::check(smg_gemm(c, 0, 0, 0, m, A_.cols, m, 1.0, S, m, A_.val(), A_.rows, 1.0, A_.adj(), A_.rows),
                  "multiply");
       return;
     }
-    amd::check(smg_multiply_rev(c, A_.val(), A_.rows, B_.val(), B_.rows, C_->adj_, C_->rows_, A_.rows, A_.cols,
+    amd::check(smg_multiply_rev(c, A_.val(), A_.rows, B_.val(), B_.rows, C_->adj(), C_->rows_, A_.rows, A_.cols,
                                 B_.cols, A_.adj(), A_.rows, B_.adj(), B_.rows),
                "multiply");
   }
@@ -107,10 +107,10 @@
   void chain() override {
     smg_ctx* x = amd::ctx();
     const long long n = (long long)A_.rows * A_.cols;
-    if (A_.adj()) amd::check(smg_axpy(x, n, c_, B_->adj_, 1, A_.adj(), 1), "multiply");
+    if (A_.adj()) amd::check(smg_axpy(x, n, c_, B_->adj(), 1, A_.adj(), 1), "multiply");
     if (c_vi_) {
       amd::check(smg_memset(x, cadj_, 0, sizeof(double)), "multiply");
-      amd::check(smg_dot(x, B_->adj_, A_.val(), n, cadj_), "multiply");
+      amd::check(smg_dot(x, B_->adj(), A_.val(), n, cadj_), "multiply");
       add_pending_adjoint(c_vi_, cadj_);
     }
   }
@@ -122,13 +122,14 @@
   dev_matrix_vari* B_;
   explicit transpose_dev_vari(dev_matrix_vari* A)
       : device_vari(0.0), A_(A), B_(new dev_matrix_vari(A->cols_, A->rows_)) {
+    A->want_adjoint();
     B_->transpose_of_ = A;
     amd::check(smg_transpose(amd::ctx(), A_->rows_, A_->cols_, A_->val(), A_->rows_, B_->raw_val(),
                              B_->rows_, 0.0),
                "transpose");
   }
   void chain() override {
-    amd::check(smg_transpose(amd::ctx(), B_->rows_, B_->cols_, B_->adj_, B_->rows_, A_->adj_,
+    amd::check(smg_transpose(amd::ctx(), B_->rows_, B_->cols_, B_->adj(), B_->rows_, A_->adj(),
                              A_->rows_, 1.0),
                "transpose");
   }
@@ -137,10 +138,12 @@
 class sum_dev_vari : public device_vari {
  public:
   dev_matrix_vari* A_;
-  sum_dev_vari(double v, dev_matrix_vari* A) : device_vari(v), A_(A) {}
+  sum_dev_vari(double v, dev_matrix_vari* A) : device_vari(v), A_(A) {
+    A->want_adjoint();
+  }
   void chain() override {
     const int uplo = A_->structure_ == dev_structure::lower ? 1 : 0;
-    amd::check(smg_shift(amd::ctx(), A_->rows_, A_->cols_, adj_, A_->adj_, A_->rows_, uplo), "sum");
+    amd::check(smg_shift(amd::ctx(), A_->rows_, A_->cols_, adj_, A_->adj(), A_->rows_, uplo), "sum");
   }
 };
 
diff --git a/math_amd/include/stan/math/rev/fun/normal_id_glm_lpdf.hpp b/math_amd/include/stan/math/rev/fun/normal_id_glm_lpdf.hpp
--- a/math_amd/include/stan/math/rev/fun/normal_id_glm_lpdf.hpp
+++ b/math_amd/include/stan/math/rev/fun/normal_id_glm_lpdf.hpp
@@ -40,7 +40,7 @@
     if (beta_vi_)
       for (int j = 0; j < M_; ++j) beta_vi_[j]->adj_ += adj_ * g_[1 + j];
     if (beta_dev_)
-      amd::check(smg_axpy(amd::ctx(), M_, adj_, g_dev_, 1, beta_dev_->adj_, 1), "normal_id_glm_lpdf");
+      amd::check(smg_axpy(amd::ctx(), M_, adj_, g_dev_, 1, beta_dev_->adj(), 1), "normal_id_glm_lpdf");
     if (sigma_vi_) sigma_vi_->adj_ += adj_ * g_[M_ + 1];
   }
 };
diff --git a/math_amd/include/stan/math/rev/fun/spd_functors.hpp b/math_amd/include/stan/math/rev/fun/spd_functors.hpp
--- a/math_amd/include/stan/math/rev/fun/spd_functors.hpp
+++ b/math_amd/include/stan/math/rev/fun/spd_functors.hpp
@@ -62,7 +62,7 @@
     const int m = B_.rows, n = B_.cols;
     if (!A_.adj() && !B_.adj()) return;
     double* ws = amd::alloc_doubles(size_t(m) * n);
-    amd::check(smg_mdivide_left_spd_rev(amd::ctx(), L_, aux_, m, n, C_->raw_val(), m, C_->adj_, m, A_.adj(), m,
+    amd::check(smg_mdivide_left_spd_rev(amd::ctx(), L_, aux_, m, n, C_->raw_val(), m, C_->adj(), m, A_.adj(), m,
                                         B_.adj(), m, ws),
                "mdivide_left_spd");
   }
@@ -81,11 +81,13 @@
   double* L_;
   double* aux_;
   log_determinant_spd_dev_vari(double v, dev_matrix_vari* A, double* L, double* aux)
-      : device_vari(v), A_(A), L_(L), aux_(aux) {}
+      : device_vari(v), A_(A), L_(L), aux_(aux) {
+    A->want_adjoint();
+  }
   void chain() override {
     const int n = A_->rows_;
     double* ws = amd::alloc_doubles(size_t(n) * n);
-    amd::check(smg_log_determinant_spd_rev(amd::ctx(), L_, aux_, n, adj_, A_->adj_, n, ws),
+    amd::check(smg_log_determinant_spd_rev(amd::ctx(), L_, aux_, n, adj_, A_->adj(), n, ws),
                "log_determinant_spd");
   }
 };
@@ -96,6 +98,7 @@
   dev_matrix_vari* C_;
   explicit mlt_self_transpose_dev_vari(dev_matrix_vari* L)
       : device_vari(0.0), L_(L), C_(new dev_matrix_vari(L->rows_, L->rows_)) {
+    L->want_adjoint();
     const int K = L->rows_, J = L->cols_;
     double* ws = amd::alloc_doubles(size_t(K) * (J > 0 ? J : 1));
     amd::check(smg_multiply_lower_tri_self_transpose_fwd(amd::ctx(), L_->val(), K, K, J, C_->raw_val(), K, ws),
@@ -104,8 +107,8 @@
   void chain() override {
     const int K = L_->rows_, J = L_->cols_;
     double* ws = amd::alloc_doubles(size_t(2) * K * J + size_t(K) * K);
-    amd::check(smg_multiply_lower_tri_self_transpose_rev(amd::ctx(), L_->val(), K, K, J, C_->adj_, K,
-                                                         L_->adj_, K, ws),
+    amd::check(smg_multiply_lower_tri_self_transpose_rev(amd::ctx(), L_->val(), K, K, J, C_->adj(), K,
+                                                         L_->adj(), K, ws),
                "multiply_lower_tri_self_transpose");
   }
 };
@@ -127,7 +130,7 @@
     const int M = B_.rows, N = B_.cols;
     if (!A_.adj() && !B_.adj()) return;
     double* ws = amd::alloc_doubles(size_t(M) * N + size_t(N) * N);
-    amd::check(smg_quad_form_sym_rev(amd::ctx(), A_.val(), M, B_.val(), M, M, N, C_->adj_, N, sym_adj_,
+    amd::check(smg_quad_form_sym_rev(amd::ctx(), A_.val(), M, B_.val(), M, M, N, C_->adj(), N, sym_adj_,
                                      A_.adj(), M, B_.adj(), M, ws),
                "quad_form_sym");
   }
diff --git a/math_amd/include/stan/math/rev/fun/tangent_ops.hpp b/math_amd/include/stan/math/rev/fun/tangent_ops.hpp
--- a/math_amd/include/stan/math/rev/fun/tangent_ops.hpp
+++ b/math_amd/include/stan/math/rev/fun/tangent_ops.hpp
@@ -29,7 +29,7 @@
   void chain() override {
     smg_ctx* c = amd::ctx();
     amd::check(smg_memset(c, out4_, 0, 4 * sizeof(double)), "gp_exp_quad_cov");
-    amd::check(smg_gp_exp_quad_cov_tangent_rev(c, x_, n_, s_, l_, ds_, dl_, K_->adj_, n_, out4_),
+    amd::check(smg_gp_exp_quad_cov_tangent_rev(c, x_, n_, s_, l_, ds_, dl_, K_->adj(), n_, out4_),
                "gp_exp_quad_cov");
     for (int i = 0; i < 4; ++i)
       if (vis_[i]) add_pending_adjoint(vis_[i], out4_ + i);
@@ -42,10 +42,11 @@
   dev_matrix_vari* Y_;
   explicit phi_dev_vari(dev_matrix_vari* X)
       : device_vari(0.0), X_(X), Y_(new dev_matrix_vari(X->rows_, X->cols_, dev_structure::lower)) {
+    X->want_adjoint();
     amd::check(smg_phi(amd::ctx(), X_->rows_, X_->val(), X_->rows_, Y_->raw_val(), Y_->rows_, 0), "phi");
   }
   void chain() override {
-    amd::check(smg_phi(amd::ctx(), X_->rows_, Y_->adj_, Y_->rows_, X_->adj_, X_->rows_, 1), "phi");
+    amd::check(smg_phi(amd::ctx(), X_->rows_, Y_->adj(), Y_->rows_, X_->adj(), X_->rows_, 1), "phi");
   }
 };
 
@@ -53,12 +54,15 @@
  public:
   dev_matrix_vari* x_;
   dev_matrix_vari* y_;
-  dot_dev_vari(double v, dev_matrix_vari* x, dev_matrix_vari* y) : device_vari(v), x_(x), y_(y) {}
+  dot_dev_vari(double v, dev_matrix_vari* x, dev_matrix_vari* y) : device_vari(v), x_(x), y_(y) {
+    x->want_adjoint();
+    y->want_adjoint();
+  }
   void chain() override {
     smg_ctx* c = amd::ctx();
     const long long n = (long long)x_->size();
-    amd::check(smg_axpy(c, n, adj_, y_->val(), 1, x_->adj_, 1), "dot_product");
-    amd::check(smg_axpy(c, n, adj_, x_->val(), 1, y_->adj_, 1), "dot_product");
+    amd::check(smg_axpy(c, n, adj_, y_->val(), 1, x_->adj(), 1), "dot_product");
+    amd::check(smg_axpy(c, n, adj_, x_->val(), 1, y_->adj(), 1), "dot_product");
   }
 };
 
@@ -66,10 +70,13 @@
  public:
   dev_matrix_vari* A_;
   dev_matrix_vari* B_;
-  diag_ratio_dev_vari(double v, dev_matrix_vari* A, dev_matrix_vari* B) : device_vari(v), A_(A), B_(B) {}
+  diag_ratio_dev_vari(double v, dev_matrix_vari* A, dev_matrix_vari* B) : device_vari(v), A_(A), B_(B) {
+    A->want_adjoint();
+    B->want_adjoint();
+  }
   void chain() override {
     amd::check(smg_diag_ratio_rev(amd::ctx(), A_->rows_, A_->val(), A_->rows_, B_->val(), B_->rows_,
-                                  adj_, A_->adj_, A_->rows_, B_->adj_, B_->rows_),
+                                  adj_, A_->adj(), A_->rows_, B_->adj(), B_->rows_),
                "diag_ratio_sum");
   }
 };
diff --git a/math_amd/include/stan/math/rev/functor/gradient.hpp b/math_amd/include/stan/math/rev/functor/gradient.hpp
--- a/math_amd/include/stan/math/rev/functor/gradient.hpp
+++ b/math_amd/include/stan/math/rev/functor/gradient.hpp
@@ -52,7 +52,7 @@
     var fx_var = f(dev_var_matrix(leaf));
     fx = fx_var.val();
     grad(fx_var.vi_);
-    amd::check(smg_memcpy_d2d(c, grad_dev, leaf->adj_, n * sizeof(double)), "gradient");
+    amd::check(smg_memcpy_d2d(c, grad_dev, leaf->adj(), n * sizeof(double)), "gradient");
   } catch (const std::exception& e) {
     recover_memory_nested();
     throw;
diff --git a/math_amd/include/stan/math/rev/meta/operands_and_partials.hpp b/math_amd/include/stan/math/rev/meta/operands_and_partials.hpp
--- a/math_amd/include/stan/math/rev/meta/operands_and_partials.hpp
+++ b/math_amd/include/stan/math/rev/meta/operands_and_partials.hpp
@@ -248,7 +248,7 @@
     for (size_t i = 0; i < size_; ++i) varis_[i]->adj_ += adj_ * partials_[i];
     for (int i = 0; i < ndev_; ++i)
       amd::check(smg_axpy(amd::ctx(), (long long)dev_[i].op->size(), adj_, dev_[i].partials, 1,
-                          dev_[i].op->adj_, 1),
+                          dev_[i].op->adj(), 1),
                  "operands_and_partials");
   }
 };
```

Measured after the change: 483.9 gradient evals/s, median of 6. +2.2%, better.
